# steineggerlab/Metabuli

Hardware: AMD Instinct MI355X
Metric: Mreads/s classified (metabuli classify hot path, reads + index resident in HBM) (higher is better)
Workload: dtype u64

## Files before the change

include/mtb.h:

```cpp
#ifndef MTB_H
#define MTB_H
#include <stddef.h>
#include <stdint.h>

#ifdef __cplusplus
extern "C" {
#endif

typedef enum {
    MTB_OK = 0,
    MTB_ERR_ARG = 1,
    MTB_ERR_IO = 2,
    MTB_ERR_DEVICE = 3,
    MTB_ERR_CAPACITY = 4,
    MTB_ERR_OOM = 5,
    MTB_ERR_UNSUPPORTED = 6
} mtb_status;

typedef struct { uint64_t value; uint64_t qinfo; } mtb_kmer;

typedef struct {
    uint64_t qinfo;
    int32_t  target_id;
    int32_t  species_id;
    uint32_t dna;
    uint16_t right_end_hamming;
    uint8_t  hamming;
    uint8_t  pad;
} mtb_match;

typedef struct {
    int32_t seq_mode;
    int32_t syncmer;
    int32_t smer_len;
    int32_t kmer_format;
    int32_t min_cons_cnt;
    int32_t min_cons_cnt_euk;
    float   min_score;
    float   min_sp_score;
    float   tie_ratio;
    int32_t accession_level;
    int32_t skip_redundancy;
} mtb_params;

typedef struct {
    int32_t  classification;
    float    score;
    int32_t  query_length;
    int32_t  query_length2;
    uint8_t  is_classified;
    uint8_t  reserved;
    uint16_t n_taxcnt;
    uint32_t taxcnt_off;
} mtb_result;

typedef struct mtb_ctx mtb_ctx;
typedef struct mtb_index mtb_index;

enum {
    MTB_K_EXTRACT_COUNT = 0, MTB_K_EXTRACT_EMIT = 1, MTB_K_RADIX_HIST = 2, MTB_K_RADIX_SCATTER = 3,
    MTB_K_JOIN = 4, MTB_K_REGROUP = 5, MTB_K_SEGSORT = 6, MTB_K_SCORE = 7, MTB_K_SCAN = 8, MTB_K_SCORE_FAST = 9,
    MTB_K_SCORE_MANY = 10,
    MTB_NUM_KERNELS = 11
};

typedef struct {
    float    ms_extract, ms_sort, ms_join, ms_regroup, ms_segsort, ms_score, ms_total;
    uint64_t n_reads, n_bases, n_kmers, n_matches, n_targets;
    float    ms_kernel[MTB_NUM_KERNELS];
    uint32_t n_launch[MTB_NUM_KERNELS];
    uint64_t n_generic_reads;
    uint64_t n_slot_reads;
    uint64_t n_deferred_reads, n_many_reads, n_many_matches, n_many_kept;
    int32_t  join_variant, join_tuned;
    float    join_tune_ms[3];
    uint32_t join_tiles, join_tiles_windowed, join_tiles_outside;
    uint32_t lslot_tail_factor, n_lslot_big_reads;
} mtb_batch_stats;

typedef enum { MTB_JOIN_AUTO = 0, MTB_JOIN_Q1W6 = 1, MTB_JOIN_Q2W5 = 2, MTB_JOIN_WINDOW = 3 } mtb_join_variant;

const char *mtb_version(void);
const char *mtb_last_error(void);
void mtb_default_params(mtb_params *p);

mtb_status mtb_ctx_create(int device, void *stream, mtb_ctx **out);
void       mtb_ctx_destroy(mtb_ctx *);
mtb_status mtb_ctx_sync(mtb_ctx *);
mtb_status mtb_ctx_set_profiling(mtb_ctx *, int on);
mtb_status mtb_ctx_set_streams(mtb_ctx *, int n);
mtb_status mtb_ctx_set_workspace_limit(mtb_ctx *, uint64_t bytes);
mtb_status mtb_ctx_set_placement_probe(mtb_ctx *, int on);
mtb_status mtb_ctx_set_join_variant(mtb_ctx *, int variant);
mtb_status mtb_ctx_set_option(mtb_ctx *, const char *name, const char *value);
uint32_t   mtb_ctx_last_sub_batches(const mtb_ctx *);
uint64_t   mtb_ctx_last_scratch_bytes(const mtb_ctx *);

mtb_status mtb_index_open(mtb_ctx *, const char *dbdir, const char *taxonomy_dir,
                          mtb_params *params, mtb_index **out);
mtb_status mtb_index_open_stats(const mtb_index *, uint64_t *out4);
mtb_status mtb_index_from_device(mtb_ctx *, uint64_t *d_values, uint32_t *d_info,
                                 uint64_t n_targets, const char *taxonomy_dir,
                                 const int32_t *taxid_list, size_t n_taxids,
                                 const mtb_params *params, mtb_index **out);
mtb_status mtb_index_clone(mtb_index *src, mtb_ctx *dst_ctx, mtb_index **out);
typedef struct {
    uint8_t  values_handle[64], info_handle[64], dir_handle[64], dirbase_handle[64];
    uint64_t values_off, info_off, dir_off, dirbase_off;
    uint64_t n_targets;
    uint32_t dir_buckets, info_mask;
    int32_t  dir_depth, packed, has_info, match_last, device;
    int64_t  exporter_pid;
    uint64_t values_ptr, info_ptr, dir_ptr, dirbase_ptr;
} mtb_index_share;
mtb_status mtb_index_export(mtb_index *src, mtb_index_share *out);
mtb_status mtb_index_import(mtb_ctx *, const mtb_index_share *, const char *taxonomy_dir, const int32_t *taxid_list, size_t n_taxids,
                            const mtb_params *params, mtb_index **out);
mtb_status mtb_index_seal(mtb_index *);
void       mtb_index_close(mtb_index *);
uint64_t   mtb_index_num_targets(const mtb_index *);
mtb_status mtb_index_state(const mtb_index *, int32_t *dir_depth, int32_t *packed, int32_t *sealed);
mtb_status mtb_index_download(mtb_index *, uint64_t *values, uint32_t *info, uint64_t cap);
int32_t    mtb_tax_lca(const mtb_index *, int32_t a, int32_t b);
int32_t    mtb_tax_species(const mtb_index *, int32_t taxid);
int32_t    mtb_tax_parent(const mtb_index *, int32_t taxid);
int32_t    mtb_tax_max_id(const mtb_index *);
int32_t    mtb_tax_original_id(const mtb_index *, int32_t taxid);
int32_t    mtb_tax_num_children(const mtb_index *, int32_t taxid);
int32_t    mtb_tax_child(const mtb_index *, int32_t taxid, int32_t k);
const char *mtb_tax_rank(const mtb_index *, int32_t taxid);
const char *mtb_tax_name(const mtb_index *, int32_t taxid);

mtb_status mtb_extract(mtb_ctx *, const mtb_params *, const char *bases, const uint64_t *offs,
                       const char *bases2, const uint64_t *offs2, uint64_t n_reads,
                       mtb_kmer *out, uint64_t cap, uint64_t *count,
                       int32_t *qlen, int32_t *qlen2);
mtb_status mtb_sort_kmers(mtb_ctx *, mtb_kmer *kmers, uint64_t n);
mtb_status mtb_match_kmers(mtb_ctx *, mtb_index *, const mtb_kmer *sorted, uint64_t n,
                     mtb_match *out, uint64_t cap, uint64_t *count);
mtb_status mtb_sort_matches(mtb_ctx *, mtb_match *matches, uint64_t n, uint64_t n_reads);
mtb_status mtb_score(mtb_ctx *, mtb_index *, const mtb_params *, const mtb_match *sorted,
                     uint64_t n_matches, uint64_t n_reads, const int32_t *qlen,
                     const int32_t *qlen2, mtb_result *results, int32_t *taxcnt_tax,
                     uint32_t *taxcnt_cnt, uint64_t taxcnt_cap, uint64_t *n_taxcnt);

mtb_status mtb_classify_batch(mtb_ctx *, mtb_index *, const mtb_params *, const char *bases,
                              const uint64_t *offs, const char *bases2, const uint64_t *offs2,
                              uint64_t n_reads, mtb_result *results, int32_t *taxcnt_tax,
                              uint32_t *taxcnt_cnt, uint64_t taxcnt_cap, uint64_t *n_taxcnt);
mtb_status mtb_classify_batch_device(mtb_ctx *, mtb_index *, const mtb_params *,
                                     const char *d_bases, const uint64_t *d_offs,
                                     const char *d_bases2, const uint64_t *d_offs2,
                                     uint64_t n_reads, uint64_t n_bases_total,
                                     mtb_result *d_results, int32_t *d_taxcnt_tax,
                                     uint32_t *d_taxcnt_cnt, uint64_t taxcnt_cap,
                                     uint64_t *n_taxcnt);
void      *mtb_host_alloc(size_t bytes);
void       mtb_host_free(void *);
mtb_status mtb_classify_batch_packed(mtb_ctx *, mtb_index *, const mtb_params *, const uint8_t *packed2, const uint8_t *nmask,
                                     const uint32_t *lens, const uint8_t *packed2_mate, const uint8_t *nmask_mate,
// ... 148 lines not shown
```

metabuli_amd/__init__.py:

```python
from __future__ import annotations

import ctypes as C
import os
import subprocess

import numpy as np

_HERE = os.path.dirname(os.path.abspath(__file__))
_CSRC = os.path.join(_HERE, "csrc")
LIB_PATH = os.environ.get("MTB_LIB") or os.path.join(_CSRC, "libmtb.so")

kmer_dt = np.dtype([("value", "<u8"), ("qinfo", "<u8")])
match_dt = np.dtype([("qinfo", "<u8"), ("target_id", "<i4"), ("species_id", "<i4"), ("dna", "<u4"),
                     ("reh", "<u2"), ("ham", "u1"), ("pad", "u1")])
result_dt = np.dtype([("classification", "<i4"), ("score", "<f4"), ("qlen", "<i4"), ("qlen2", "<i4"),
                      ("is_classified", "u1"), ("flag", "u1"), ("n_taxcnt", "<u2"), ("taxcnt_off", "<u4")])

block_dt = np.dtype([("seq", "<u4"), ("strand", "<i4"), ("start", "<u8"), ("end", "<u8")])

MTB_OK, MTB_ERR_ARG, MTB_ERR_IO, MTB_ERR_DEVICE, MTB_ERR_CAPACITY, MTB_ERR_OOM, MTB_ERR_UNSUPPORTED = range(7)


class Params(C.Structure):
    _fields_ = [("seq_mode", C.c_int32), ("syncmer", C.c_int32), ("smer_len", C.c_int32),
                ("kmer_format", C.c_int32), ("min_cons_cnt", C.c_int32), ("min_cons_cnt_euk", C.c_int32),
                ("min_score", C.c_float), ("min_sp_score", C.c_float), ("tie_ratio", C.c_float),
                ("accession_level", C.c_int32), ("skip_redundancy", C.c_int32)]


class BatchStats(C.Structure):
    _fields_ = [("ms_extract", C.c_float), ("ms_sort", C.c_float), ("ms_join", C.c_float), ("ms_regroup", C.c_float),
                ("ms_segsort", C.c_float), ("ms_score", C.c_float), ("ms_total", C.c_float),
                ("n_reads", C.c_uint64), ("n_bases", C.c_uint64), ("n_kmers", C.c_uint64),
                ("n_matches", C.c_uint64), ("n_targets", C.c_uint64),
                ("ms_kernel", C.c_float * 11), ("n_launch", C.c_uint32 * 11), ("n_generic_reads", C.c_uint64), ("n_slot_reads", C.c_uint64),
                ("n_deferred_reads", C.c_uint64), ("n_many_reads", C.c_uint64), ("n_many_matches", C.c_uint64), ("n_many_kept", C.c_uint64),
                ("join_variant", C.c_int32), ("join_tuned", C.c_int32), ("join_tune_ms", C.c_float * 3),
                ("join_tiles", C.c_uint32), ("join_tiles_windowed", C.c_uint32), ("join_tiles_outside", C.c_uint32),
                ("lslot_tail_factor", C.c_uint32), ("n_lslot_big_reads", C.c_uint32)]


SHARE_BYTES = 4 * 64 + 4 * 8 + 8 + 2 * 4 + 5 * 4 + 4 + 8 + 4 * 8
JOIN_VARIANTS = {0: "other", 1: "q1w6", 2: "q2w5", 3: "window", -3: "q1w5", -4: "q2w6", -15: "windoww5", -16: "windoww6", -17: "windoww7"}


class JoinFootprint(C.Structure):
    _fields_ = [("n_queries", C.c_uint64), ("distinct_buckets", C.c_uint64), ("dir_sectors", C.c_uint64),
                ("target_sectors", C.c_uint64), ("n_buckets", C.c_uint64), ("n_targets", C.c_uint64)]


KERNEL_NAMES = ["extract_count", "extract_emit", "radix_hist", "radix_scatter", "join", "regroup", "segsort", "score", "scan", "score_fast", "score_many"]


class MtbError(RuntimeError):
    def __init__(self, status, msg):
        super().__init__(f"mtb status {status}: {msg}")
        self.status = status


def build(force=False):
    if force and os.path.exists(LIB_PATH):
        os.remove(LIB_PATH)
    subprocess.check_call(["make", "-C", _CSRC, "libmtb.so"], stdout=subprocess.DEVNULL)
    return LIB_PATH


_lib = None


def lib():
    global _lib
    if _lib is not None:
        return _lib
    if not os.path.exists(LIB_PATH):
        raise RuntimeError(f"{LIB_PATH} not found: the HIP extension must be built (python -c 'import __graft_entry__ as g; g.build()'); "
                           "there is no CPU implementation of this path")
    L = C.CDLL(LIB_PATH)
    L.mtb_version.restype = C.c_char_p
    L.mtb_last_error.restype = C.c_char_p
    L.mtb_index_num_targets.restype = C.c_uint64
    L.mtb_index_num_targets.argtypes = [C.c_void_p]
    for f in ("mtb_tax_lca", "mtb_tax_species", "mtb_tax_parent", "mtb_tax_max_id"):
        getattr(L, f).restype = C.c_int32
    L.mtb_tax_lca.argtypes = [C.c_void_p, C.c_int32, C.c_int32]
    L.mtb_tax_species.argtypes = [C.c_void_p, C.c_int32]
    L.mtb_tax_parent.argtypes = [C.c_void_p, C.c_int32]
    L.mtb_tax_max_id.argtypes = [C.c_void_p]
    L.mtb_tax_original_id.restype = C.c_int32
    L.mtb_tax_original_id.argtypes = [C.c_void_p, C.c_int32]
    for f in ("mtb_tax_rank", "mtb_tax_name"):
        getattr(L, f).restype = C.c_char_p
        getattr(L, f).argtypes = [C.c_void_p, C.c_int32]
    _lib = L
    return L


def part_bounds(dbdir, n_parts):
    b = np.zeros(n_parts, np.uint64)
    _chk(lib().mtb_index_part_bounds(dbdir.encode(), C.c_uint32(n_parts), _p(b)))
    return b


def default_params(**kw):
    p = Params(seq_mode=1, syncmer=1, smer_len=5, kmer_format=2, min_cons_cnt=4, min_cons_cnt_euk=9,
               min_score=0.0, min_sp_score=0.0, tie_ratio=0.95, accession_level=0, skip_redundancy=1)
    for k, v in kw.items():
        setattr(p, k, v)
    return p


def _p(a):
    if a is None:
        return None
    if isinstance(a, int):
        return C.c_void_p(a)
    return a.ctypes.data_as(C.c_void_p)


def _chk(st):
    if st != MTB_OK:
        raise MtbError(st, lib().mtb_last_error().decode())

# ... 605 lines not shown
```

metabuli_amd/csrc/kernels_score.h:

```cpp
#ifndef MTB_KERNELS_SCORE_H
#define MTB_KERNELS_SCORE_H
#include "dev_util.h"
#include "mtb_core.h"
#include "kernels_join.h"
#include "mtb_score_par.h"

#ifdef MTB_SCORE_PHASE_CYCLES
#define MTB_NPHASE 16
__device__ unsigned long long mtb_phase_cycles[MTB_NPHASE];
__shared__ unsigned long long mtb_phase_lds[MTB_NPHASE];
#define MTB_PHASE_BEGIN() unsigned long long ph_t0_ = __builtin_readcyclecounter()
#define MTB_PHASE_MARK(k) do { unsigned long long t_ = __builtin_readcyclecounter(); if (threadIdx.x == 0) mtb_phase_lds[k] += t_ - ph_t0_; ph_t0_ = t_; } while (0)
#define MTB_PHASE_KERNEL_BEGIN() do { if (threadIdx.x < MTB_NPHASE) mtb_phase_lds[threadIdx.x] = 0; __syncthreads(); } while (0)
#define MTB_PHASE_KERNEL_END() do { __syncthreads(); if (threadIdx.x < MTB_NPHASE) atomicAdd(&mtb_phase_cycles[threadIdx.x], mtb_phase_lds[threadIdx.x]); } while (0)
#else
#define MTB_PHASE_BEGIN() do {} while (0)
#define MTB_PHASE_MARK(k) do {} while (0)
#define MTB_PHASE_KERNEL_BEGIN() do {} while (0)
#define MTB_PHASE_KERNEL_END() do {} while (0)
#endif

#ifndef MTB_SCORE_LDS
#define MTB_SCORE_LDS 160
#endif
#ifndef MTB_SCORE_MINWAVES
#define MTB_SCORE_MINWAVES 4
#endif
#define MTB_SCORE_BKT 128

__host__ __device__ __forceinline__ uint64_t score_slab_bytes(uint64_t n, uint64_t nb) {
    uint64_t b = mtb_sws_bytes<uint32_t>(n);
    b += nb * 12 + (MTB_LR_MAXE + MTB_LR_MAXE * MTB_LR_K) * 4 + ((nb + 15) & ~15ull);
    return (b + 63) & ~63ull;
}

__global__ __launch_bounds__(64) void k_taxcnt_bound(const uint64_t *__restrict__ seg_start, const uint32_t *__restrict__ cursor,
                                                      const int32_t *__restrict__ qlen, const int32_t *__restrict__ qlen2, uint64_t n_reads,
                                                      int32_t dna_shift, uint32_t *__restrict__ bound) {
    uint64_t r = (uint64_t)blockIdx.x * 64 + threadIdx.x;
    if (r >= n_reads) return;
    uint64_t nb = (uint64_t)mtb_num_buckets(qlen[r] + qlen2[r], dna_shift);
    if (cursor) { bound[r] = (uint32_t)nb; return; }
    uint64_t n = seg_start[r + 1] - seg_start[r];
    bound[r] = (uint32_t)(n < nb ? n : nb);
}

__global__ __launch_bounds__(256) void k_count_flags(const uint8_t *__restrict__ f, uint64_t n, unsigned long long *__restrict__ out) {
    uint32_t c = 0;
    for (uint64_t i = (uint64_t)blockIdx.x * 256 + threadIdx.x; i < n; i += (uint64_t)gridDim.x * 256) c += f[i] == 1 ? 1u : 0u;
    for (int d = 32; d > 0; d >>= 1) c += __shfl_down(c, d, 64);
    if ((threadIdx.x & 63) == 0 && c) atomicAdd(out, (unsigned long long)c);
}

__global__ __launch_bounds__(256) void k_list_flag2(const uint8_t *__restrict__ f, uint64_t n, uint32_t *__restrict__ list, uint32_t *__restrict__ n_list) {
    __shared__ uint32_t s_w[4]; __shared__ uint32_t s_base;
    const uint64_t r = (uint64_t)blockIdx.x * 256 + threadIdx.x;
    const bool on = r < n && f[r] == 2;
    const uint64_t m = __ballot(on);
    const uint32_t wv = threadIdx.x >> 6, lane = threadIdx.x & 63u;
    if (lane == 0) s_w[wv] = (uint32_t)__popcll(m);
    __syncthreads();
    if (threadIdx.x == 0) { const uint32_t tot = s_w[0] + s_w[1] + s_w[2] + s_w[3]; s_base = tot ? atomicAdd(n_list, tot) : 0u; }
    __syncthreads();
    if (on) {
        uint32_t at = s_base + (uint32_t)__popcll(m & ((1ull << lane) - 1ull));
        for (uint32_t q = 0; q < wv; q++) at += s_w[q];
        list[at] = (uint32_t)r;
    }
}

__global__ __launch_bounds__(256) void k_list_large(const uint64_t *__restrict__ seg_start, uint64_t n_reads, uint32_t threshold,
                                                     uint32_t *__restrict__ large, uint32_t *__restrict__ n_large, uint32_t *__restrict__ max_seg) {
    uint64_t r = (uint64_t)blockIdx.x * 256 + threadIdx.x;
    uint32_t n = 0;
    if (r < n_reads) {
        n = (uint32_t)(seg_start[r + 1] - seg_start[r]);
        if (n > threshold) large[atomicAdd(n_large, 1u)] = (uint32_t)r;
    }
    for (int d = 32; d > 0; d >>= 1) { uint32_t o = __shfl_down(n, d, 64); n = o > n ? o : n; }
    if ((threadIdx.x & 63) == 0 && n > threshold) atomicMax(max_seg, n);
}

__device__ __forceinline__ int32_t taxcnt_gather_wave(const int32_t *btax, const uint8_t *bham, int32_t nb, int32_t *otax, uint32_t *ocnt, int32_t cap) {
    const int32_t lane = (int32_t)threadIdx.x;
    int32_t ntc = 0;
    int32_t last = -1;
    while (ntc < cap) {
        int32_t mn = INT32_MAX;
        for (int32_t q = lane; q < nb; q += 64) if (bham[q] != 255) { int32_t t = btax[q]; if (t > last && t < mn) mn = t; }
        for (int d = 32; d > 0; d >>= 1) { int32_t o = __shfl_xor(mn, d, 64); mn = o < mn ? o : mn; }
        if (mn == INT32_MAX) break;
        uint32_t cnt = 0;
        for (int32_t q0 = 0; q0 < nb; q0 += 64) { int32_t q = q0 + lane; cnt += (uint32_t)__popcll(__ballot(q < nb && bham[q] != 255 && btax[q] == mn)); }
        if (lane == 0) { otax[ntc] = mn; ocnt[ntc] = cnt; }
        ntc++; last = mn;
    }
    return ntc;
}

template <typename IDX>
__device__ __forceinline__ void score_sync() {
    if (sizeof(IDX) == 2) { __builtin_amdgcn_fence(__ATOMIC_ACQ_REL, "wavefront"); __builtin_amdgcn_wave_barrier(); }
    else __syncthreads();
}

template <typename IDX, bool SORT, bool KEY64, typename REC, bool INPLACE = false, int CAP = MTB_SCORE_LDS>
__device__ __forceinline__ void score_read_par(const REC *src, int32_t n, mtb_sws<IDX> w, int32_t *btax,
                                               uint8_t *bham, int32_t *otax, uint32_t *ocnt, int32_t *lr_lev, int32_t *lr_anc,
                                               int32_t nb, int32_t read_len, const mtb_tax_view &tx, const mtb_score_params &sp,
                                               uint64_t tc_off, uint64_t tc_room, int32_t *__restrict__ tc_tax,
                                               uint32_t *__restrict__ tc_cnt, uint64_t tc_cap, mtb_match *__restrict__ sorted_out,
                                               mtb_result &R) {
    constexpr int MAXPER = (CAP + 63) / 64;
    if (sizeof(IDX) == 2) __builtin_assume(n >= 1 && n <= CAP);
    const int32_t lane = (int32_t)threadIdx.x;
    const uint64_t lt = lanemask_lt();
    w.n = n;
    MTB_PHASE_BEGIN();
    if (SORT) {
        uint64_t *k1 = (uint64_t *)w.path; uint32_t *k2 = (uint32_t *)(k1 + n);
        mtb_match rec[MAXPER]; uint64_t a1[MAXPER]; uint32_t a2[MAXPER]; int32_t rank[MAXPER];
#pragma unroll
        for (int k = 0; k < MAXPER; k++) {
            int32_t i = lane + 64 * k;
            rank[k] = 0; a1[k] = 0; a2[k] = 0;
            if (i < n) {
                rec[k] = rec_m(src[i]);
                if (KEY64) {
                    a1[k] = ((uint64_t)(uint32_t)rec[k].species_id << 41) | ((uint64_t)mtb_q_frame(rec[k].qinfo) << 38) |
                            ((uint64_t)(mtb_q_pos(rec[k].qinfo) & 0x7FFu) << 27) | ((uint64_t)(rec[k].hamming & 7u) << 24) | (rec[k].dna & 0xFFFFFFu);
                    k1[i] = a1[k];
                } else { a1[k] = mtb_key1(rec[k]); a2[k] = mtb_key2(rec[k]); k1[i] = a1[k]; k2[i] = a2[k]; }
            }
        }
        score_sync<IDX>();
        MTB_PHASE_MARK(0);
        const int32_t nslot = (n + 63) >> 6;
        uint32_t n_desc = 0; int32_t split = 0;
#pragma unroll
        for (int k = 0; k < MAXPER; k++) {
// ... 656 lines not shown
```

metabuli_amd/csrc/kernels_score_fast.h:

```cpp
#ifndef MTB_KERNELS_SCORE_FAST_H
#define MTB_KERNELS_SCORE_FAST_H
#include "dev_util.h"
#include "kernels_score.h"
#include "mtb_core.h"
#include "mtb_score_par.h"

#define MTB_FAST_BKT 128
#ifndef MTB_FAST_MERGE_SINGLES
#define MTB_FAST_MERGE_SINGLES 1
#endif

#ifdef MTB_FAST_DEBUG
__device__ unsigned long long mtb_fast_reasons[32];
#define MTB_FAST_COUNT(k, v) do { if (threadIdx.x == 0) atomicAdd(&mtb_fast_reasons[k], (unsigned long long)(v)); } while (0)
#define MTB_FAST_T0() unsigned long long ft_ = __builtin_readcyclecounter()
#define MTB_FAST_MARK(k) do { const unsigned long long t_ = __builtin_readcyclecounter(); if (threadIdx.x == 0) s_ph[k] += t_ - ft_; ft_ = t_; } while (0)
#else
#define MTB_FAST_COUNT(k, v) do {} while (0)
#define MTB_FAST_T0() do {} while (0)
#define MTB_FAST_MARK(k) do {} while (0)
#endif

#define MTB_DPP_RED(v, OP) do { \
    { const uint32_t o_ = (uint32_t)__builtin_amdgcn_update_dpp((int)(v), (int)(v), 0x111, 0xF, 0xF, false); (v) = OP((v), o_); } \
    { const uint32_t o_ = (uint32_t)__builtin_amdgcn_update_dpp((int)(v), (int)(v), 0x112, 0xF, 0xF, false); (v) = OP((v), o_); } \
    { const uint32_t o_ = (uint32_t)__builtin_amdgcn_update_dpp((int)(v), (int)(v), 0x114, 0xF, 0xF, false); (v) = OP((v), o_); } \
    { const uint32_t o_ = (uint32_t)__builtin_amdgcn_update_dpp((int)(v), (int)(v), 0x118, 0xF, 0xF, false); (v) = OP((v), o_); } \
    { const uint32_t o_ = (uint32_t)__builtin_amdgcn_update_dpp((int)(v), (int)(v), 0x142, 0xA, 0xF, false); (v) = OP((v), o_); } \
    { const uint32_t o_ = (uint32_t)__builtin_amdgcn_update_dpp((int)(v), (int)(v), 0x143, 0xC, 0xF, false); (v) = OP((v), o_); } } while (0)
#define MTB_MINU(a, b) ((b) < (a) ? (b) : (a))
#define MTB_MAXU(a, b) ((b) > (a) ? (b) : (a))
__device__ __forceinline__ uint32_t wave_min_u32(uint32_t v) { MTB_DPP_RED(v, MTB_MINU); return (uint32_t)__builtin_amdgcn_readlane((int)v, 63); }
__device__ __forceinline__ uint32_t wave_max_u32(uint32_t v) { MTB_DPP_RED(v, MTB_MAXU); return (uint32_t)__builtin_amdgcn_readlane((int)v, 63); }

struct FKey { uint32_t lo, hi; };
__device__ __forceinline__ uint32_t fk_species(const FKey &k) { return k.hi >> 10; }
__device__ __forceinline__ uint32_t fk_frame(const FKey &k) { return (k.hi >> 7) & 7u; }
__device__ __forceinline__ uint32_t fk_pos(const FKey &k) { return ((k.hi & 127u) << 4) | (k.lo >> 27); }
__device__ __forceinline__ uint32_t fk_ham(const FKey &k) { return (k.lo >> 24) & 7u; }
__device__ __forceinline__ uint32_t fk_dna(const FKey &k) { return k.lo & 0xFFFFFFu; }

struct FastPath { int32_t start, end; float score; int32_t ham; uint32_t rehs;  int32_t species; };

template <int K, int KL = K, bool BYFRAME = false>
__global__ __launch_bounds__(64, K <= 3 ? 5 : 4) void k_score_fast(const mtb_slot16 *__restrict__ slots_all, uint64_t n_reads, const int32_t *__restrict__ qlen,
                                                       const int32_t *__restrict__ qlen2, mtb_tax_view tx, mtb_score_params sp,
                                                       const uint64_t *__restrict__ tc_off, mtb_result *__restrict__ results,
                                                       int32_t *__restrict__ tc_tax, uint32_t *__restrict__ tc_cnt, uint64_t tc_cap, uint64_t tc_base,
                                                       const uint32_t *__restrict__ cursor, uint32_t stride, uint32_t direct, uint32_t epoch,
                                                       uint8_t *__restrict__ slow_flag, uint32_t *__restrict__ cnt_out) {
    constexpr int NMAX = 64 * K;
    __shared__ FKey s_key[NMAX];
    __shared__ uint64_t s_aux[NMAX];
    __shared__ uint64_t s_pp[NMAX];
    __shared__ FastPath s_path[64];
    __shared__ uint32_t s_pf[64];
    __shared__ uint32_t s_tl[(BYFRAME || MTB_FAST_MERGE_SINGLES) ? 64 : 1];
    typedef uint32_t __attribute__((may_alias)) u32a; typedef int32_t __attribute__((may_alias)) i32a;
    static_assert(NMAX * 8 >= 2 * MTB_FAST_BKT * 4 && NMAX * 8 >= 256 * 4 && NMAX * 8 >= (MTB_LR_MAXE + MTB_LR_MAXE * MTB_LR_K) * 4, "tables fit the arrays they live in");
    u32a *const s_hcnt = (u32a *)s_pp;
    u32a *const s_hmin = (u32a *)s_key; i32a *const s_btax = (i32a *)s_key + MTB_FAST_BKT;
    i32a *const s_otax = (i32a *)s_pp; u32a *const s_ocnt = (u32a *)s_pp + MTB_FAST_BKT;
    i32a *const s_lev = (i32a *)s_aux; i32a *const s_anc = (i32a *)s_aux + MTB_LR_MAXE;
    const int32_t lane = (int32_t)threadIdx.x;
    MTB_BEGIN_ACQUIRE();
#ifdef MTB_FAST_DEBUG
    __shared__ unsigned long long s_ph[16];
    if (threadIdx.x < 16) s_ph[threadIdx.x] = 0;
#endif
    const uint64_t lt = lanemask_lt();
    const uint64_t le = lt | (1ull << lane);
    const uint32_t tail_cap = stride - direct;
    const uint32_t div_m = (65536u + (uint32_t)sp.dna_shift - 1u) / (uint32_t)sp.dna_shift;
    const uint32_t lines = (stride * (uint32_t)sizeof(mtb_slot16) + 127u) / 128u;

    for (uint64_t r = blockIdx.x; r < n_reads; r += gridDim.x) {
        if (r + gridDim.x < n_reads && (uint32_t)lane < lines) {
            const uint8_t *pf = (const uint8_t *)(slots_all + (r + gridDim.x) * (uint64_t)stride) + (uint64_t)lane * 128u;
            __builtin_amdgcn_global_load_lds((const __attribute__((address_space(1))) void *)pf, (__attribute__((address_space(3))) void *)s_pf, 4, 0, 0);
        }
        MTB_FAST_T0();
        const int32_t ql1 = qlen[r], ql2 = qlen2[r];
        const int32_t read_len = ql1 + ql2;
        const int32_t nb = mtb_num_buckets(read_len, sp.dna_shift);
        const uint32_t cur = cursor[r];
        const mtb_slot16 *slots = slots_all + r * (uint64_t)stride;
        mtb_slot16 x[KL];
#pragma unroll
        for (int k = 0; k < KL; k++) { const uint32_t i = (uint32_t)lane + 64u * k; x[k].a = 0; x[k].b = 0; if (i < stride) x[k] = slots[i]; }
        bool slow = cur > tail_cap || nb > MTB_FAST_BKT;
        wave_fence();
        MTB_FAST_MARK(0);
        int32_t n = 0, n_live = 0;
        uint32_t spc[KL]; bool live[KL]; int32_t dst[KL];
        uint32_t smin = 0xFFFFFFFFu, smax = 0u;
#pragma unroll
        for (int k = 0; k < KL; k++) {
            const uint32_t i = (uint32_t)lane + 64u * k;
            live[k] = i < stride && mtb_slot_epoch(x[k]) == epoch && (i < direct || i - direct < cur);
            spc[k] = live[k] ? (uint32_t)(x[k].a >> 32) : 0xFFFFFFFFu;
            dst[k] = 0;
            n_live += (int32_t)__popcll(__ballot(live[k]));
            smin = spc[k] < smin ? spc[k] : smin;
            if (live[k]) smax = spc[k] > smax ? spc[k] : smax;
        }
        smin = wave_min_u32(smin); smax = wave_max_u32(smax);
        uint32_t todo_min = 0xFFFFFFFFu;
        if (smin != smax) {
            for (int32_t q = lane; q < 256; q += 64) s_hcnt[q] = 0;
            wave_fence();
#pragma unroll
            for (int k = 0; k < KL; k++) if (live[k]) atomicAdd(&s_hcnt[(spc[k] * 0x9E3779B1u) >> 24], 1u);
            wave_fence();
#pragma unroll
            for (int k = 0; k < KL; k++) if (live[k] && s_hcnt[(spc[k] * 0x9E3779B1u) >> 24] < 2u) { live[k] = false; spc[k] = 0xFFFFFFFFu; }
        } else if (n_live < 2) {
#pragma unroll
            for (int k = 0; k < KL; k++) { live[k] = false; spc[k] = 0xFFFFFFFFu; }
        }
        if (BYFRAME) {
#pragma unroll
            for (int k = 0; k < KL; k++) if (live[k]) spc[k] = (spc[k] << 3) | ((uint32_t)(x[k].b >> 52) & 7u);
        }
#pragma unroll
        for (int k = 0; k < KL; k++) todo_min = spc[k] < todo_min ? spc[k] : todo_min;
        for (int round = 0; ; round++) {
            const uint32_t m = wave_min_u32(todo_min);
            if (m == 0xFFFFFFFFu) break;
            if (round == 24) { slow = true; break; }
            todo_min = 0xFFFFFFFFu;
#pragma unroll
            for (int k = 0; k < KL; k++) {
                const bool mine = spc[k] == m;
                const uint64_t mask = __ballot(mine);
                if (mine) { dst[k] = n + (int32_t)__popcll(mask & lt); spc[k] = 0xFFFFFFFFu; }
                n += (int32_t)__popcll(mask);
                todo_min = spc[k] < todo_min ? spc[k] : todo_min;
            }
        }
        if (KL > K && n > NMAX) slow = true;
#pragma unroll
        for (int k = 0; k < KL; k++) {
            if (live[k] && !slow) {
                const uint64_t b = x[k].b;
                const uint32_t bh = (uint32_t)(b >> 32), ps_ = (bh >> 8) & 0x7FFu;
                FKey fk; fk.hi = ((uint32_t)(x[k].a >> 32) << 10) | (((bh >> 20) & 7u) << 7) | (ps_ >> 4);
                fk.lo = ((ps_ & 15u) << 27) | (((bh >> 23) & 7u) << 24) | ((uint32_t)b & 0xFFFFFFu);
                s_key[dst[k]] = fk;
                s_aux[dst[k]] = (x[k].a & 0xFFFFFFFFull) | (((b >> 24) & 0xFFFFull) << 32) | ((uint32_t)lane + 64u * k >= direct ? (1ull << 63) : 0ull);
            }
        }
        MTB_FAST_MARK(1);
        mtb_result R = mtb_result_blank(ql1, ql2, (uint32_t)tc_base);
        if (!slow && n == 0) { if (lane == 0) { cnt_out[r] = (uint32_t)n_live; results[r] = R; } continue; }
        wave_fence();
        {
            uint32_t nt = 0;
            bool any_tail = false;
#pragma unroll
            for (int k = 0; k < KL; k++) any_tail |= live[k] && (uint32_t)lane + 64u * k >= direct;
            if ((BYFRAME || MTB_FAST_MERGE_SINGLES) && !slow && __any(any_tail)) {
                FKey ke[K]; uint64_t ax[K]; int32_t np[K]; bool tl[K];
                const int32_t nsl = (n + 63) >> 6;
                auto same_run = [&](const FKey &a, const FKey &b) { return BYFRAME ? ((a.hi ^ b.hi) >> 7) == 0 : ((a.hi ^ b.hi) >> 10) == 0; };
                auto less = [&](const FKey &a, const FKey &b) { return a.hi < b.hi || (a.hi == b.hi && a.lo < b.lo); };
                bool unsorted = false;
#pragma unroll
                for (int k = 0; k < K; k++) {
                    const int32_t i = lane + 64 * k;
                    ke[k].lo = 0; ke[k].hi = 0; ax[k] = 0; np[k] = i; tl[k] = false;
                    if (k < nsl && i < n) {
                        ke[k] = s_key[i]; ax[k] = s_aux[i]; tl[k] = (ax[k] >> 63) != 0;
                        if (i > 0 && !tl[k]) { const FKey pk = s_key[i - 1]; if ((s_aux[i - 1] >> 63) == 0 && same_run(pk, ke[k]) && less(ke[k], pk)) unsorted = true; }
                    }
                    if (k < nsl) {
                        const uint64_t tm = __ballot(tl[k]);
                        if (tl[k]) { const uint32_t at = nt + (uint32_t)__popcll(tm & lt); if (at < 64u) s_tl[at] = (uint32_t)i; }
                        nt += (uint32_t)__popcll(tm);
                    }
                }
                if (nt > 64u || __any(unsorted)) slow = true;
                wave_fence();
                if (!slow) {
                    const bool mine = (uint32_t)lane < nt;
                    const int32_t ti = mine ? (int32_t)s_tl[lane] : 0;
                    const FKey kt = s_key[ti]; const uint64_t at = s_aux[ti];
                    uint32_t n_tl_run = 0, n_tl_less = 0;
                    for (uint32_t u = 0; u < nt; u++) {
                        FKey ku; ku.hi = (uint32_t)rl_i((int32_t)kt.hi, (int32_t)u); ku.lo = (uint32_t)rl_i((int32_t)kt.lo, (int32_t)u);
                        if (same_run(ku, kt)) { n_tl_run++; n_tl_less += (less(ku, kt) || (!less(kt, ku) && u < (uint32_t)lane)) ? 1u : 0u; }
#pragma unroll
                        for (int k = 0; k < K; k++)
                            if (k < nsl && !tl[k] && same_run(ke[k], ku) && !less(ke[k], ku)) np[k]++;
                    }
                    const uint32_t rid = BYFRAME ? kt.hi >> 7 : kt.hi >> 10;
                    int32_t lo0 = 0, hi0 = n, lo1 = 0, hi1 = n;
                    for (int32_t len = n; len; len >>= 1) {
                        const int32_t m0 = (lo0 + hi0) >> 1, m1 = (lo1 + hi1) >> 1;
                        const uint32_t r0 = BYFRAME ? s_key[m0 < n ? m0 : 0].hi >> 7 : s_key[m0 < n ? m0 : 0].hi >> 10;
                        const uint32_t r1 = BYFRAME ? s_key[m1 < n ? m1 : 0].hi >> 7 : s_key[m1 < n ? m1 : 0].hi >> 10;
                        if (lo0 < hi0) { if (r0 < rid) lo0 = m0 + 1; else hi0 = m0; }
                        if (lo1 < hi1) { if (r1 <= rid) lo1 = m1 + 1; else hi1 = m1; }
                    }
                    const int32_t run_start = lo0, n_dir_run = lo1 - lo0 - (int32_t)n_tl_run;
                    int32_t lo2 = run_start, hi2 = run_start + n_dir_run;
                    for (int32_t len = n; len; len >>= 1) {
                        const int32_t m2 = (lo2 + hi2) >> 1;
                        const FKey km = s_key[m2 < n ? m2 : 0];
                        if (lo2 < hi2) { if (less(km, kt)) lo2 = m2 + 1; else hi2 = m2; }
                    }
                    const int32_t place = lo2 + (int32_t)n_tl_less;
                    wave_fence();
#pragma unroll
                    for (int k = 0; k < K; k++) { const int32_t i = lane + 64 * k; if (k < nsl && i < n && !tl[k]) { s_key[np[k]] = ke[k]; s_aux[np[k]] = ax[k]; } }
                    if (mine) { s_key[place] = kt; s_aux[place] = at & ~(1ull << 63); }
                    wave_fence();
                }
            }
        }
        FKey key[K]; uint32_t tid[K], reh[K];
        int32_t tcanon[K]; uint8_t euk[K];
        const mtb_tax_node *nodes = (const mtb_tax_node *)tx.node;
        bool bhead[K], linked[K];
        int32_t shv[K];
        uint64_t bmask[K + 1], lmask[K + 1], rmask[K];
        const int32_t nslot = (n + 63) >> 6;
        bool bad = false, bad2 = false;
#ifdef MTB_FAST_DEBUG
        if (slow) MTB_FAST_COUNT(cur > tail_cap || nb > MTB_FAST_BKT ? 0 : 1, 1);
#endif
#pragma unroll
        for (int k = 0; k < K; k++) {
            const int32_t i = lane + 64 * k;
            key[k].lo = 0; key[k].hi = 0; tid[k] = 0; reh[k] = 0; bhead[k] = true; linked[k] = false; shv[k] = 0; tcanon[k] = -1; euk[k] = 0;
            bmask[k] = ~0ull; lmask[k] = 0; rmask[k] = 0;
            if (k < nslot && !slow) {
                FKey pk; pk.lo = 0; pk.hi = 0;
                if (i < n) {
                    key[k] = s_key[i]; const uint64_t a = s_aux[i]; tid[k] = (uint32_t)a; reh[k] = (uint32_t)(a >> 32) & 0xFFFFu; if (i > 0) pk = s_key[i - 1];
                }
                {
                    const int32_t t_ = (int32_t)tid[k], s_ = (int32_t)fk_species(key[k]);
                    const bool tv = i < n && t_ >= 0 && t_ <= tx.max_taxid, sv = i < n && s_ >= 0 && s_ <= tx.max_taxid;
                    const int32_t tc_ = nodes[tv ? t_ : 0].canon; const uint8_t eu_ = tx.under_euk[sv ? s_ : 0];
                    tcanon[k] = tv ? tc_ : -1; euk[k] = sv ? eu_ : 0;
                }
                const bool first = i == 0;
                if (i < n && !first) {
                    if (pk.hi > key[k].hi || (pk.hi == key[k].hi && pk.lo > key[k].lo)) bad = true;
                    if (pk.hi == key[k].hi && ((pk.lo ^ key[k].lo) >> 27) == 0) bad2 = true;
                }
                bhead[k] = i >= n || first || ((pk.hi ^ key[k].hi) >> 7) != 0;
                if (i < n && !bhead[k]) {
                    const int32_t pos = (int32_t)fk_pos(key[k]), ppos = (int32_t)fk_pos(pk);
                    const int32_t s = (pos - ppos) / 3;
                    if (s > 0 && s <= sp.max_codon_shift) {
                        shv[k] = s;
                        const bool fwd = fk_frame(key[k]) < 3u;
                        linked[k] = mtb_consecutive(fk_dna(pk), fk_dna(key[k]), s, fwd, sp.kmer_format);
                    }
                }
                bmask[k] = __ballot(bhead[k]);
                lmask[k] = __ballot(linked[k]);
                rmask[k] = __ballot(i < n && !linked[k]);
            }
        }
        bmask[K] = ~0ull; lmask[K] = 0;
#ifdef MTB_FAST_DEBUG
        if (!slow) { if (__any(bad)) MTB_FAST_COUNT(2, 1); else if (__any(bad2)) MTB_FAST_COUNT(3, 1); }
#endif
        slow = slow || __any(bad || bad2);
        if (slow) { if (lane == 0) slow_flag[r] = cur > tail_cap ? 2 : 1; continue; }
        if (lane == 0) cnt_out[r] = (uint32_t)n_live;
        MTB_FAST_MARK(2);
        float ps[K]; int32_t phd[K]; int32_t root[K];
        bool cand[K];
        {
            float carry_s = 0.0f; int32_t carry_hd = 0, last_root = 0;
#pragma unroll
            for (int k = 0; k < K; k++) {
                ps[k] = 0.0f; phd[k] = 0; root[k] = 0; cand[k] = false;
                if (k < nslot) {
                    const int32_t i = lane + 64 * k;
                    float is = 0.0f; int32_t ihd = 0;
                    if (linked[k]) mtb_link_inc(reh[k], shv[k], &is, &ihd);
                    ps[k] = wave_inclusive_scan_dpp(is) + carry_s; phd[k] = wave_inclusive_scan_dpp(ihd) + carry_hd;
                    carry_s = rl_f(ps[k], 63); carry_hd = rl_i(phd[k], 63);
                    const uint64_t mr = rmask[k];
                    const uint64_t lo_roots = mr & le;
                    root[k] = lo_roots ? 64 * k + 63 - (int32_t)__builtin_clzll(lo_roots) : last_root;
                    if (mr) last_root = 64 * k + 63 - (int32_t)__builtin_clzll(mr);
                    if (i < n) s_pp[i] = (uint64_t)__float_as_uint(ps[k]) | ((uint64_t)(uint32_t)phd[k] << 32);
                    const uint64_t bnext = (bmask[k] >> 1) | ((bmask[k + 1] & 1ull) << 63);
                    const uint64_t lnext = (lmask[k] >> 1) | ((lmask[k + 1] & 1ull) << 63);
                    const bool has_next = !((bnext >> lane) & 1ull);
                    const bool conn = (lnext >> lane) & 1ull;
                    cand[k] = i < n && (!bhead[k] || has_next) && !conn;
                }
            }
        }
        wave_fence();
        MTB_FAST_MARK(3);
        int32_t ne = 0;
        bool too_many = false;
#pragma unroll
        for (int k = 0; k < K; k++) {
            if (k < nslot) {
                bool e = false;
                FastPath P; P.start = 0; P.end = 0; P.score = 0.0f; P.ham = 0; P.rehs = 0; P.species = 0;
                if (cand[k]) {
                    const int32_t spc = (int32_t)fk_species(key[k]);
                    const int32_t md = euk[k] ? sp.min_cons_cnt_euk : sp.min_cons_cnt;
                    const int32_t rt = root[k];
                    const uint64_t pr = s_pp[rt]; const FKey rkey = s_key[rt];
                    const uint32_t rreh = (uint32_t)(s_aux[rt] >> 32);
                    const int32_t dhd = phd[k] - (int32_t)(uint32_t)(pr >> 32);
                    const int32_t depth = 1 + mtb_link_depth(dhd);
                    if (depth >= md) {
                        e = true;
                        P.start = (int32_t)fk_pos(rkey);
                        P.end = (int32_t)fk_pos(key[k]) + 23;
                        P.score = mtb_part_score(rreh, 8, false) + (rt == lane + 64 * k ? 0.0f : ps[k] - __uint_as_float((uint32_t)pr));
                        P.ham = (int32_t)fk_ham(rkey) + (rt == lane + 64 * k ? 0 : mtb_link_ham(dhd));
                        P.rehs = rreh | (reh[k] << 16);
                        P.species = spc;
                    }
                }
                const uint64_t me = __ballot(e);
                const int32_t at = ne + (int32_t)__popcll(me & lt);
                if (e && at < 64) s_path[at] = P;
                ne += (int32_t)__popcll(me);
            }
        }
        too_many = ne > 64;
        if (too_many) MTB_FAST_COUNT(4, 1); else { MTB_FAST_COUNT(5, 1); MTB_FAST_COUNT(6, ne); }
        if (too_many) { if (lane == 0) slow_flag[r] = 1; continue; }
        if (ne == 0) { if (lane == 0) results[r] = R; continue; }
        wave_fence();
        MTB_FAST_MARK(4);
        FastPath P = s_path[lane < ne ? lane : 0];
        const bool have = lane < ne;
        int32_t prev_spc = __shfl_up(P.species, 1, 64);
        const bool shead = have && (lane == 0 || prev_spc != P.species);
        const uint64_t hmask = __ballot(shead);
        const int32_t nsp = (int32_t)__popcll(hmask);
        MTB_FAST_COUNT(7, nsp);

        float sp_score = -1.0f; int32_t sp_id = 0;
        int32_t s_idx = 0;
        const uint32_t ord = __float_as_uint(P.score);
        const uint32_t tie = ((uint32_t)(1023 - (P.ham < 1023 ? P.ham : 1023)) << 17) | ((uint32_t)(P.start & 0x7FF) << 6) | (uint32_t)(63 - lane);
        for (uint64_t hm = hmask; hm; hm &= hm - 1, s_idx++) {
            const int32_t slo = (int32_t)__builtin_ctzll(hm);
            const int32_t shi = (hm & (hm - 1)) ? (int32_t)__builtin_ctzll(hm & (hm - 1)) : ne;
            const bool in = lane >= slo && lane < shi;
// ... 140 lines not shown
```

metabuli_amd/csrc/mtb_api.hip:

```cpp
#include <hip/hip_runtime.h>

#include <fcntl.h>
#include <limits.h>
#include <stdlib.h>
#include <sys/stat.h>
#include <unistd.h>

#include <atomic>
#include <chrono>
#include <condition_variable>
#include <mutex>
#include <functional>
#include <map>
#include <string>
#include <thread>
#include <vector>

#include "../../include/mtb.h"
#include "host_db.h"
#include "host/merge_plan.h"
#include "host/audit_plan.h"
#include "host/clade_filter.h"
#include "kernels_extract.h"
#include "kernels_extract_blocks.h"
#include "kernels_index.h"
#include "kernels_join.h"
#include "kernels_build.h"
#include "kernels_merge.h"
#include "kernels_clade_filter.h"
#include "kernels_audit.h"
#include "kernels_coverage.h"
#include "kernels_inspect.h"
#include "kernels_dir.h"
#include "kernels_scan.h"
#include "kernels_score.h"
#include "kernels_score_fast.h"
#include "kernels_score_long.h"
#include "kernels_score_many.h"
#include "kernels_seg_order.h"
#include "kernels_sort.h"
#include "mtb_core.h"
#include "mtb_options.h"

#if defined(__HIP_DEVICE_COMPILE__) && defined(__AMDGCN__) && !defined(__gfx950__)
#error "libmtb is written for gfx950 (MI355X) only: 160 KB of LDS per CU (k_score_long holds 70 KB per workgroup), global_load_lds_dwordx4, wave64"
#endif

static thread_local std::string g_err;
static mtb_status fail(mtb_status s, const std::string &m) { g_err = m; return s; }

#define HIPCHK(x)                                                                                  \
    do {                                                                                           \
        hipError_t e_ = (x);                                                                       \
        if (e_ != hipSuccess)                                                                      \
            return fail(MTB_ERR_DEVICE, std::string(#x) + ": " + hipGetErrorString(e_));           \
    } while (0)
#define STCHK(x)                                                                                   \
    do { mtb_status s_ = (x); if (s_ != MTB_OK) return s_; } while (0)

__global__ __launch_bounds__(256) void k_taxcnt_n(const mtb_result *__restrict__ res, uint64_t n, uint32_t *__restrict__ cnt) {
    const uint64_t i = (uint64_t)blockIdx.x * 256 + threadIdx.x;
    if (i < n) cnt[i] = res[i].n_taxcnt;
}
__global__ __launch_bounds__(256) void k_taxcnt_pack(mtb_result *__restrict__ res, uint64_t n, const uint64_t *__restrict__ new_off, const int32_t *__restrict__ tt,
                                                      const uint32_t *__restrict__ tc, int32_t *__restrict__ tt2, uint32_t *__restrict__ tc2) {
    const uint64_t i = (uint64_t)blockIdx.x * 256 + threadIdx.x;
    if (i >= n) return;
    const uint32_t k = res[i].n_taxcnt, src = res[i].taxcnt_off;
    const uint64_t dst = new_off[i];
    for (uint32_t j = 0; j < k; j++) { tt2[dst + j] = tt[src + j]; tc2[dst + j] = tc[src + j]; }
    res[i].taxcnt_off = (uint32_t)dst;
}

__global__ __launch_bounds__(256) void k_pack_slots(const uint32_t *__restrict__ lens, uint64_t n, uint32_t *__restrict__ slots) {
    const uint64_t i = (uint64_t)blockIdx.x * 256 + threadIdx.x;
    if (i < n) slots[i] = (lens[i] + 7u) >> 3;
}
__global__ __launch_bounds__(64) void k_unpack_reads(const uint8_t *__restrict__ packed2, const uint8_t *__restrict__ nmask, const uint64_t *__restrict__ offs,
                                                     const uint64_t *__restrict__ slot_off, uint64_t n, char *__restrict__ bases) {
    for (uint64_t r = blockIdx.x; r < n; r += gridDim.x) {
        const uint64_t o = offs[r], s0 = slot_off[r];
        const uint32_t L = (uint32_t)(offs[r + 1] - o);
        for (uint32_t k = threadIdx.x; k < L; k += 64) {
            const uint64_t g = s0 + (k >> 3); const uint32_t j = k & 7u;
            const uint32_t w = (uint32_t)packed2[2 * g] | ((uint32_t)packed2[2 * g + 1] << 8);
            const bool bad = (nmask[g] >> j) & 1u;
            const uint32_t c = (w >> (2 * j)) & 3u;
            bases[o + k] = bad ? 'N' : (char)((0x47544341u >> (8 * c)) & 0xFFu);
        }
    }
}

enum BufKind : uint8_t { BUF_WORK = 0, BUF_IO = 1, BUF_FIXED = 2 };
struct DevBuf { void *p = nullptr; size_t cap = 0; BufKind kind = BUF_WORK; };
#define MTB_SLAB_POOL_MAX (16ull << 30)
#define MTB_LONG_WIN_MAX_PER_Q 24.0
#define MTB_OVF_STRIPES 256u

enum Scal : uint32_t {
    SC_JOIN_COUNT = 0, SC_JOIN_OVERFLOW = 1,
    SC_BAD_SEQ = SC_JOIN_OVERFLOW,
    SC_N_LARGE = 2, SC_MAX_SEG = 3,
    SC_MAX_LEN = 4, SC_OPEN_CARRY = 5,
    SC_N_GENERIC = 6, SC_LONG_N_SECOND = 7,
    SC_EXTRACT = 8, SC_WIN_STATS = 16,
    SC_N_UNGROUPED = 18, SC_MAX_BIG_SEG = 19, SC_N_DEFERRED = 20, SC_DEFER_N_LARGE = 21,
    SC_SCORE_WORK = 22, SC_LONG_WORK = 24,
    SC_LS_N_FAIL = 25, SC_LS_N_ALL = 26, SC_LS_MAX_SEG = 27, SC_LS_WORK = 28,
    SC_OPEN_FLAGS = 29, SC_WORDS = 30
};
struct ExtractCounters { uint64_t records , overflow, real, max_q , off_max_q, off_reads, off_max_len , spare; };
static_assert(sizeof(ExtractCounters) == 8 * (SC_WIN_STATS - SC_EXTRACT) && SC_WIN_STATS + 2 <= SC_N_UNGROUPED && SC_SCORE_WORK + 2 <= SC_LONG_WORK && SC_OPEN_FLAGS < SC_WORDS, "scalar names overlap or leave the block");
struct mtb_ctx {
    int device = 0;
    int audit_mode = 0;
    hipStream_t stream = nullptr;
    mtb_tables *d_tabs = nullptr;
    mtb_tables h_tabs;
    std::map<std::string, DevBuf> bufs;
    std::mutex bufs_mu;
    std::mutex reserve_mu;
    std::atomic<bool> reserve_cancel{false};
    uint64_t *d_scal = nullptr;
    unsigned long long *d_ovfctr = nullptr;
    uint64_t ovf_region = 0, ovf_max_region = 0;
    hipEvent_t ev[8];
    mtb_batch_stats stats;
    int profiling = 0;
    struct KEv { int id; hipEvent_t a, b; };
    std::vector<KEv> kev;
    std::vector<hipEvent_t> ev_pool;
    std::vector<mtb_ctx *> lanes;
    bool is_lane = false;
    uint32_t seg_epoch = 0;
    const void *seg_clean_p = nullptr; size_t seg_clean_cap = 0;
    double extract_yield = 0.0;
    uint64_t part_n_reads = 0; uint32_t part_max_len = 0;
    int part_mode = 0; uint32_t part_max_q = 0; uint64_t part_nk_real = 0;
    bool placement_probe = false;
    uint64_t ws_limit = 0;
    double ws_per_base = 0.0;
    uint64_t ws_max_sub_bases = 0;
    int ws_seq_mode = 0;
    uint32_t last_sub_batches = 0;
    bool fast_used = false;
    const mtb_kmer *last_sorted = nullptr; uint64_t last_sorted_n = 0;
    struct DeadSeg { char *p; size_t cap, used; };
    DeadSeg dead[3]; int n_dead = 0;
    uint64_t last_scratch_bytes = 0;
    hipStream_t copy_stream = nullptr; hipEvent_t copy_done[2] = {nullptr, nullptr};
    hipEvent_t unpacked[2] = {nullptr, nullptr};
    bool unpacked_rec[2] = {false, false};
    uint64_t prefetch_issued = 0, prefetch_used = 0;
    hipStream_t down_stream = nullptr; hipEvent_t down_ready = nullptr, down_done = nullptr; bool down_pending = false; int res_set = 0;
    int pk_set = 0;
    struct Prefetched { const void *key = nullptr, *key2 = nullptr; uint64_t n_reads = 0; bool valid = false; } pre[2];
    struct JoinTune { uint64_t key = 0; int calls = 0, pending = -1, best = -1; float ms[3] = {0.0f, 0.0f, 0.0f}; hipEvent_t e0 = nullptr, e1 = nullptr; } join_tunes[4]; uint32_t join_tune_next = 0;
    uint64_t many_stats[4] = {0, 0, 0, 0};
    uint32_t lslot_tf_start = 1;
    unsigned long long *d_cov_pend = nullptr; uint64_t cov_pend_words = 0; bool cov_call = false;
    MtbOptions opt;
};
template <typename T> static T *scal(mtb_ctx *c, Scal s) { return (T *)(c->d_scal + s); }
static hipError_t scal_clear(mtb_ctx *c, Scal first, uint32_t words = 1) { return hipMemsetAsync(c->d_scal + first, 0, 8 * (size_t)words, c->stream); }
static DevBuf buf_get(mtb_ctx *c, const std::string &name) { std::lock_guard<std::mutex> lk(c->bufs_mu); auto it = c->bufs.find(name); return it == c->bufs.end() ? DevBuf() : it->second; }
static size_t buf_cap(mtb_ctx *c, const char *name) { return buf_get(c, name).cap; }
static size_t held_bytes(mtb_ctx *c, BufKind upto) { std::lock_guard<std::mutex> lk(c->bufs_mu); size_t b = 0; for (auto &kv : c->bufs) if (kv.second.kind == BUF_WORK || kv.second.kind == upto) b += kv.second.cap; return b; }
static void release_workspace(mtb_ctx *c) {
    std::lock_guard<std::mutex> lk(c->bufs_mu);
    for (auto &kv : c->bufs) if (kv.second.p && kv.second.kind != BUF_IO) { hipError_t e = hipFree(kv.second.p); (void)e; kv.second.p = nullptr; kv.second.cap = 0; }
    c->ws_per_base = 0.0; c->ws_max_sub_bases = 0;
    c->seg_clean_p = nullptr; c->seg_clean_cap = 0;
}

struct KTimer {
    mtb_ctx *c; int id; hipEvent_t a = nullptr, b = nullptr;
    KTimer(mtb_ctx *c_, int id_) : c(c_), id(id_) {
        if (!c->profiling) return;
        a = take(); b = take();
        hipError_t e = hipEventRecord(a, c->stream); (void)e;
    }
    ~KTimer() {
        if (!c->profiling) return;
        hipError_t e = hipEventRecord(b, c->stream); (void)e;
        c->kev.push_back({id, a, b});
    }
    hipEvent_t take() {
        hipEvent_t ev;
        if (!c->ev_pool.empty()) { ev = c->ev_pool.back(); c->ev_pool.pop_back(); return ev; }
        hipError_t e = hipEventCreate(&ev); (void)e;
        return ev;
    }
};
static void collect_kernel_times(mtb_ctx *c) {
    for (auto &k : c->kev) {
        float ms = 0;
        if (hipEventElapsedTime(&ms, k.a, k.b) == hipSuccess) { c->stats.ms_kernel[k.id] += ms; c->stats.n_launch[k.id]++; }
        c->ev_pool.push_back(k.a); c->ev_pool.push_back(k.b);
    }
    c->kev.clear();
}

struct mtb_index {
    mtb_ctx *ctx = nullptr;
    uint64_t T = 0;
    uint64_t *d_values = nullptr; uint32_t *d_info = nullptr; bool own = false;
    bool own_tax = true;
    bool match_last = false;
    mtbhost::Taxonomy tax;
    int32_t *d_canon = nullptr, *d_parent = nullptr, *d_depth = nullptr, *d_spparent = nullptr, *d_tax2species = nullptr;
    uint8_t *d_under = nullptr, *d_accleaf = nullptr;
    mtb_tax_node *d_node = nullptr;
    mtb_params params;
    uint32_t info_mask = 0xFFFFFFFFu;
    uint32_t *d_dir = nullptr; uint64_t *d_dirbase = nullptr; int32_t dir_L = 0; uint32_t dir_buckets = 0;
    bool packed = false;
    bool info_owned = false;
    std::mutex state_mu; std::condition_variable state_cv; int users = 0;
    int views = 0;
    mtb_index *parent = nullptr;
    uint64_t open_chunks = 0, open_chunk_words = 0, open_peak_bytes = 0, open_free0 = 0;
    void *ipc_stage[4] = {nullptr, nullptr, nullptr, nullptr};
    bool is_part = false;
    uint32_t *d_cov_bits = nullptr; unsigned long long *d_cov_hits = nullptr;
};

enum ResKind { RES_ROWS = 0, RES_TAX = 1, RES_CNT = 2 };
static const char *res_name(ResKind k, int set) { static const char *const names[2][3] = {{"results", "tctax2", "tccnt2"}, {"resultsb", "tctax2b", "tccnt2b"}}; return names[set ? 1 : 0][k]; }
template <typename T>
static mtb_status ensure(mtb_ctx *c, const char *name, size_t elems, T **out, BufKind kind = BUF_WORK) {
    if (c->down_pending) {
        const int fl = c->res_set ^ 1;
        if (!strcmp(name, res_name(RES_ROWS, fl)) || !strcmp(name, res_name(RES_TAX, fl)) || !strcmp(name, res_name(RES_CNT, fl))) { HIPCHK(hipEventSynchronize(c->down_done)); c->down_pending = false; }
    }
    std::lock_guard<std::mutex> lk(c->bufs_mu);
    DevBuf &b = c->bufs.emplace(name, DevBuf{nullptr, 0, kind}).first->second;
    size_t bytes = elems * sizeof(T);
    if (bytes == 0) bytes = 64;
// ... 50 lines not shown
        const size_t want = bytes + bytes / 16 + 256 + (c->opt.segm_pad ? (1u << 20) : 0);
        hipError_t e = hipExtMallocWithFlags(&b.p, want, hipDeviceMallocContiguous);
        if (e != hipSuccess) { b.p = nullptr; (void)hipGetLastError(); return fail(MTB_ERR_OOM, std::string("contiguous allocation failed for ") + name + ": " + hipGetErrorString(e)); }
        b.cap = want;
        *out = (mtb_slot16 *)b.p;
        return MTB_OK;
    }
    const bool no_probe = c->opt.no_placement_probe != 0, env_probe = c->opt.placement_probe != 0;
    if (b.cap >= bytes || bytes < (8ull << 30) || no_probe || !(c->placement_probe || env_probe)) return plain();
    if (b.p) { hipError_t e = hipFree(b.p); (void)e; b.p = nullptr; b.cap = 0; }
    const size_t want = bytes + bytes / 16 + 256;
    const auto t_begin = std::chrono::steady_clock::now();
    struct Cand { void *p; float ms; size_t bytes; };
    std::vector<Cand> held;
    std::vector<float> seen; std::vector<void *> seen_p, pads; std::vector<size_t> sizes;
    hipEvent_t e0 = nullptr, e1 = nullptr;
    struct Guard {
        std::vector<Cand> &held; std::vector<void *> &pads; hipEvent_t &e0, &e1; bool armed = true;
        ~Guard() { if (!armed) return; for (auto &h : held) { hipError_t e = hipFree(h.p); (void)e; } for (void *q : pads) { hipError_t e = hipFree(q); (void)e; }
                   if (e0) { hipError_t e = hipEventDestroy(e0); (void)e; } if (e1) { hipError_t e = hipEventDestroy(e1); (void)e; } }
    } guard{held, pads, e0, e1};
    HIPCHK(hipEventCreate(&e0)); HIPCHK(hipEventCreate(&e1));
    for (int attempt = 0; attempt < 8; attempt++) {
        if (attempt >= 2 && std::chrono::duration<double>(std::chrono::steady_clock::now() - t_begin).count() > 2.0) break;
        size_t fr = 0, tot = 0;
        HIPCHK(hipMemGetInfo(&fr, &tot));
        if (want + (attempt ? (8ull << 30) : 0) > fr) {
            if (held.size() < 2) break;
            size_t worst = 0; for (size_t k = 1; k < held.size(); k++) if (held[k].ms > held[worst].ms) worst = k;
            { hipError_t e = hipFree(held[worst].p); (void)e; } held.erase(held.begin() + (long)worst);
            void *pad = nullptr;
            if (hipMalloc(&pad, ((size_t)(attempt % 3) + 1) * (3ull << 30)) == hipSuccess) pads.push_back(pad); else (void)hipGetLastError();
            HIPCHK(hipMemGetInfo(&fr, &tot));
            if (want + (4ull << 30) > fr) break;
        }
        void *p = nullptr;
        const size_t ask = want;
        if (hipMalloc(&p, ask) != hipSuccess) { (void)hipGetLastError(); break; }
        sizes.push_back(ask);
        float best = 1e30f;
        for (int rep = 0; rep < 3; rep++) {
            HIPCHK(hipEventRecord(e0, c->stream));
            hipLaunchKernelGGL(k_probe_scatter, dim3(8192), dim3(256), 0, c->stream, (mtb_slot16 *)p, (uint64_t)(bytes / sizeof(mtb_slot16)), 8u, 12345u + (uint32_t)rep);
            HIPCHK(hipEventRecord(e1, c->stream));
            HIPCHK(hipEventSynchronize(e1));
            float ms = 0; HIPCHK(hipEventElapsedTime(&ms, e0, e1));
            if (rep && ms < best) best = ms;
        }
        held.push_back({p, best, ask}); seen.push_back(best); seen_p.push_back(p);
        float lo = 1e30f; for (float v : seen) lo = std::min(lo, v);
        int near = 0; for (float v : seen) if (v <= lo * 1.03f) near++;
        float hi = 0.0f; for (float v : seen) hi = std::max(hi, v);
        if (seen.size() >= 4 && near >= 2 && lo <= 0.9f * hi) break;
    }
    guard.armed = false;
    (void)hipEventDestroy(e0); (void)hipEventDestroy(e1);
    for (void *q : pads) { hipError_t e = hipFree(q); (void)e; }
    if (held.empty()) return plain();
    size_t pick = 0;
    for (size_t k = 1; k < held.size(); k++) if (held[k].ms < held[pick].ms) pick = k;
    for (size_t k = 0; k < held.size(); k++) if (k != pick) { hipError_t e = hipFree(held[k].p); (void)e; }
    std::vector<Cand> &cands = held;
    if (c->opt.placement_verbose) { fprintf(stderr, "mtb: slot buffer placement probe:"); for (size_t k = 0; k < seen.size(); k++) fprintf(stderr, " %.3f@%p", seen[k], seen_p[k]); fprintf(stderr, " ms -> %.3f (%.0f ms spent)\n", cands[pick].ms, std::chrono::duration<double, std::milli>(std::chrono::steady_clock::now() - t_begin).count()); }
    b.p = cands[pick].p; b.cap = cands[pick].bytes;
    *out = (mtb_slot16 *)b.p;
    return MTB_OK;
}
static void release(mtb_ctx *c, const char *name) {
    std::lock_guard<std::mutex> lk(c->bufs_mu);
    auto it = c->bufs.find(name);
    if (it != c->bufs.end()) { if (it->second.p) { hipError_t e = hipFree(it->second.p); (void)e; } c->bufs.erase(it); }
}

extern "C" {

const char *mtb_version(void) { return "metabuli_amd 0.1 (gfx950)"; }
const char *mtb_last_error(void) { return g_err.c_str(); }

void mtb_default_params(mtb_params *p) {
    p->seq_mode = 2; p->syncmer = 0; p->smer_len = 5; p->kmer_format = 1; p->min_cons_cnt = 4; p->min_cons_cnt_euk = 9;
    p->min_score = 0.0f; p->min_sp_score = 0.0f; p->tie_ratio = 0.95f; p->accession_level = 0; p->skip_redundancy = 0;
}

mtb_status mtb_ctx_create(int device, void *stream, mtb_ctx **out) {
    if (!out) return fail(MTB_ERR_ARG, "out is NULL");
    int n = 0;
    hipError_t e = hipGetDeviceCount(&n);
    if (e != hipSuccess || n <= 0) return fail(MTB_ERR_DEVICE, "no HIP device available (this library has no CPU path)");
    if (device < 0 || device >= n) return fail(MTB_ERR_ARG, "bad device ordinal");
    HIPCHK(hipSetDevice(device));
    mtb_ctx *c = new mtb_ctx();
    c->device = device; c->stream = (hipStream_t)stream;
    mtb_build_tables(&c->h_tabs);
    HIPCHK(hipMalloc((void **)&c->d_tabs, sizeof(mtb_tables)));
    HIPCHK(hipMemcpy(c->d_tabs, &c->h_tabs, sizeof(mtb_tables), hipMemcpyHostToDevice));
    HIPCHK(hipMalloc((void **)&c->d_scal, SC_WORDS * sizeof(uint64_t)));
    HIPCHK(hipMalloc((void **)&c->d_ovfctr, MTB_OVF_STRIPES * 64));
    for (int i = 0; i < 8; i++) HIPCHK(hipEventCreate(&c->ev[i]));
    memset(&c->stats, 0, sizeof(c->stats));
    mtbopt::from_environment(&c->opt);
    *out = c;
    return MTB_OK;
}
void mtb_ctx_destroy(mtb_ctx *c) {
    if (!c) return;
    for (mtb_ctx *l : c->lanes) mtb_ctx_destroy(l);
    c->lanes.clear();
    hipError_t e = hipSetDevice(c->device); (void)e;
    e = hipStreamSynchronize(c->stream);
    { std::lock_guard<std::mutex> lk(c->bufs_mu); for (auto &kv : c->bufs) if (kv.second.p) e = hipFree(kv.second.p); }
    if (c->d_tabs && !c->is_lane) e = hipFree(c->d_tabs);
    if (c->d_scal) e = hipFree(c->d_scal);
    if (c->d_ovfctr) e = hipFree(c->d_ovfctr);
    if (c->d_cov_pend && !c->is_lane) e = hipFree(c->d_cov_pend);
    if (c->is_lane && c->stream) e = hipStreamDestroy(c->stream);
    if (c->down_stream) { e = hipStreamSynchronize(c->down_stream); e = hipStreamDestroy(c->down_stream); }
    if (c->down_ready) e = hipEventDestroy(c->down_ready);
    if (c->down_done) e = hipEventDestroy(c->down_done);
    if (c->copy_stream) { e = hipStreamSynchronize(c->copy_stream); e = hipStreamDestroy(c->copy_stream); }
    for (int k = 0; k < 2; k++) { if (c->copy_done[k]) e = hipEventDestroy(c->copy_done[k]); if (c->unpacked[k]) e = hipEventDestroy(c->unpacked[k]); }
    for (int q = 0; q < 4; q++) if (c->join_tunes[q].e0) { e = hipEventDestroy(c->join_tunes[q].e0); e = hipEventDestroy(c->join_tunes[q].e1); }
    for (int i = 0; i < 8; i++) e = hipEventDestroy(c->ev[i]);
    for (auto &k : c->kev) { e = hipEventDestroy(k.a); e = hipEventDestroy(k.b); }
    for (auto &x : c->ev_pool) e = hipEventDestroy(x);
    delete c;
}
mtb_status mtb_ctx_sync(mtb_ctx *c) { HIPCHK(hipStreamSynchronize(c->stream)); return MTB_OK; }
mtb_status mtb_ctx_set_profiling(mtb_ctx *c, int on) {
    if (!c) return fail(MTB_ERR_ARG, "NULL ctx");
    c->profiling = on;
    for (mtb_ctx *l : c->lanes) l->profiling = on;
    return MTB_OK;
}
mtb_status mtb_ctx_set_placement_probe(mtb_ctx *c, int on) {
    if (!c) return fail(MTB_ERR_ARG, "NULL ctx");
    c->placement_probe = on != 0;
    for (mtb_ctx *l : c->lanes) l->placement_probe = on != 0;
    return MTB_OK;
}
mtb_status mtb_ctx_set_workspace_limit(mtb_ctx *c, uint64_t bytes) {
    if (!c) return fail(MTB_ERR_ARG, "NULL ctx");
    c->ws_limit = bytes;
    for (mtb_ctx *l : c->lanes) l->ws_limit = bytes;
    return MTB_OK;
}
mtb_status mtb_ctx_set_option(mtb_ctx *c, const char *name, const char *value) {
    if (!c || !name) return fail(MTB_ERR_ARG, "NULL ctx / name");
    if (!mtbopt::set(&c->opt, name, value)) return fail(MTB_ERR_ARG, std::string("unknown switch or bad value: ") + name + "=" + (value ? value : "(unset)"));
    for (mtb_ctx *l : c->lanes) l->opt = c->opt;
    return MTB_OK;
}
mtb_status mtb_ctx_set_join_variant(mtb_ctx *c, int variant) {
    static const char *const names[] = {"auto", "q1w6", "q2w5", "window"};
    if (!c || variant < 0 || variant > 3) return fail(MTB_ERR_ARG, "variant must be MTB_JOIN_AUTO .. MTB_JOIN_WINDOW");
    return mtb_ctx_set_option(c, "MTB_JOIN_VARIANT", names[variant]);
}
uint32_t mtb_ctx_last_sub_batches(const mtb_ctx *c) { return c ? c->last_sub_batches : 0; }
uint64_t mtb_ctx_last_scratch_bytes(const mtb_ctx *c) { return c ? c->last_scratch_bytes : 0; }
mtb_status mtb_ctx_set_streams(mtb_ctx *c, int n) {
    if (!c || n < 1 || n > 8) return fail(MTB_ERR_ARG, "streams must be 1..8");
    HIPCHK(hipSetDevice(c->device));
    while ((int)c->lanes.size() > (n == 1 ? 0 : n)) { mtb_ctx_destroy(c->lanes.back()); c->lanes.pop_back(); }
    while (n > 1 && (int)c->lanes.size() < n) {
        mtb_ctx *l = new mtb_ctx();
        l->device = c->device; l->is_lane = true; l->d_tabs = c->d_tabs; l->h_tabs = c->h_tabs; l->profiling = c->profiling; l->placement_probe = c->placement_probe; l->opt = c->opt;
        HIPCHK(hipStreamCreateWithFlags(&l->stream, hipStreamNonBlocking));
        HIPCHK(hipMalloc((void **)&l->d_scal, SC_WORDS * sizeof(uint64_t)));
        HIPCHK(hipMalloc((void **)&l->d_ovfctr, MTB_OVF_STRIPES * 64));
        for (int i = 0; i < 8; i++) HIPCHK(hipEventCreate(&l->ev[i]));
        memset(&l->stats, 0, sizeof(l->stats));
        c->lanes.push_back(l);
    }
    return MTB_OK;
}

}

static mtb_status d2h(mtb_ctx *c, void *dst, const void *src, size_t bytes) {
    HIPCHK(hipMemcpyAsync(dst, src, bytes, hipMemcpyDeviceToHost, c->stream));
    HIPCHK(hipStreamSynchronize(c->stream));
    return MTB_OK;
}
static mtb_status h2d(mtb_ctx *c, void *dst, const void *src, size_t bytes) {
    if (bytes == 0) return MTB_OK;
    HIPCHK(hipMemcpyAsync(dst, src, bytes, hipMemcpyHostToDevice, c->stream));
    HIPCHK(hipStreamSynchronize(c->stream));
    return MTB_OK;
}

static bool sort_msd_first(const mtb_ctx *c) { return !c->opt.sort_lsd; }

static uint64_t extract_bound(uint64_t n_bases, uint32_t grid) { return 2 * n_bases + (uint64_t)grid * MTB_EXTRACT_CHUNK; }
static uint64_t extract_cap_guess(const mtb_ctx *c, const mtb_params *p, uint64_t n_bases, uint32_t grid) {
    const double guess = c->extract_yield > 0.0 ? c->extract_yield : (p->syncmer ? 1.0 : 2.0);
    return std::min<uint64_t>(extract_bound(n_bases, grid), (uint64_t)((double)n_bases * guess * 1.15) + 4096 + (uint64_t)grid * 64);
}

struct Reads {
    const char *d_bases = nullptr; const uint64_t *d_offs = nullptr; const char *d_bases2 = nullptr; const uint64_t *d_offs2 = nullptr; uint64_t n_reads = 0;
    Reads range(uint64_t lo, uint64_t cnt) const { Reads r = *this; r.d_offs += lo; if (r.d_offs2) r.d_offs2 += lo; r.n_reads = cnt; return r; }
};
struct ReadLens { const int32_t *d_ql = nullptr, *d_ql2 = nullptr; uint32_t max_len = 0; };
struct ResultSink { mtb_result *d_res = nullptr; int32_t *d_tc_tax = nullptr; uint32_t *d_tc_cnt = nullptr; uint64_t tc_cap = 0, tc_base = 0; };
struct ExtractOpts {
    bool single_pass = false;
    bool tag_ordinals = false, want_digits = false;
    bool want_max_len = true;
    uint32_t *d_counts = nullptr;
    uint8_t *d_off_reads = nullptr;
};
struct Extracted {
    mtb_kmer *d_k = nullptr; uint64_t nk = 0, nk_real = 0;
    uint32_t max_len = 0, max_q = 0;
    uint16_t *d_dig = nullptr; uint64_t n_bases = 0;
    uint64_t off_max_q = 0, off_reads = 0, off_max_len = 0;
};
static mtb_status dev_extract(mtb_ctx *c, const mtb_params *p, const Reads &rd, int32_t *d_qlen, int32_t *d_qlen2, const ExtractOpts &opt, Extracted *ex) {
    const uint64_t n_reads = rd.n_reads;
    if (n_reads >= (1ull << 29)) return fail(MTB_ERR_ARG, "more than 2^29-1 reads per batch (sequenceID is 29 bits, Kmer.h:13)");
    if (p->kmer_format != 1 && p->kmer_format != 2) return fail(MTB_ERR_UNSUPPORTED, "only kmer_format 1 and 2 are implemented");
    if (p->syncmer && (p->smer_len < 1 || p->smer_len > 8)) return fail(MTB_ERR_ARG, "smer_len out of range");
    *ex = Extracted();
    if (n_reads == 0) return MTB_OK;
    const bool single_pass = opt.single_pass;
    ExtractArgs a{rd.d_bases, rd.d_offs, rd.d_bases2, rd.d_offs2, n_reads, p->seq_mode, p->syncmer, p->smer_len, p->kmer_format, (single_pass && opt.tag_ordinals) ? 1 : 0, sort_msd_first(c) ? 54 : 34};
    uint32_t grid = (uint32_t)std::min<uint64_t>(n_reads, 256ull * 256);
    HIPCHK(scal_clear(c, SC_MAX_LEN));
    uint64_t &n_bases = ex->n_bases;
    if (single_pass) {
        uint64_t o[2];
        STCHK(d2h(c, &o[0], rd.d_offs, 8)); STCHK(d2h(c, &o[1], rd.d_offs + n_reads, 8));
        n_bases = o[1] - o[0];
        if (p->seq_mode == 2 && rd.d_offs2) { STCHK(d2h(c, &o[0], rd.d_offs2, 8)); STCHK(d2h(c, &o[1], rd.d_offs2 + n_reads, 8)); n_bases += o[1] - o[0]; }
    }
    if (single_pass && n_bases) {
        const uint64_t bound = extract_bound(n_bases, grid);
        uint64_t cap = extract_cap_guess(c, p, n_bases, grid);
        cap = std::max<uint64_t>(cap, std::min<uint64_t>(bound, buf_cap(c, "kmersA") / sizeof(mtb_kmer)));
        for (int attempt = 0; attempt < 2; attempt++) {
            mtb_kmer *d_k; uint16_t *d_dig = nullptr;
            STCHK(ensure(c, "kmersA", cap, &d_k));
            if (opt.want_digits) { STCHK(ensure(c, "digA", cap + 8, &d_dig)); ex->d_dig = d_dig; }
            HIPCHK(scal_clear(c, SC_EXTRACT, 8));
            if (opt.d_off_reads) HIPCHK(hipMemsetAsync(opt.d_off_reads, 0, n_reads, c->stream));
            { KTimer kt(c, MTB_K_EXTRACT_EMIT);
            hipLaunchKernelGGL((k_extract<2>), dim3(grid), dim3(64), 0, c->stream, a, c->d_tabs, opt.d_counts, (const uint64_t *)nullptr,
                               d_k, d_qlen, d_qlen2, scal<uint32_t>(c, SC_MAX_LEN), scal<unsigned long long>(c, SC_EXTRACT), cap, d_dig, opt.d_off_reads); }
            HIPCHK(hipGetLastError());
            ExtractCounters sc;
            STCHK(d2h(c, &sc, scal<uint64_t>(c, SC_EXTRACT), sizeof(sc)));
            ex->off_max_q = sc.off_max_q; ex->off_reads = sc.off_reads; ex->off_max_len = sc.off_max_len;
            if (opt.want_max_len) { uint64_t ml = 0; STCHK(d2h(c, &ml, scal<uint64_t>(c, SC_MAX_LEN), 8)); ex->max_len = (uint32_t)ml; }
            if (sc.overflow == 0) {
                if (sc.records >= (1ull << 32)) return fail(MTB_ERR_ARG, "more than 2^32-1 query metamers in one batch; split the batch");
                c->extract_yield = (double)sc.records / (double)n_bases;
                ex->d_k = d_k; ex->nk = sc.records; ex->nk_real = sc.real; ex->max_q = (uint32_t)sc.max_q;
                return MTB_OK;
            }
            if (cap >= bound) return fail(MTB_ERR_DEVICE, "extract: output bound exceeded");
            cap = bound;
        }
    }
    uint32_t *d_cnt; uint64_t *d_koff; uint64_t *d_ws;
    STCHK(ensure(c, "counts", n_reads, &d_cnt)); STCHK(ensure(c, "koff", n_reads + 1, &d_koff));
    STCHK(ensure(c, "scanws", scan_ws_elems(n_reads + 1), &d_ws));
// ... 297 lines not shown
    } else {
        JoinSegArgs sa; memset(&sa, 0, sizeof(sa));
        hipLaunchKernelGGL((k_join<false>), dim3(grid), dim3(256), 0, c->stream, d_q, n, index_view(ix), (const mtb_tables *)c->d_tabs,
                           (const uint64_t *)d_bounds, d_out, cap, scal<unsigned long long>(c, SC_JOIN_COUNT), d_read_cnt, scal<uint32_t>(c, SC_JOIN_OVERFLOW), sa);
    } }
    HIPCHK(hipGetLastError());
    uint64_t sc[2];
    STCHK(d2h(c, sc, scal<uint64_t>(c, SC_JOIN_COUNT), 16));
    if (win_tiles) {
        uint64_t ws[2];
        STCHK(d2h(c, ws, scal<uint64_t>(c, SC_WIN_STATS), 16));
        c->stats.join_tiles = win_tiles; c->stats.join_tiles_windowed = (uint32_t)ws[0]; c->stats.join_tiles_outside = (uint32_t)ws[1];
    }
    if (striped) {
        unsigned long long h[MTB_OVF_STRIPES * 8];
        STCHK(d2h(c, h, c->d_ovfctr, sizeof(h)));
        uint64_t tot = 0, mx = 0;
        for (uint32_t k = 0; k < MTB_OVF_STRIPES; k++) { tot += h[8 * k]; mx = std::max<uint64_t>(mx, h[8 * k]); }
        c->ovf_max_region = mx;
        if (seg->rb) {
            *count = tot;
            if (tot > seg->ovf_cap) return fail(MTB_ERR_CAPACITY, "match buffer too small");
            return MTB_OK;
        }
        *count = mx > c->ovf_region ? (mx + mx / 8 + 64) * MTB_OVF_STRIPES : tot;
        if (tot >= (1ull << 32)) return fail(MTB_ERR_ARG, "more than 2^32-1 matches in one batch; split the batch");
        if (mx > c->ovf_region) return fail(MTB_ERR_CAPACITY, "match buffer too small");
        return MTB_OK;
    }
    c->ovf_region = 0;
    *count = sc[0];
    if (sc[0] >= (1ull << 32)) return fail(MTB_ERR_ARG, "more than 2^32-1 matches in one batch; split the batch");
    if (sc[0] > (seg ? seg->ovf_cap : cap)) return fail(MTB_ERR_CAPACITY, "match buffer too small");
    return MTB_OK;
}

template <typename REC>
static mtb_status dev_regroup(mtb_ctx *c, const mtb_match *d_in, uint64_t m, uint64_t n_reads, uint32_t *d_read_cnt,
                              uint64_t **seg_start, REC *d_out) {
    uint64_t *d_seg; uint64_t *d_ws; uint32_t *d_cur;
    STCHK(ensure(c, "segstart", n_reads + 1, &d_seg));
    STCHK(ensure(c, "scanws", scan_ws_elems(n_reads + 1), &d_ws));
    STCHK(ensure(c, "cursor", n_reads, &d_cur));
    { KTimer kt(c, MTB_K_SCAN); scan_launch<uint32_t, uint64_t, false>(c->stream, d_read_cnt, n_reads, true, d_seg, d_ws); }
    HIPCHK(hipMemsetAsync(d_cur, 0, n_reads * 4, c->stream));
    if (m) { KTimer kt(c, MTB_K_REGROUP); hipLaunchKernelGGL((k_regroup<REC>), dim3((uint32_t)((m + 255) / 256)), dim3(256), 0, c->stream, d_in, m, (const uint64_t *)d_seg, d_cur, d_out); }
    HIPCHK(hipGetLastError());
    *seg_start = d_seg;
    return MTB_OK;
}

static mtb_status dev_segsort(mtb_ctx *c, mtb_match *d_m, const uint64_t *d_seg, uint64_t n_reads, uint32_t *max_seg) {
    uint32_t *d_large;
    STCHK(ensure(c, "large", n_reads, &d_large));
    HIPCHK(scal_clear(c, SC_N_LARGE, 2));
    uint32_t grid = (uint32_t)std::min<uint64_t>(n_reads, 256ull * 40);
    { KTimer kt(c, MTB_K_SEGSORT);
    hipLaunchKernelGGL(k_segsort_small, dim3(grid), dim3(64), 0, c->stream, d_m, d_seg, n_reads, d_large, scal<uint32_t>(c, SC_N_LARGE),
                       scal<uint32_t>(c, SC_MAX_SEG)); }
    hipLaunchKernelGGL((k_segsort_large<mtb_match>), dim3(1024), dim3(256), 0, c->stream, d_m, d_seg, (const uint32_t *)d_large,
                       scal<const uint32_t>(c, SC_N_LARGE));
    HIPCHK(hipGetLastError());
    if (max_seg) { uint64_t sc[2]; STCHK(d2h(c, sc, scal<uint64_t>(c, SC_N_LARGE), 16)); *max_seg = (uint32_t)sc[1]; }
    return MTB_OK;
}

struct ScoreSrc {
    const mtb_match *m = nullptr;
    const uint64_t *seg = nullptr;
    const uint32_t *cursor = nullptr;
    uint32_t stride = 0, direct = 0, epoch = 0;
    uint32_t *big_list = nullptr, *n_big = nullptr;
    uint32_t *cnt_out = nullptr;
    uint32_t cap = MTB_SCORE_LDS;
    const uint32_t *list = nullptr, *n_list = nullptr;
    int seg_by_list = 0;
    bool sort = false;
    uint32_t max_seg = 0;
    uint32_t max_len_deferred = 0;
    uint32_t grid = 0;
    const uint8_t *only_flagged = nullptr;
    const uint32_t *seg_cnt = nullptr;
    const void *bound_by_buckets = nullptr;
};

struct ScoreLaunch { const uint64_t *d_tcoff; bool key64; mtb_score_params sp; ReadLens lens; ResultSink out; };
typedef std::function<mtb_status(ScoreSrc *, bool *, const ScoreLaunch &)> ScoreSecond;
static mtb_status taxcnt_layout(mtb_ctx *c, uint64_t n_reads, const uint64_t *d_seg, const uint32_t *d_cnt, const ReadLens &lens, const ResultSink &out, int dna_shift, uint64_t *d_tcoff, uint64_t *n_tc) {
    uint32_t *d_bound; uint64_t *d_ws;
    STCHK(ensure(c, "bound", n_reads, &d_bound)); STCHK(ensure(c, "scanws", scan_ws_elems(n_reads + 1), &d_ws));
    hipLaunchKernelGGL(k_taxcnt_bound, dim3((uint32_t)((n_reads + 63) / 64)), dim3(64), 0, c->stream, d_seg, d_cnt, lens.d_ql, lens.d_ql2, n_reads, dna_shift, d_bound);
    { KTimer kt(c, MTB_K_SCAN); scan_launch<uint32_t, uint64_t, false>(c->stream, d_bound, n_reads, true, d_tcoff, d_ws); }
    STCHK(d2h(c, n_tc, d_tcoff + n_reads, 8));
    if (*n_tc > out.tc_cap) return fail(MTB_ERR_CAPACITY, "taxcnt buffers too small");
    if (out.tc_base + *n_tc >= (1ull << 32)) return fail(MTB_ERR_ARG, "more than 2^32-1 taxcnt slots in one batch (mtb_result.taxcnt_off is 32 bits); split the batch");
    return MTB_OK;
}
static mtb_status dev_score(mtb_ctx *c, mtb_index *ix, const mtb_params *p, uint64_t n_reads, const ReadLens &lens, const ResultSink &out, uint64_t *n_tc,
                            const ScoreSrc &first, const ScoreSecond *second) {
    mtb_score_params sp; mtb_make_score_params(p, &sp);
    uint64_t *d_tcoff;
    STCHK(ensure(c, "tcoff", n_reads + 1, &d_tcoff));
    STCHK(taxcnt_layout(c, n_reads, first.seg, first.cursor ? first.cursor : (const uint32_t *)first.bound_by_buckets, lens, out, sp.dna_shift, d_tcoff, n_tc));
    const bool key64 = ix->tax.max_id < (1 << 22) && lens.max_len + 3 < (1u << 11);
    const uint32_t max_nb_first = (uint32_t)mtb_num_buckets((int32_t)lens.max_len, sp.dna_shift);
    const uint32_t max_nb_second = (uint32_t)mtb_num_buckets((int32_t)std::max(lens.max_len, first.max_len_deferred), sp.dna_shift);
    if (max_nb_second > 65535u) return fail(MTB_ERR_ARG, "read too long for mtb_result.n_taxcnt (16 bits): more than 65535 position buckets");
    ScoreSrc second_src;
    for (int pass = 0; pass < 2; pass++) {
        const uint32_t max_nb = pass ? max_nb_second : max_nb_first;
        const ScoreSrc *S = &first;
        if (pass == 1) {
            if (!second) break;
            bool go = false;
            const ScoreLaunch SL{d_tcoff, key64, sp, lens, out};
            STCHK((*second)(&second_src, &go, SL));
            if (!go) break;
            S = &second_src;
        }
        uint32_t grid = S->grid ? S->grid : (uint32_t)std::min<uint64_t>(n_reads, std::max<uint64_t>(256ull * 14, n_reads / 8));
        bool need_slab = S->max_seg > S->cap || max_nb > MTB_SCORE_BKT;
        uint32_t slab_n = need_slab ? std::max<uint32_t>(S->max_seg, 1) : 0;
        uint32_t slab_nb = need_slab ? max_nb : 0;
        uint64_t slab_bytes = need_slab ? score_slab_bytes(slab_n, slab_nb) : 0;
        uint8_t *d_slabs = nullptr;
        const bool dynamic = need_slab && !S->cursor;
        if (dynamic) grid = std::min<uint32_t>(grid, 256u * 14u);
        if (slab_bytes) {
            while ((uint64_t)grid * slab_bytes > (MTB_SLAB_POOL_MAX) && grid > 64) grid /= 2;
            STCHK(ensure(c, "slabs", (size_t)grid * slab_bytes, &d_slabs, BUF_FIXED));
        }
        unsigned long long *d_work = nullptr;
        if (dynamic) { d_work = scal<unsigned long long>(c, SC_SCORE_WORK) + pass; HIPCHK(hipMemsetAsync(d_work, 0, 8, c->stream)); }
#define MTB_LAUNCH_SCORE(SRT, K, CAPV, DYNV, SLOTV) hipLaunchKernelGGL((k_score<SRT, K, mtb_match, CAPV, DYNV, SLOTV>), dim3(grid), dim3(64), 0, c->stream, S->m, S->seg, n_reads, lens.d_ql, \
        lens.d_ql2, tax_view(ix), sp, (const uint64_t *)d_tcoff, out.d_res, out.d_tc_tax, out.d_tc_cnt, out.tc_cap, d_slabs, slab_bytes, slab_n, slab_nb, (mtb_match *)nullptr,  \
        out.tc_base, S->list, S->n_list, S->cursor, S->stride, S->seg_by_list, S->direct, S->epoch, S->big_list, S->n_big, S->cnt_out, d_work, S->only_flagged, S->seg_cnt)
        ScoreSrc S_rest;
        const bool pairs = p->seq_mode == 2;
        if (S->cursor && pass == 0 && key64 && S->stride <= 384u && !c->opt.no_fast_scorer && !(pairs && c->opt.no_fast_pairs)) {
            uint8_t *d_slow;
            STCHK(ensure(c, "slowflag", n_reads, &d_slow));
            HIPCHK(hipMemsetAsync(d_slow, 0, n_reads, c->stream));
            HIPCHK(scal_clear(c, SC_N_GENERIC));
#define MTB_LAUNCH_FAST(...) hipLaunchKernelGGL((k_score_fast<__VA_ARGS__>), dim3(grid), dim3(64), 0, c->stream, (const mtb_slot16 *)S->m, n_reads, lens.d_ql, lens.d_ql2, tax_view(ix), sp, \
            (const uint64_t *)d_tcoff, out.d_res, out.d_tc_tax, out.d_tc_cnt, out.tc_cap, out.tc_base, S->cursor, S->stride, S->direct, S->epoch, d_slow, S->cnt_out)
            { KTimer ktf(c, MTB_K_SCORE_FAST);
              if (pairs) { if (S->stride <= 192) MTB_LAUNCH_FAST(3, 3, true); else if (S->stride <= 256) MTB_LAUNCH_FAST(4, 4, true); else MTB_LAUNCH_FAST(5, 6, true); }
              else if (S->stride <= 128) MTB_LAUNCH_FAST(2); else if (S->stride <= 192) MTB_LAUNCH_FAST(3); else if (S->stride <= 256) MTB_LAUNCH_FAST(4); else MTB_LAUNCH_FAST(5, 6, false); }
#undef MTB_LAUNCH_FAST
            hipLaunchKernelGGL(k_count_flags, dim3(256), dim3(256), 0, c->stream, (const uint8_t *)d_slow, n_reads, scal<unsigned long long>(c, SC_N_GENERIC));
            if (S->big_list && S->n_big) hipLaunchKernelGGL(k_list_flag2, dim3((uint32_t)((n_reads + 255) / 256)), dim3(256), 0, c->stream, (const uint8_t *)d_slow, n_reads, S->big_list, S->n_big);
            c->fast_used = true;
            S_rest = *S; S_rest.only_flagged = d_slow;
            S = &S_rest;
        }
        KTimer kt(c, pass == 0 ? MTB_K_SCORE : MTB_K_SEGSORT);
        if (S->cursor) {
#define MTB_LAUNCH_SLOT(CAPV) do { if (key64) MTB_LAUNCH_SCORE(true, true, CAPV, false, true); else MTB_LAUNCH_SCORE(true, false, CAPV, false, true); } while (0)
            if (S->cap <= 144) MTB_LAUNCH_SLOT(144);
            else if (S->cap <= 160) MTB_LAUNCH_SLOT(160);
            else if (S->cap <= 224) MTB_LAUNCH_SLOT(224);
            else if (S->cap <= 288) MTB_LAUNCH_SLOT(288);
            else MTB_LAUNCH_SLOT(320);
#undef MTB_LAUNCH_SLOT
        } else if (dynamic) {
            if (!S->sort) MTB_LAUNCH_SCORE(false, false, MTB_SCORE_LDS, true, false);
            else if (key64) MTB_LAUNCH_SCORE(true, true, MTB_SCORE_LDS, true, false); else MTB_LAUNCH_SCORE(true, false, MTB_SCORE_LDS, true, false);
        }
        else if (S->sort) { if (key64) MTB_LAUNCH_SCORE(true, true, MTB_SCORE_LDS, false, false); else MTB_LAUNCH_SCORE(true, false, MTB_SCORE_LDS, false, false); }
        else if (S->cap >= 320) MTB_LAUNCH_SCORE(false, false, 320, false, false);
        else MTB_LAUNCH_SCORE(false, false, MTB_SCORE_LDS, false, false);
#undef MTB_LAUNCH_SCORE
    }
    HIPCHK(hipGetLastError());
    return MTB_OK;
}

struct LongSegs {
    const mtb_match *d_m = nullptr; const uint64_t *d_seg = nullptr; uint32_t max_seg = 0;
    const uint32_t *d_segcnt = nullptr, *d_list = nullptr; uint32_t n_list = 0;
};
static mtb_status dev_score_long(mtb_ctx *c, mtb_index *ix, const mtb_params *p, uint64_t n_reads, const ReadLens &lens, const ResultSink &out, uint64_t *n_tc, const LongSegs &sg) {
    mtb_score_params sp; mtb_make_score_params(p, &sp);
    uint64_t *d_tcoff; uint8_t *d_todo;
    STCHK(ensure(c, "tcoff", n_reads + 1, &d_tcoff)); STCHK(ensure(c, "slowflag", n_reads, &d_todo));
    if (!sg.d_list) {
        STCHK(taxcnt_layout(c, n_reads, sg.d_seg, sg.d_segcnt, lens, out, sp.dna_shift, d_tcoff, n_tc));
        const uint32_t max_nb = (uint32_t)mtb_num_buckets((int32_t)lens.max_len, sp.dna_shift);
        if (max_nb > 65535u) return fail(MTB_ERR_ARG, "read too long for mtb_result.n_taxcnt (16 bits): more than 65535 position buckets");
    }
    HIPCHK(hipMemsetAsync(d_todo, 0, n_reads, c->stream));
    unsigned long long *d_work = scal<unsigned long long>(c, SC_LONG_WORK);
    HIPCHK(hipMemsetAsync(d_work, 0, 8, c->stream));
    HIPCHK(scal_clear(c, SC_LONG_N_SECOND));
    {   KTimer kt(c, MTB_K_SCORE_FAST);
        const uint64_t n_it = sg.d_list ? sg.n_list : n_reads;
        hipLaunchKernelGGL((k_score_long<MTB_LONG_MAXBLK, MTB_LONG_MAXSP, 512, 2048>), dim3((uint32_t)std::min<uint64_t>(n_it, 256ull * 4)), dim3(MTB_LONG_NT), 0, c->stream, sg.d_m, sg.d_seg, n_reads, lens.d_ql, lens.d_ql2, tax_view(ix), sp, (const uint64_t *)d_tcoff,
                           out.d_res, out.d_tc_tax, out.d_tc_cnt, out.tc_cap, out.tc_base, d_todo, d_work, sg.d_segcnt, sg.d_list, sg.n_list, 0u);
        hipLaunchKernelGGL(k_count_flags, dim3(256), dim3(256), 0, c->stream, (const uint8_t *)d_todo, n_reads, scal<unsigned long long>(c, SC_LONG_N_SECOND));
        uint64_t n_second = 0;
        STCHK(d2h(c, &n_second, scal<uint64_t>(c, SC_LONG_N_SECOND), 8));
        HIPCHK(scal_clear(c, SC_N_GENERIC));
        if (n_second) {
            HIPCHK(hipMemsetAsync(d_work, 0, 8, c->stream));
            hipLaunchKernelGGL((k_score_long<MTB_LONG_MAXBLK, MTB_LONG_MAXSP>), dim3((uint32_t)std::min<uint64_t>(n_it, 256ull * 2)), dim3(MTB_LONG_NT), 0, c->stream, sg.d_m, sg.d_seg, n_reads, lens.d_ql, lens.d_ql2, tax_view(ix), sp, (const uint64_t *)d_tcoff,
                               out.d_res, out.d_tc_tax, out.d_tc_cnt, out.tc_cap, out.tc_base, d_todo, d_work, sg.d_segcnt, sg.d_list, sg.n_list, 1u);
        }
#ifdef MTB_LONG_PHASE_CYCLES
    {
        HIPCHK(hipStreamSynchronize(c->stream));
        unsigned long long h[16], z[16] = {0};
        HIPCHK(hipMemcpyFromSymbol(h, HIP_SYMBOL(mtb_long_cycles), sizeof(h)));
        HIPCHK(hipMemcpyToSymbol(HIP_SYMBOL(mtb_long_cycles), z, sizeof(z)));
        static const char *nm[10] = {"setup", "block list", "walk", "rank", "species ranges", "combination", "decision", "filter", "taxCnt gather", "descent + output + next read"};
        unsigned long long tot = 0; for (int k = 0; k < 10; k++) tot += h[k];
        fprintf(stderr, "k_score_long phases (%llu reads):", (unsigned long long)(sg.d_list ? sg.n_list : n_reads));
        for (int k = 0; k < 10; k++) fprintf(stderr, " %s %.1f %%;", nm[k], tot ? 100.0 * (double)h[k] / (double)tot : 0.0);
        fprintf(stderr, "\n");
    }
#endif
    }
    hipLaunchKernelGGL(k_count_flags, dim3(256), dim3(256), 0, c->stream, (const uint8_t *)d_todo, n_reads, scal<unsigned long long>(c, SC_N_GENERIC));
    HIPCHK(hipGetLastError());
    uint64_t n_left = 0;
    STCHK(d2h(c, &n_left, scal<uint64_t>(c, SC_N_GENERIC), 8));
    c->fast_used = true;
    if (n_left == 0) return MTB_OK;
    ScoreSrc a; a.m = sg.d_m; a.seg = sg.d_seg; a.sort = false; a.max_seg = std::max<uint32_t>(sg.max_seg, MTB_SCORE_LDS + 1); a.only_flagged = d_todo; a.seg_cnt = sg.d_segcnt;
    a.bound_by_buckets = sg.d_segcnt ? (const void *)sg.d_segcnt : (const void *)sg.d_list;
    uint32_t *d_nl = nullptr;
    if (sg.d_list) { STCHK(ensure(c, "lnlist", 2, &d_nl)); STCHK(h2d(c, d_nl, &sg.n_list, 4)); a.list = sg.d_list; a.n_list = d_nl; a.seg_by_list = 1; }
    uint64_t n_tc2 = 0;
    STCHK(dev_score(c, ix, p, n_reads, lens, out, &n_tc2, a,  nullptr));
    HIPCHK(scal_clear(c, SC_N_GENERIC));
// ... 944 lines not shown
    scan_launch<uint32_t, uint64_t, false>(c->stream, d_rc, n_reads, true, d_seg, d_ws);
    std::vector<uint32_t> rc(n_reads);
    STCHK(d2h(c, rc.data(), d_rc, n_reads * 4));
    uint32_t max_seg = 0, max_len = 0;
    for (uint64_t i = 0; i < n_reads; i++) { max_seg = std::max(max_seg, rc[i]); max_len = std::max<uint32_t>(max_len, (uint32_t)(qlen[i] + (qlen2 ? qlen2[i] : 0))); }
    mtb_result *d_res; int32_t *d_tt; uint32_t *d_tc;
    STCHK(ensure(c, res_name(RES_ROWS, 0), n_reads, &d_res, BUF_IO)); STCHK(ensure(c, "tctax", taxcnt_cap, &d_tt, BUF_IO)); STCHK(ensure(c, "tccnt", taxcnt_cap, &d_tc, BUF_IO));
    ScoreSrc src; src.m = d_m; src.seg = d_seg; src.sort = false; src.max_seg = max_seg;
    const ReadLens lens{d_ql, d_ql2, max_len};
    const ResultSink out{d_res, d_tt, d_tc, taxcnt_cap,  0};
    mtb_status st = (p->seq_mode == 3 && !c->opt.no_long_scorer)
        ? dev_score_long(c, ix, p, n_reads, lens, out, n_taxcnt, LongSegs{d_m, d_seg, max_seg})
        : dev_score(c, ix, p, n_reads, lens, out, n_taxcnt, src,  nullptr);
    if (st != MTB_OK) return st;
    STCHK(d2h(c, results, d_res, n_reads * sizeof(mtb_result)));
    if (*n_taxcnt) { STCHK(d2h(c, taxcnt_tax, d_tt, *n_taxcnt * 4)); STCHK(d2h(c, taxcnt_cnt, d_tc, *n_taxcnt * 4)); }
    return MTB_OK;
}

}

static mtb_status score_join_order(mtb_ctx *c, mtb_index *ix, const mtb_params *p, mtb_match *d_tmp, uint64_t nm, uint64_t n_reads, uint32_t *d_rc,
                                   const ReadLens &lens, const ResultSink &out, uint64_t *n_taxcnt) {
    hipStream_t st = c->stream; mtb_match *d_m; uint64_t *d_seg;
    STCHK(ensure(c, "matches", nm, &d_m));
    STCHK(dev_regroup(c, d_tmp, nm, n_reads, d_rc, &d_seg, d_m));
    HIPCHK(hipEventRecord(c->ev[4], st));
    const bool long_scorer = p->seq_mode == 3 && !c->opt.no_long_scorer;
    uint32_t max_seg = 0;
    {
        uint32_t *d_large;
        STCHK(ensure(c, "large", n_reads, &d_large));
        HIPCHK(scal_clear(c, SC_N_LARGE, 2));
        { KTimer kt(c, MTB_K_SEGSORT);
        hipLaunchKernelGGL(k_list_large, dim3((uint32_t)((n_reads + 255) / 256)), dim3(256), 0, st, (const uint64_t *)d_seg, n_reads,
                           long_scorer ? 1u : (uint32_t)MTB_SCORE_LDS, d_large, scal<uint32_t>(c, SC_N_LARGE), scal<uint32_t>(c, SC_MAX_SEG)); }
        uint64_t sc[2];
        STCHK(d2h(c, sc, scal<uint64_t>(c, SC_N_LARGE), 16));
        max_seg = (uint32_t)sc[1];
        if (sc[0]) {
            const size_t lds = (size_t)MTB_SEGLDS_CHUNK * 14;
            HIPCHK(hipFuncSetAttribute((const void *)k_segsort_lds<mtb_match>, hipFuncAttributeMaxDynamicSharedMemorySize, (int)lds));
            KTimer kt(c, MTB_K_SEGSORT);
            hipLaunchKernelGGL((k_segsort_lds<mtb_match>), dim3(std::min<uint32_t>((uint32_t)sc[0], 2048)), dim3(MTB_SEGLDS_THREADS), lds, st, d_m,
                               (const uint64_t *)d_seg, (const uint32_t *)d_large, scal<const uint32_t>(c, SC_N_LARGE), d_tmp);
        }
    }
    HIPCHK(hipEventRecord(c->ev[5], st));
    if (long_scorer) return dev_score_long(c, ix, p, n_reads, lens, out, n_taxcnt, LongSegs{d_m, d_seg, max_seg});
    ScoreSrc a; a.m = d_m; a.seg = d_seg; a.sort = true; a.max_seg = max_seg;
    return dev_score(c, ix, p, n_reads, lens, out, n_taxcnt, a,  nullptr);
}

static void slot_geometry(const mtb_ctx *c, uint32_t max_q, uint32_t *direct, uint32_t *stride) {
    const uint32_t tail_min = c->opt.tail_min > 0 ? (uint32_t)std::max(8, c->opt.tail_min) & ~7u : 16u;
    *direct = std::max<uint32_t>(8, (max_q + 7) & ~7u);
    *stride = *direct + std::max<uint32_t>(tail_min, (*direct / 8 + 7) & ~7u);
}
struct SlotSegs {
    mtb_slot16 *d_segm = nullptr; uint32_t *d_rc = nullptr, stride = 0, direct = 0, epoch = 0;
    mtb_match *d_ovf = nullptr; uint64_t n_ovf = 0, ovf_region = 0;
    const uint8_t *d_off_reads = nullptr; uint32_t max_len_off = 0;
};
static mtb_status make_slots(mtb_ctx *c, uint64_t n_reads, uint32_t max_q, uint32_t *d_rc, SlotSegs *sl) {
    hipStream_t st = c->stream; *sl = SlotSegs(); sl->d_rc = d_rc;
    slot_geometry(c, max_q, &sl->direct, &sl->stride);
    STCHK(ensure_placed(c, "segm", n_reads * (uint64_t)sl->stride, &sl->d_segm));
    const DevBuf sb = buf_get(c, "segm");
    const char *clear_mode = c->opt.segm_clear[0] ? c->opt.segm_clear : nullptr;
    const bool always = clear_mode && !strcmp(clear_mode, "always");
    if (sb.p != c->seg_clean_p || sb.cap != c->seg_clean_cap || c->seg_epoch == 0 || c->seg_epoch >= MTB_SLOT_EPOCHS || always) {
        if (clear_mode && !strcmp(clear_mode, "kernel")) hipLaunchKernelGGL(k_clear_words, dim3(2048), dim3(256), 0, st, (uint64_t *)sb.p, (uint64_t)(sb.cap / 8));
        else HIPCHK(hipMemsetAsync(sb.p, 0, sb.cap, st));
        if (clear_mode && !strcmp(clear_mode, "sync")) HIPCHK(hipDeviceSynchronize());
        c->seg_epoch = 0; c->seg_clean_p = sb.p; c->seg_clean_cap = sb.cap;
    }
    sl->epoch = ++c->seg_epoch;
    return MTB_OK;
}
static uint64_t ovf_cap_first(mtb_ctx *c, uint64_t n_items) { return std::max<uint64_t>(buf_cap(c, "ovf") / sizeof(mtb_match), n_items / 64 + 4096); }
static uint64_t ovf_cap_regrown(uint64_t n) { return n + n / 16 + 1024; }

static mtb_status score_fixed_slots(mtb_ctx *c, mtb_index *ix, const mtb_params *p, uint64_t n_reads, const ReadLens &lens, uint64_t nk_real, const SlotSegs &sl,
                                    const ResultSink &out, uint64_t *n_taxcnt, uint64_t *nm_out) {
    hipStream_t st = c->stream;
    uint64_t nm = 0;
    memset(c->many_stats, 0, sizeof(c->many_stats));
    uint32_t *d_biglist, *d_bigcnt, *d_bigidx, *d_bigcur, *d_cnt; uint64_t *d_bigstart = nullptr, *d_ws2, *d_tot; mtb_match *d_big = nullptr;
    STCHK(ensure(c, "biglist", n_reads, &d_biglist)); STCHK(ensure(c, "bigidx", n_reads, &d_bigidx)); STCHK(ensure(c, "livecnt", n_reads, &d_cnt));
    STCHK(ensure(c, "segstart", n_reads + 1, &d_tot)); STCHK(ensure(c, "scanws", scan_ws_elems(n_reads + 1), &d_ws2));
    HIPCHK(hipMemsetAsync(d_cnt, 0, n_reads * 4, st));
    HIPCHK(scal_clear(c, SC_N_UNGROUPED, 3));
    uint64_t big_total = 0;
    ScoreSrc a; a.m = (const mtb_match *)sl.d_segm; a.cursor = sl.d_rc;        a.stride = sl.stride; a.direct = sl.direct; a.epoch = sl.epoch; a.sort = true; a.max_len_deferred = sl.max_len_off;
    {
        const uint32_t want = std::min<uint32_t>(sl.direct, (uint32_t)((double)nk_real / (double)n_reads * 1.12) + 1);
        a.cap = want <= 144 ? 144 : want <= 160 ? 160 : want <= 224 ? 224 : want <= 288 ? 288 : 320;
    }
    a.max_seg = a.cap;
    a.big_list = d_biglist; a.n_big = scal<uint32_t>(c, SC_N_DEFERRED); a.cnt_out = d_cnt;
    ScoreSecond second = [&](ScoreSrc *b, bool *go, const ScoreLaunch &SL) -> mtb_status {
        uint64_t sc = 0;
        STCHK(d2h(c, &sc, scal<uint64_t>(c, SC_N_DEFERRED), 8));
        uint32_t n_big = (uint32_t)sc;
        *go = n_big != 0;
        if (!n_big) return MTB_OK;
        c->many_stats[0] = n_big; c->many_stats[1] = 0;
        const bool no_many = c->opt.no_score_many != 0;
        uint32_t *d_novf = nullptr; uint64_t *d_ostart = nullptr; mtb_match *d_ovfg = nullptr;
        if (!no_many && sl.stride <= 384u) {
            KTimer ktm(c, MTB_K_SCORE_MANY);
            uint32_t *d_ocur = nullptr, *d_rest;
            STCHK(ensure(c, "restlist", n_reads, &d_rest));
            const bool have_ovf = sl.ovf_region ? c->ovf_max_region != 0 : sl.n_ovf != 0;
            if (have_ovf) {
                STCHK(ensure(c, "novf", n_reads, &d_novf)); STCHK(ensure(c, "ocur", n_reads, &d_ocur)); STCHK(ensure(c, "ovfstart", n_reads + 1, &d_ostart));
                STCHK(scratch(c, "ovfg", sl.n_ovf + 1, &d_ovfg));
                HIPCHK(hipMemsetAsync(d_ocur, 0, n_reads * 4, st));
                hipLaunchKernelGGL(k_ovf_count, dim3((uint32_t)((n_reads + 255) / 256)), dim3(256), 0, st, (const uint32_t *)sl.d_rc, sl.d_off_reads, n_reads, sl.stride - sl.direct, d_novf);
                scan_launch<uint32_t, uint64_t, false>(st, d_novf, n_reads, true, d_ostart, d_ws2);
                if (sl.ovf_region) hipLaunchKernelGGL(k_ovf_group, dim3((uint32_t)((c->ovf_max_region + 255) / 256), MTB_OVF_STRIPES), dim3(256), 0, st, (const mtb_match *)sl.d_ovf, sl.n_ovf,
                                                   (const uint64_t *)d_ostart, (const uint32_t *)d_novf, d_ocur, d_ovfg, sl.ovf_region, (const unsigned long long *)c->d_ovfctr);
                else hipLaunchKernelGGL(k_ovf_group, dim3((uint32_t)((sl.n_ovf + 255) / 256)), dim3(256), 0, st, (const mtb_match *)sl.d_ovf, sl.n_ovf,
                                        (const uint64_t *)d_ostart, (const uint32_t *)d_novf, d_ocur, d_ovfg, (uint64_t)0, (const unsigned long long *)nullptr);
            }
            unsigned long long *d_ms;
            STCHK(ensure(c, "manystat", 16, &d_ms));
            HIPCHK(hipMemsetAsync(d_ms, 0, 16 * 8, st));
            const bool cap192 = c->opt.many_cap ? c->opt.many_cap <= 192 : sl.stride <= 192u;
            const uint32_t gridm = std::min<uint32_t>(n_big, 256u * (cap192 ? 12u : 7u));
#define MTB_LAUNCH_MANY(K64, CAPV) hipLaunchKernelGGL((k_score_many<K64, CAPV>), dim3(gridm), dim3(64), 0, st, (const mtb_slot16 *)sl.d_segm, sl.stride, sl.direct, sl.epoch, (const uint32_t *)sl.d_rc, sl.d_off_reads, \
            (const mtb_match *)d_ovfg, (const uint64_t *)d_ostart, (const uint32_t *)d_biglist, scal<const uint32_t>(c, SC_N_DEFERRED), SL.lens.d_ql, SL.lens.d_ql2, tax_view(ix), SL.sp, SL.d_tcoff, SL.out.d_res, \
            SL.out.d_tc_tax, SL.out.d_tc_cnt, SL.out.tc_cap, SL.out.tc_base, d_rest, (uint32_t *)d_ms, d_cnt, d_ms + 1, d_ms + 2)
            if (cap192) { if (SL.key64) MTB_LAUNCH_MANY(true, 192); else MTB_LAUNCH_MANY(false, 192); }
            else { if (SL.key64) MTB_LAUNCH_MANY(true, 320); else MTB_LAUNCH_MANY(false, 320); }
#undef MTB_LAUNCH_MANY
            HIPCHK(hipGetLastError());
            uint64_t ms4[8] = {0, 0, 0, 0, 0, 0, 0, 0};
            STCHK(d2h(c, ms4, d_ms, 64));
            const uint32_t n_rest = (uint32_t)(ms4[0] & 0xFFFFFFFFull);
            c->many_stats[1] = n_big - n_rest; c->many_stats[2] = ms4[2]; c->many_stats[3] = ms4[3];
            if (c->opt.many_verbose) fprintf(stderr, "mtb: k_score_many: %u reads listed, %u handed on (routed off / buckets / counts %llu, species table full %llu, survivors beyond the staging %llu); %llu matches, %llu survive the dead-species drop\n",
                                                    n_big, n_rest, (unsigned long long)ms4[4], (unsigned long long)ms4[5], (unsigned long long)ms4[6], (unsigned long long)ms4[2], (unsigned long long)ms4[3]);
            n_big = n_rest;
            const unsigned long long *d_nleft = d_ms;
            if (n_big && SL.key64 && !c->opt.no_many_sort) {
                uint32_t *d_bc3, *d_segcnt, *d_rest2; uint64_t *d_bs3; uint8_t *d_todo; mtb_match *d_big3;
                STCHK(ensure(c, "bigcnt", n_big, &d_bc3)); STCHK(ensure(c, "bigstart", (uint64_t)n_big + 1, &d_bs3)); STCHK(ensure(c, "bigseg", n_big, &d_segcnt));
                STCHK(ensure(c, "restlist2", n_reads, &d_rest2)); STCHK(ensure(c, "todoflag", n_reads, &d_todo));
                hipLaunchKernelGGL(k_big_count, dim3(std::min<uint32_t>(n_big, 4096)), dim3(64), 0, st, (const mtb_slot16 *)sl.d_segm, sl.stride, sl.direct, sl.epoch,
                                   (const uint32_t *)sl.d_rc, (const uint32_t *)d_rest, n_big, d_bc3, d_bigidx, scal<uint32_t>(c, SC_MAX_BIG_SEG), sl.d_off_reads);
                scan_launch<uint32_t, uint64_t, false>(st, d_bc3, n_big, true, d_bs3, d_ws2);
                uint64_t total3 = 0;
                STCHK(d2h(c, &total3, d_bs3 + n_big, 8));
                STCHK(scratch(c, "manym", total3 + 1, &d_big3));
                HIPCHK(hipMemsetAsync(d_todo, 0, n_reads, st));
                hipLaunchKernelGGL((k_many_sort<11, 2048u>), dim3(std::min<uint32_t>(n_big, 256u * 8u)), dim3(MTB_MSORT_NT), 0, st, (const mtb_slot16 *)sl.d_segm, sl.stride, sl.direct, sl.epoch, (const uint32_t *)sl.d_rc, sl.d_off_reads,
                                   (const mtb_match *)d_ovfg, (const uint64_t *)d_ostart, (const uint32_t *)d_rest, n_big, SL.lens.d_ql, SL.lens.d_ql2, SL.sp.dna_shift, (const uint64_t *)d_bs3, d_big3, d_segcnt, d_todo, 0u, 2u);
                hipLaunchKernelGGL((k_many_sort<12, 4096u>), dim3(std::min<uint32_t>(n_big, 256u * 3u)), dim3(MTB_MSORT_NT), 0, st, (const mtb_slot16 *)sl.d_segm, sl.stride, sl.direct, sl.epoch, (const uint32_t *)sl.d_rc, sl.d_off_reads,
                                   (const mtb_match *)d_ovfg, (const uint64_t *)d_ostart, (const uint32_t *)d_rest, n_big, SL.lens.d_ql, SL.lens.d_ql2, SL.sp.dna_shift, (const uint64_t *)d_bs3, d_big3, d_segcnt, d_todo, 2u, 1u);
                hipLaunchKernelGGL((k_score_long<2048, 256, 256, 256>), dim3(std::min<uint32_t>(n_big, 256u * 5u)), dim3(MTB_LONG_NT), 0, st, (const mtb_match *)d_big3, (const uint64_t *)d_bs3, n_reads, SL.lens.d_ql, SL.lens.d_ql2,
                                   tax_view(ix), SL.sp, SL.d_tcoff, SL.out.d_res, SL.out.d_tc_tax, SL.out.d_tc_cnt, SL.out.tc_cap, SL.out.tc_base, d_todo, d_ms + 8, (const uint32_t *)d_segcnt, (const uint32_t *)d_rest, n_big);
                hipLaunchKernelGGL(k_list_flagged, dim3((n_big + 255) / 256), dim3(256), 0, st, (const uint32_t *)d_rest, n_big, (const uint8_t *)d_todo, (const uint32_t *)d_bc3, d_rest2, (uint32_t *)(d_ms + 9), d_cnt);
                HIPCHK(hipGetLastError());
                uint64_t left = 0;
                STCHK(d2h(c, &left, d_ms + 9, 8));
                if (c->opt.many_verbose) fprintf(stderr, "mtb: k_many_sort + k_score_long: %u reads (%llu records), %llu left for the exact-segment path\n", n_big, (unsigned long long)total3, (unsigned long long)(left & 0xFFFFFFFFull));
                n_big = (uint32_t)(left & 0xFFFFFFFFull);
                d_rest = d_rest2; d_nleft = d_ms + 9;
            }
            c->many_stats[1] = c->many_stats[0] - n_big;
            *go = n_big != 0;
            if (!n_big) return MTB_OK;
            d_biglist = d_rest;
            HIPCHK(hipMemcpyAsync(scal<uint64_t>(c, SC_N_DEFERRED), d_nleft, 8, hipMemcpyDeviceToDevice, st));
        }
        KTimer kt(c, MTB_K_SEGSORT);
        HIPCHK(hipMemsetAsync(d_bigidx, 0xFF, n_reads * 4, st));
        STCHK(ensure(c, "bigcnt", n_big, &d_bigcnt)); STCHK(ensure(c, "bigstart", (uint64_t)n_big + 1, &d_bigstart)); STCHK(ensure(c, "bigcur", n_big, &d_bigcur));
        hipLaunchKernelGGL(k_big_count, dim3(std::min<uint32_t>(n_big, 4096)), dim3(64), 0, st, (const mtb_slot16 *)sl.d_segm, sl.stride, sl.direct, sl.epoch,
                           (const uint32_t *)sl.d_rc, (const uint32_t *)d_biglist, n_big, d_bigcnt, d_bigidx, scal<uint32_t>(c, SC_MAX_BIG_SEG), sl.d_off_reads,
                           (const uint32_t *)(d_ovfg ? d_novf : nullptr), scal<unsigned long long>(c, SC_N_UNGROUPED));
        scan_launch<uint32_t, uint64_t, false>(st, d_bigcnt, n_big, true, d_bigstart, d_ws2);
        uint64_t mx = 0, n_ungrouped = 0;
        STCHK(d2h(c, &big_total, d_bigstart + n_big, 8));
        STCHK(d2h(c, &mx, scal<uint64_t>(c, SC_MAX_BIG_SEG), 8));
        STCHK(d2h(c, &n_ungrouped, scal<uint64_t>(c, SC_N_UNGROUPED), 8));
        STCHK(scratch(c, "bigm", big_total, &d_big));
        hipLaunchKernelGGL(k_big_copy, dim3(std::min<uint32_t>(n_big, 4096)), dim3(64), 0, st, (const mtb_slot16 *)sl.d_segm, sl.stride, sl.direct, sl.epoch,
                           (const uint32_t *)sl.d_rc, (const uint32_t *)d_biglist, (const uint64_t *)d_bigstart, n_big, d_bigcur, d_big,
                           (const mtb_match *)d_ovfg, (const uint64_t *)d_ostart, (const uint32_t *)(d_ovfg ? d_novf : nullptr));
        const uint32_t *skip_grouped = d_ovfg ? d_novf : nullptr;
        if (d_ovfg && n_ungrouped == 0) {  }
        else if (sl.ovf_region) {
            if (c->ovf_max_region) hipLaunchKernelGGL(k_big_ovf, dim3((uint32_t)((c->ovf_max_region + 255) / 256), MTB_OVF_STRIPES), dim3(256), 0, st, (const mtb_match *)sl.d_ovf, sl.n_ovf,
                                                      (const uint32_t *)d_bigidx, (const uint64_t *)d_bigstart, d_bigcur, d_big, sl.ovf_region, (const unsigned long long *)c->d_ovfctr, skip_grouped);
        } else
        if (sl.n_ovf) hipLaunchKernelGGL(k_big_ovf, dim3((uint32_t)((sl.n_ovf + 255) / 256)), dim3(256), 0, st, (const mtb_match *)sl.d_ovf, sl.n_ovf,
                                      (const uint32_t *)d_bigidx, (const uint64_t *)d_bigstart, d_bigcur, d_big, (uint64_t)0, (const unsigned long long *)nullptr, skip_grouped);
        uint32_t *d_lg;
        STCHK(ensure(c, "large", n_big, &d_lg));
        HIPCHK(scal_clear(c, SC_DEFER_N_LARGE));
        hipLaunchKernelGGL(k_segsort_small, dim3(std::min<uint32_t>(n_big, 256u * 40u)), dim3(64), 0, st, d_big, (const uint64_t *)d_bigstart, (uint64_t)n_big, d_lg,
                           scal<uint32_t>(c, SC_DEFER_N_LARGE), (uint32_t *)nullptr);
        hipLaunchKernelGGL((k_segsort_large<mtb_match>), dim3(std::min<uint32_t>(n_big, 1024)), dim3(256), 0, st, d_big, (const uint64_t *)d_bigstart,
                           (const uint32_t *)d_lg, scal<const uint32_t>(c, SC_DEFER_N_LARGE));
        HIPCHK(hipGetLastError());
        b->m = d_big; b->seg = d_bigstart; b->list = d_biglist; b->n_list = scal<const uint32_t>(c, SC_N_DEFERRED); b->seg_by_list = 1;
        b->sort = false; b->max_seg = (uint32_t)mx; b->grid = std::min<uint32_t>(n_big, 256u * 14u); b->cap = 320;
        return MTB_OK;
    };
    STCHK(dev_score(c, ix, p, n_reads, lens, out, n_taxcnt, a, &second));
    { KTimer kt(c, MTB_K_SCAN); scan_launch<uint32_t, uint64_t, false>(st, d_cnt, n_reads, true, d_tot, d_ws2); }
    STCHK(d2h(c, &nm, d_tot + n_reads, 8));
    nm += big_total;
    *nm_out = nm;
    return MTB_OK;
}

static mtb_status download_packed(mtb_ctx *c, mtb_result *d_res, const int32_t *d_tt, const uint32_t *d_tc, uint64_t n_reads, mtb_result *results,
                                  int32_t *taxcnt_tax, uint32_t *taxcnt_cnt, uint64_t *n_taxcnt, uint64_t host_cap = ~0ull, int async_set = -1 ) {
    uint32_t *d_n; uint64_t *d_off, *d_ws; int32_t *d_tt2; uint32_t *d_tc2;
    STCHK(ensure(c, "tcn", n_reads, &d_n)); STCHK(ensure(c, "tcnewoff", n_reads + 1, &d_off)); STCHK(ensure(c, "scanws", scan_ws_elems(n_reads + 1), &d_ws));
    hipLaunchKernelGGL(k_taxcnt_n, dim3((uint32_t)((n_reads + 255) / 256)), dim3(256), 0, c->stream, (const mtb_result *)d_res, n_reads, d_n);
    scan_launch<uint32_t, uint64_t, false>(c->stream, d_n, n_reads, true, d_off, d_ws);
    uint64_t total = 0;
    STCHK(d2h(c, &total, d_off + n_reads, 8));
    if (total > host_cap) { *n_taxcnt = total; return fail(MTB_ERR_CAPACITY, "taxcnt arrays too small for the batch's taxID:count lists"); }
    STCHK(ensure(c, res_name(RES_TAX, async_set == 1), total, &d_tt2)); STCHK(ensure(c, res_name(RES_CNT, async_set == 1), total, &d_tc2));
    hipLaunchKernelGGL(k_taxcnt_pack, dim3((uint32_t)((n_reads + 255) / 256)), dim3(256), 0, c->stream, d_res, n_reads, (const uint64_t *)d_off, d_tt, d_tc, d_tt2, d_tc2);
    HIPCHK(hipGetLastError());
    if (async_set >= 0) {
        HIPCHK(hipEventRecord(c->down_ready, c->stream));
        HIPCHK(hipStreamWaitEvent(c->down_stream, c->down_ready, 0));
        HIPCHK(hipMemcpyAsync(results, d_res, n_reads * sizeof(mtb_result), hipMemcpyDeviceToHost, c->down_stream));
        if (total) { HIPCHK(hipMemcpyAsync(taxcnt_tax, d_tt2, total * 4, hipMemcpyDeviceToHost, c->down_stream)); HIPCHK(hipMemcpyAsync(taxcnt_cnt, d_tc2, total * 4, hipMemcpyDeviceToHost, c->down_stream)); }
        HIPCHK(hipEventRecord(c->down_done, c->down_stream));
        c->down_pending = true;
        *n_taxcnt = total;
        return MTB_OK;
    }
    STCHK(d2h(c, results, d_res, n_reads * sizeof(mtb_result)));
    if (total) { STCHK(d2h(c, taxcnt_tax, d_tt2, total * 4)); STCHK(d2h(c, taxcnt_cnt, d_tc2, total * 4)); }
    *n_taxcnt = total;
    return MTB_OK;
}

static uint64_t cov_bitmap_words(const mtb_index *ix) { return std::max<uint64_t>((ix->T + 31) / 32, 1); }
static uint64_t cov_bin_words(const mtb_index *ix) { return (uint64_t)ix->tax.max_id + 1 + MTB_COV_EXTRA; }
static dim3 cov_grid(uint64_t n, uint64_t per_block, uint64_t most) { return dim3((uint32_t)std::max<uint64_t>(1, std::min<uint64_t>((n + per_block - 1) / per_block, most))); }
struct CovCall {
    mtb_ctx *c = nullptr; mtb_index *ix = nullptr;
    mtb_status begin(mtb_ctx *c_, mtb_index *ix_) {
        if (!ix_->d_cov_bits || c_->cov_call) return MTB_OK;
        const uint64_t words = cov_bin_words(ix_);
        if (c_->cov_pend_words < words) {
            if (c_->d_cov_pend) { hipError_t e = hipFree(c_->d_cov_pend); (void)e; c_->d_cov_pend = nullptr; c_->cov_pend_words = 0; }
            if (hipMalloc((void **)&c_->d_cov_pend, words * 8) != hipSuccess) { c_->d_cov_pend = nullptr; (void)hipGetLastError(); return fail(MTB_ERR_OOM, "no HBM for the pending coverage bins"); }
            c_->cov_pend_words = words;
        }
        HIPCHK(hipMemsetAsync(c_->d_cov_pend, 0, words * 8, c_->stream));
        HIPCHK(hipStreamSynchronize(c_->stream));
        for (mtb_ctx *l : c_->lanes) { l->d_cov_pend = c_->d_cov_pend; l->cov_pend_words = c_->cov_pend_words; }
        c = c_; ix = ix_; c->cov_call = true;
        return MTB_OK;
    }
    mtb_status end(mtb_status st) {
        if (!c) return st;
        mtb_ctx *cc = c; c = nullptr; cc->cov_call = false;
        if (st != MTB_OK) return st;
        const uint64_t words = cov_bin_words(ix);
        hipLaunchKernelGGL(k_cov_commit, cov_grid(words, 256, ~0u), dim3(256), 0, cc->stream, ix->d_cov_hits, cc->d_cov_pend, words, (uint64_t)ix->tax.max_id + 1 + MTB_COV_N_BATCHES, 1u);
        HIPCHK(hipGetLastError());
        HIPCHK(hipStreamSynchronize(cc->stream));
        return MTB_OK;
    }
    ~CovCall() { if (c) c->cov_call = false; }
};
static mtb_status dev_cov_mark(mtb_ctx *c, mtb_index *ix, const mtb_kmer *d_q, uint64_t n, const mtb_result *d_res, uint64_t n_reads, uint32_t *d_rs, IndexUse *use) {
    if (!c->d_cov_pend || c->cov_pend_words < cov_bin_words(ix)) return fail(MTB_ERR_ARG, "k-mer coverage: no classify call is open on this context");
    if (n_reads == 0 || n == 0) return MTB_OK;
    hipStream_t st = c->stream;
    hipLaunchKernelGGL(k_cov_read_species, cov_grid(n_reads, 256, ~0u), dim3(256), 0, st, d_res, n_reads, (const int32_t *)ix->d_tax2species, ix->tax.max_id, d_rs);
    HIPCHK(hipGetLastError());
    bool packed = false;
    use->hold(ix, &packed);
    const mtb_index_view v = index_view(ix); const mtb_dir_view dv = dir_view(ix);
    const dim3 grid = cov_grid(n, 256, 1u << 14);
    if (packed) hipLaunchKernelGGL((k_cov_mark<true, true>), grid, dim3(256), 0, st, d_q, n, (const uint32_t *)d_rs, n_reads, v, dv, ix->d_cov_bits, c->d_cov_pend);
    else if (ix->d_dir) hipLaunchKernelGGL((k_cov_mark<false, true>), grid, dim3(256), 0, st, d_q, n, (const uint32_t *)d_rs, n_reads, v, dv, ix->d_cov_bits, c->d_cov_pend);
    else hipLaunchKernelGGL((k_cov_mark<false, false>), grid, dim3(256), 0, st, d_q, n, (const uint32_t *)d_rs, n_reads, v, dv, ix->d_cov_bits, c->d_cov_pend);
    HIPCHK(hipGetLastError());
    return MTB_OK;
}

// ... 257 lines not shown
    bool lslot = p->seq_mode == 3 && ix->d_dir && long_slots && !c->opt.no_long_slots;
    const bool aa6 = p->kmer_format == 2;
    ExtractOpts xo; xo.single_pass = true; xo.tag_ordinals = fixed || lslot; xo.want_digits = aa6;
    if (lslot) { STCHK(ensure(c, "dcnt", n_reads, &xo.d_counts)); HIPCHK(hipMemsetAsync(xo.d_counts, 0, n_reads * 4, st)); }
    if (fixed && ix->d_dir) STCHK(ensure(c, "offreads", n_reads, &xo.d_off_reads));
    Extracted ex; STCHK(dev_extract(c, p, rd, d_ql, d_ql2, xo, &ex));
    ReadLens lens{d_ql, d_ql2, ex.max_len};
    uint32_t max_q = ex.max_q; const uint32_t max_len_all = ex.max_len; bool route_off = false;
    if (fixed && xo.d_off_reads && ex.off_reads > 0 && ex.off_reads * 4 <= n_reads && ex.max_len + 3 < 65536u && max_q < 65535u && ex.off_reads < n_reads) {
        route_off = true;
        max_q = (uint32_t)ex.off_max_q; lens.max_len = (uint32_t)ex.off_max_len;
    }
    if ((fixed && !route_off && (lens.max_len + 3 >= MTB_SLOT_MAX_POS || max_q > MTB_SLOT_MAX_Q)) || (lslot && (lens.max_len + 3 >= 65536u || max_q >= 65535u))) {
        fixed = false; lslot = false;
        ExtractOpts untagged; untagged.single_pass = true; untagged.want_digits = aa6;
        STCHK(dev_extract(c, p, rd, d_ql, d_ql2, untagged, &ex));
        lens.max_len = ex.max_len; max_q = ex.max_q;
    }
    HIPCHK(hipEventRecord(c->ev[1], st));
    int aa_first_shift = 34;
    if (aa6 && fixed && ix->d_dir && c->opt.sort_pairs > 0) aa_first_shift = 64 - 10 * std::max(1, std::min(3, c->opt.sort_pairs));
    mtb_kmer *d_s; uint32_t *d_rc;
    STCHK(dev_sort(c, ex.d_k, ex.nk, aa6 ? MTB_SORT_AA6 : 32, &d_s, aa_first_shift == 34 ? ex.d_dig : nullptr, aa_first_shift));
    HIPCHK(hipEventRecord(c->ev[2], st));
    SortedQueries q; q.d_s = d_s; q.nk = ex.nk; q.low_bits = aa6 ? aa_first_shift : 32; q.max_q = max_q; q.d_counts = xo.d_counts;
    c->last_sorted = (fixed && ix->d_dir) ? d_s : nullptr; c->last_sorted_n = ex.nk;
    STCHK(ensure(c, "readcnt", n_reads, &d_rc));
    HIPCHK(hipMemsetAsync(d_rc, 0, n_reads * 4, st));
    uint64_t nm = 0;
    if (fixed) {
        SlotSegs sl;
        STCHK(make_slots(c, n_reads, max_q, d_rc, &sl));
        if (route_off) { sl.d_off_reads = xo.d_off_reads; sl.max_len_off = max_len_all; }
        uint64_t ovf_cap = ovf_cap_first(c, q.nk);
        for (int attempt = 0; attempt < 3; attempt++) {
            STCHK(ensure(c, "ovf", ovf_cap, &sl.d_ovf));
            JoinSegArgs sa; memset(&sa, 0, sizeof(sa));
            sa.seg = sl.d_segm; sa.stride = sl.stride; sa.direct = sl.direct; sa.cursor = d_rc; sa.ovf = sl.d_ovf; sa.ovf_cap = ovf_cap;
            sa.ovf_counter = nullptr; sa.epoch = sl.epoch; sa.off = sl.d_off_reads;
            sa.dense_ovf = attempt == 2 ? 1u : 0u;
            sa.retry = attempt > 0 ? 1u : 0u;
            mtb_status s2 = dev_join(c, ix, q.d_s, q.nk, MatchList(), &sl.n_ovf, &sa, q.low_bits);
            if (s2 == MTB_OK) break;
            if (s2 != MTB_ERR_CAPACITY || attempt == 2) return s2;
            ovf_cap = ovf_cap_regrown(sl.n_ovf);
            HIPCHK(hipMemsetAsync(d_rc, 0, n_reads * 4, st));
        }
        sl.ovf_region = c->ovf_region;
        for (int k = 3; k <= 5; k++) HIPCHK(hipEventRecord(c->ev[k], st));
        set_dead_segments(c, d_s);
        struct DeadEnd { mtb_ctx *c; ~DeadEnd() { c->n_dead = 0; } } dead_end{c};
        STCHK(score_fixed_slots(c, ix, p, n_reads, lens, ex.nk_real, sl, out, n_taxcnt, &nm));
    } else if (lslot) {
        bool done = false;
        STCHK(score_long_slots(c, ix, p, n_reads, lens, q, out, n_taxcnt, &nm, &done));
        if (!done) { *redo_exact = true; return MTB_OK; }
    } else {
        MatchList ml; ml.d_read_cnt = d_rc;
        ml.cap = std::max<uint64_t>(buf_cap(c, "jtemp") / sizeof(mtb_match), q.nk + q.nk / 2 + 1024);
        for (int attempt = 0; attempt < 3; attempt++) {
            STCHK(ensure(c, "jtemp", ml.cap, &ml.d_out));
            mtb_status s2 = dev_join(c, ix, q.d_s, q.nk, ml, &nm,  nullptr, q.low_bits);
            if (s2 == MTB_OK) break;
            if (s2 != MTB_ERR_CAPACITY || attempt == 2) return s2;
            ml.cap = nm + nm / 16 + 1024;
            HIPCHK(hipMemsetAsync(d_rc, 0, n_reads * 4, st));
        }
        HIPCHK(hipEventRecord(c->ev[3], st));
        STCHK(score_join_order(c, ix, p, ml.d_out, nm, n_reads, d_rc, lens, out, n_taxcnt));
    }
    IndexUse cov_use;
    if (d_cov_rs) STCHK(dev_cov_mark(c, ix, d_s, ex.nk, out.d_res, n_reads, d_cov_rs, &cov_use));
    HIPCHK(hipEventRecord(c->ev[6], st));
    HIPCHK(hipEventSynchronize(c->ev[6]));
    cov_use.release();
    mtb_batch_stats &S = c->stats;
    float *const stage_ms[6] = {&S.ms_extract, &S.ms_sort, &S.ms_join, &S.ms_regroup, &S.ms_segsort, &S.ms_score};
    for (int k = 0; k < 6; k++) HIPCHK(hipEventElapsedTime(stage_ms[k], c->ev[k], c->ev[k + 1]));
    HIPCHK(hipEventElapsedTime(&S.ms_total, c->ev[0], c->ev[6]));
    collect_kernel_times(c);
    S.n_reads = n_reads; S.n_bases = ex.n_bases; S.n_kmers = ex.nk_real; S.n_matches = nm; S.n_targets = ix->T;
    STCHK(take_generic_reads(c, n_reads, &S.n_generic_reads));
    S.n_slot_reads = (fixed || lslot) ? n_reads : 0;
    if (fixed) { S.n_deferred_reads = c->many_stats[0]; S.n_many_reads = c->many_stats[1]; S.n_many_matches = c->many_stats[2]; S.n_many_kept = c->many_stats[3]; }
    return MTB_OK;
}
static mtb_status classify_one(mtb_ctx *c, mtb_index *ix, const mtb_params *p, const Reads &rd, const ResultSink &out, uint64_t *n_taxcnt) {
    bool redo_exact = false;
    STCHK(classify_attempt(c, ix, p, rd, out, n_taxcnt,  true, &redo_exact));
    return redo_exact ? classify_attempt(c, ix, p, rd, out, n_taxcnt,  false, &redo_exact) : MTB_OK;
}

static void merge_stats(mtb_batch_stats &S, const mtb_batch_stats &L) {
    S.ms_extract += L.ms_extract; S.ms_sort += L.ms_sort; S.ms_join += L.ms_join; S.ms_regroup += L.ms_regroup;
    S.ms_segsort += L.ms_segsort; S.ms_score += L.ms_score;
    S.n_reads += L.n_reads; S.n_bases += L.n_bases; S.n_kmers += L.n_kmers; S.n_matches += L.n_matches; S.n_targets = L.n_targets;
    S.n_generic_reads += L.n_generic_reads; S.n_slot_reads += L.n_slot_reads;
    S.n_deferred_reads += L.n_deferred_reads; S.n_many_reads += L.n_many_reads; S.n_many_matches += L.n_many_matches; S.n_many_kept += L.n_many_kept;
    for (int i = 0; i < MTB_NUM_KERNELS; i++) { S.ms_kernel[i] += L.ms_kernel[i]; S.n_launch[i] += L.n_launch[i]; }
    S.join_variant = L.join_variant; S.join_tuned = L.join_tuned;
    for (int v = 0; v < 3; v++) S.join_tune_ms[v] = L.join_tune_ms[v];
    S.join_tiles += L.join_tiles; S.join_tiles_windowed += L.join_tiles_windowed; S.join_tiles_outside += L.join_tiles_outside;
    S.lslot_tail_factor = L.lslot_tail_factor; S.n_lslot_big_reads += L.n_lslot_big_reads;
}

static mtb_status classify_budgeted(mtb_ctx *c, mtb_index *ix, const mtb_params *p, const Reads &rd, uint64_t n_bases_total, const ResultSink &out, uint64_t *n_taxcnt) {
    const uint64_t n_reads = rd.n_reads, taxcnt_cap = out.tc_cap;
    HIPCHK(hipSetDevice(c->device));
    *n_taxcnt = 0;
    c->last_sub_batches = 0; c->last_scratch_bytes = 0;
    if (n_reads == 0) { memset(&c->stats, 0, sizeof(c->stats)); return MTB_OK; }
    if (c->ws_seq_mode != p->seq_mode) {
        if (c->ws_seq_mode) { HIPCHK(hipStreamSynchronize(c->stream)); release_workspace(c); }
        c->ws_seq_mode = p->seq_mode;
    }
    size_t fr = 0, tot = 0;
    HIPCHK(hipMemGetInfo(&fr, &tot));
    const size_t held = held_bytes(c, BUF_FIXED);
    uint64_t budget = c->ws_limit ? c->ws_limit : (uint64_t)fr + held;
    if (!c->ws_limit) budget -= std::min<uint64_t>(budget / 16, 4ull << 30);
    if (p->seq_mode == 3 && !c->ws_limit) budget -= std::min<uint64_t>(budget / 4, MTB_SLAB_POOL_MAX);
    const double mean_len = (double)n_bases_total / (double)n_reads;
    double per_base = c->ws_per_base;
    if (per_base <= 0.0) {
        const double yield = (c->extract_yield > 0.0 ? c->extract_yield : (p->syncmer ? 1.0 : 2.0)) * 1.15;
        per_base = yield * (16 + 16 + 2 + 2) + (p->seq_mode == 3 ? yield * 1.5 * 48 : yield * 1.2 * 16 + 24.0 * 16 / std::max(mean_len, 1.0)) + 100.0 / std::max(mean_len, 1.0);
    }
    const double safety = c->ws_per_base > 0.0 ? 1.02 : 1.08;
    uint64_t fit = (uint64_t)((double)budget / (per_base * safety * mean_len));
    fit = std::max<uint64_t>(fit, 1);
    uint64_t n_sub = (n_reads + fit - 1) / fit;
    if (c->opt.host_timing)
        fprintf(stderr, "mtb budget: free %.1f GiB + held %.1f GiB -> budget %.1f GiB; %.1f bytes per base (%s) x %.2f -> %llu reads fit, %llu sub-batch(es) for %llu reads\n",
                (double)fr / 1073741824.0, (double)held / 1073741824.0, (double)budget / 1073741824.0, per_base, c->ws_per_base > 0.0 ? "measured" : "estimate", safety,
                (unsigned long long)fit, (unsigned long long)n_sub, (unsigned long long)n_reads);
    mtb_batch_stats S; memset(&S, 0, sizeof(S));
    uint64_t tc_used = 0, lo = 0;
    uint32_t done = 0;
    while (lo < n_reads) {
        const uint64_t left_sub = std::max<uint64_t>(1, n_sub > done ? n_sub - done : 1);
        uint64_t cnt = (n_reads - lo + left_sub - 1) / left_sub;
        uint64_t n_tc = 0;
        mtb_status st;
        for (;;) {
            st = classify_one(c, ix, p, rd.range(lo, cnt),
                              ResultSink{out.d_res + lo, out.d_tc_tax + tc_used, out.d_tc_cnt + tc_used, taxcnt_cap - std::min(taxcnt_cap, tc_used), out.tc_base + tc_used}, &n_tc);
            if (st != MTB_ERR_OOM || cnt <= 1024) break;
            HIPCHK(hipStreamSynchronize(c->stream));
            if (c->opt.host_timing) fprintf(stderr, "mtb budget: %llu reads ran out of memory (%s); halving\n", (unsigned long long)cnt, mtb_last_error());
            release_workspace(c);
            cnt = (cnt + 1) / 2; n_sub *= 2; done *= 2;
        }
        if (st == MTB_ERR_CAPACITY) {
            const uint64_t rest = n_reads - lo - cnt;
            *n_taxcnt = std::max<uint64_t>(taxcnt_cap + 1, tc_used + n_tc + (uint64_t)((double)n_tc / (double)cnt * (double)rest * 1.05) + 64);
            return st;
        }
        if (st != MTB_OK) return st;
        c->ws_max_sub_bases = std::max<uint64_t>(c->ws_max_sub_bases, c->stats.n_bases);
        if (c->ws_max_sub_bases) c->ws_per_base = (double)held_bytes(c, BUF_WORK) / (double)c->ws_max_sub_bases;
        if (c->opt.host_timing) {
            std::lock_guard<std::mutex> lk(c->bufs_mu);
            fprintf(stderr, "mtb budget: sub-batch of %llu reads (%llu bases) done; buffers (GiB):", (unsigned long long)cnt, (unsigned long long)c->stats.n_bases);
            for (auto &kv : c->bufs) if (kv.second.cap >= (256u << 20)) fprintf(stderr, " %s %.2f", kv.first.c_str(), (double)kv.second.cap / 1073741824.0);
            fprintf(stderr, "\n");
        }
        merge_stats(S, c->stats); S.ms_total += c->stats.ms_total;
        tc_used += n_tc; lo += cnt; done++;
    }
    c->stats = S;
    c->last_sub_batches = done;
    *n_taxcnt = tc_used;
    return MTB_OK;
}

extern "C" {

static mtb_status classify_batch_device_impl(mtb_ctx *c, mtb_index *ix, const mtb_params *p, const char *d_bases, const uint64_t *d_offs,
                                             const char *d_bases2, const uint64_t *d_offs2, uint64_t n_reads, uint64_t n_bases_total,
                                             mtb_result *d_results, int32_t *d_taxcnt_tax, uint32_t *d_taxcnt_cnt, uint64_t taxcnt_cap,
                                             uint64_t *n_taxcnt) {
    const size_t L = c->lanes.size();
    if (L < 2 || n_reads < 4096 * L)
        return classify_budgeted(c, ix, p, Reads{d_bases, d_offs, d_bases2, d_offs2, n_reads}, n_bases_total, ResultSink{d_results, d_taxcnt_tax, d_taxcnt_cnt, taxcnt_cap,  0}, n_taxcnt);
    HIPCHK(hipSetDevice(c->device));
    HIPCHK(hipStreamSynchronize(c->stream));
// ... 321 lines not shown
    if (part_starts && p->seq_mode != 3 && !c->opt.part_exact) {
        const bool aa6 = p->kmer_format == 2;
        ExtractOpts tagged; tagged.single_pass = true; tagged.tag_ordinals = true; tagged.want_digits = aa6;
        STCHK(dev_extract(c, p, rd, d_ql, d_ql2, tagged, &ex));
        const uint64_t nk = ex.nk;
        if (ex.max_len + 3 < MTB_SLOT_MAX_POS && ex.max_q <= 384) {
            const int low_bits = aa6 ? 34 : 32;
            STCHK(dev_sort(c, ex.d_k, ex.nk, aa6 ? MTB_SORT_AA6 : 32, &d_s, ex.d_dig,  34));
            c->part_max_len = ex.max_len; c->part_mode = 1; c->part_max_q = ex.max_q; c->part_nk_real = ex.nk_real;
            std::vector<uint64_t> key(2 * n_parts), pos(2 * n_parts);
            for (uint32_t q = 0; q < n_parts; q++) {
                const uint64_t pre = bounds[q] >> low_bits;
                key[2 * q] = pre << low_bits;
                key[2 * q + 1] = pre + 1 >= (1ull << (64 - low_bits)) ? UINT64_MAX : (pre + 1) << low_bits;
            }
            if (nk) STCHK(lower_bounds(c, (const uint64_t *)d_s, nk, 2, key.data(), 2 * n_parts, pos.data()));
            for (uint32_t q = 0; q < n_parts; q++) {
                const uint64_t lo = q == 0 ? 0 : pos[2 * q];
                const uint64_t hi = q + 1 < n_parts ? (key[2 * (q + 1) + 1] == UINT64_MAX ? nk : pos[2 * (q + 1) + 1]) : nk;
                part_starts[q] = lo; part_counts[q] = hi > lo ? hi - lo : 0;
            }
            *d_sorted = d_s; *n_kmers = nk;
            return MTB_OK;
        }
    }
    STCHK(dev_extract(c, p, rd, d_ql, d_ql2,  ExtractOpts(), &ex));
    const uint64_t nk = ex.nk;
    STCHK(dev_sort(c, ex.d_k, ex.nk, 24, &d_s,  nullptr, 0));
    c->part_max_len = ex.max_len;
    std::vector<uint64_t> pos(n_parts);
    if (nk) STCHK(lower_bounds(c, (const uint64_t *)d_s, nk, 2, bounds, n_parts, pos.data()));
    for (uint32_t q = 0; q < n_parts; q++) { uint64_t hi = q + 1 < n_parts ? pos[q + 1] : nk; part_counts[q] = hi >= pos[q] ? hi - pos[q] : 0; if (part_starts) part_starts[q] = pos[q]; }
    if (nk && pos[0] != 0) return fail(MTB_ERR_ARG, "bounds[0] must be 0");
    *d_sorted = d_s; *n_kmers = nk;
    return MTB_OK;
}

mtb_status mtb_part_join(mtb_ctx *c, mtb_index *ix, const mtb_kmer *d_kmers, uint64_t n, mtb_match *d_out, uint64_t cap, uint64_t *count) {
    if (!c || !ix || !count) return fail(MTB_ERR_ARG, "NULL argument");
    HIPCHK(hipSetDevice(c->device));
    *count = 0;
    if (n == 0 || ix->T == 0) return MTB_OK;
    if (ix->d_dir && !c->opt.part_exact) {
        JoinSegArgs sa; memset(&sa, 0, sizeof(sa));
        sa.list = 1; sa.ovf = d_out; sa.ovf_cap = cap;
        return dev_join(c, ix, d_kmers, n, MatchList(), count, &sa,  32);
    }
    return dev_join(c, ix, d_kmers, n, MatchList{d_out, cap}, count,  nullptr, ix->params.kmer_format == 2 ? 34 : 32);
}

mtb_status mtb_part_score(mtb_ctx *c, mtb_index *ix, const mtb_params *p, mtb_match *d_matches, uint64_t n_matches, uint64_t n_reads,
                          mtb_result *results, int32_t *taxcnt_tax, uint32_t *taxcnt_cnt, uint64_t taxcnt_cap, uint64_t *n_taxcnt) {
    if (!c || !ix || !p || !results || !n_taxcnt) return fail(MTB_ERR_ARG, "NULL argument");
    if (n_reads != c->part_n_reads) return fail(MTB_ERR_ARG, "mtb_part_score must follow mtb_part_extract of the same batch on the same context");
    HIPCHK(hipSetDevice(c->device));
    *n_taxcnt = 0;
    if (n_reads == 0) return MTB_OK;
    if (n_matches >= (1ull << 32)) return fail(MTB_ERR_ARG, "more than 2^32-1 matches in one batch; split the batch");
    int32_t *d_ql, *d_ql2; uint32_t *d_rc; mtb_result *d_res; int32_t *d_tt; uint32_t *d_tc;
    STCHK(ensure(c, "qlen", n_reads, &d_ql)); STCHK(ensure(c, "qlen2", n_reads, &d_ql2));
    STCHK(ensure(c, "readcnt", n_reads, &d_rc));
    STCHK(ensure(c, res_name(RES_ROWS, 0), n_reads, &d_res, BUF_IO)); STCHK(ensure(c, "tctax", taxcnt_cap, &d_tt, BUF_IO)); STCHK(ensure(c, "tccnt", taxcnt_cap, &d_tc, BUF_IO));
    const ResultSink sink{d_res, d_tt, d_tc, taxcnt_cap,  0};
    if (c->part_mode == 1) {
        hipStream_t st = c->stream; SlotSegs sl;
        STCHK(make_slots(c, n_reads, c->part_max_q, d_rc, &sl));
        uint64_t ovf_cap = ovf_cap_first(c, n_matches);
        for (int attempt = 0; attempt < 3; attempt++) {
            STCHK(ensure(c, "ovf", ovf_cap, &sl.d_ovf));
            HIPCHK(hipMemsetAsync(d_rc, 0, n_reads * 4, st));
            HIPCHK(scal_clear(c, SC_JOIN_COUNT, 2));
            JoinSegArgs sa; memset(&sa, 0, sizeof(sa));
            sa.seg = sl.d_segm; sa.stride = sl.stride; sa.direct = sl.direct; sa.cursor = d_rc; sa.ovf = sl.d_ovf; sa.ovf_cap = ovf_cap; sa.ovf_counter = scal<unsigned long long>(c, SC_JOIN_COUNT); sa.epoch = sl.epoch;
            if (n_matches) hipLaunchKernelGGL(k_slot_place, dim3((uint32_t)((n_matches + 255) / 256)), dim3(256), 0, st, (const mtb_match *)d_matches, n_matches, sa, n_reads, scal<uint32_t>(c, SC_BAD_SEQ));
            HIPCHK(hipGetLastError());
            uint64_t sc[2]; STCHK(d2h(c, sc, scal<uint64_t>(c, SC_JOIN_COUNT), 16));
            if (sc[1] & 0xFFFFFFFFull) return fail(MTB_ERR_ARG, "match records with a sequenceID outside 1..n_reads");
            sl.n_ovf = sc[0];
            if (sl.n_ovf <= ovf_cap) break;
            if (attempt == 2) return fail(MTB_ERR_CAPACITY, "overflow list too small");
            ovf_cap = ovf_cap_regrown(sl.n_ovf);
        }
        uint64_t nm = 0; memset(&c->stats, 0, sizeof(c->stats));
        STCHK(score_fixed_slots(c, ix, p, n_reads, ReadLens{d_ql, d_ql2, c->part_max_len}, c->part_nk_real, sl, sink, n_taxcnt, &nm));
        c->stats.n_reads = n_reads; c->stats.n_matches = nm; c->stats.n_slot_reads = n_reads; c->stats.n_kmers = c->part_nk_real;
        STCHK(take_generic_reads(c,  0, &c->stats.n_generic_reads));
        return download_packed(c, d_res, d_tt, d_tc, n_reads, results, taxcnt_tax, taxcnt_cnt, n_taxcnt);
    }
    STCHK(count_reads(c, d_matches, n_matches, n_reads, d_rc));
    STCHK(score_join_order(c, ix, p, d_matches, n_matches, n_reads, d_rc, ReadLens{d_ql, d_ql2, c->part_max_len}, sink, n_taxcnt));
    return download_packed(c, d_res, d_tt, d_tc, n_reads, results, taxcnt_tax, taxcnt_cnt, n_taxcnt);
}

static mtb_status run_parallel_status(uint32_t n, const std::function<mtb_status(uint32_t)> &f, std::string *err) {
    std::vector<mtb_status> st(n, MTB_OK); std::vector<std::string> errs(n);
    std::vector<std::thread> th;
    for (uint32_t k = 0; k < n; k++) th.emplace_back([&, k] { st[k] = f(k); if (st[k] != MTB_OK) errs[k] = g_err; });
    for (auto &t : th) t.join();
    for (uint32_t k = 0; k < n; k++) if (st[k] != MTB_OK) { *err = errs[k]; return st[k]; }
    return MTB_OK;
}

mtb_status mtb_classify_batch_partitioned(mtb_ctx **ctxs, mtb_index **parts, uint32_t n, const uint64_t *bounds, const mtb_params *p,
                                          const char *bases, const uint64_t *offs, const char *bases2, const uint64_t *offs2, uint64_t n_reads,
                                          mtb_result *results, int32_t *taxcnt_tax, uint32_t *taxcnt_cnt, uint64_t taxcnt_cap, uint64_t *n_taxcnt) {
    if (!ctxs || !parts || !bounds || !p || !n_taxcnt || n == 0) return fail(MTB_ERR_ARG, "NULL argument");
    *n_taxcnt = 0;
    if (n_reads == 0) return MTB_OK;
    if (!bases || !offs || !results) return fail(MTB_ERR_ARG, "NULL argument");
    const bool paired = p->seq_mode == 2;
    if (paired && (!bases2 || !offs2)) return fail(MTB_ERR_ARG, "seq_mode 2 needs bases2/offs2");
    struct Rank {
        uint64_t lo = 0, hi = 0;
        const mtb_kmer *d_sorted = nullptr; uint64_t nk = 0;
        std::vector<uint64_t> counts, starts;
        std::vector<uint64_t> m_count, m_start;
        mtb_match *d_matches = nullptr;
        std::vector<mtb_result> res; std::vector<int32_t> tt; std::vector<uint32_t> tc; uint64_t ntc = 0;
    };
    for (uint32_t i = 0; i < n; i++) for (uint32_t j = 0; j < n; j++) {
        if (!ctxs[i] || !ctxs[j] || ctxs[i]->device == ctxs[j]->device) continue;
        int can = 0;
        if (hipDeviceCanAccessPeer(&can, ctxs[i]->device, ctxs[j]->device) != hipSuccess) { (void)hipGetLastError(); continue; }
        if (!can) continue;
        if (hipSetDevice(ctxs[i]->device) != hipSuccess) { (void)hipGetLastError(); continue; }
        const hipError_t e = hipDeviceEnablePeerAccess(ctxs[j]->device, 0);
        if (e != hipSuccess) (void)hipGetLastError();
    }
    std::vector<Rank> R(n);
    for (uint32_t k = 0; k < n; k++) { R[k].lo = n_reads * k / n; R[k].hi = n_reads * (k + 1) / n; R[k].counts.assign(n, 0); R[k].starts.assign(n, 0); R[k].m_count.assign(n, 0); R[k].m_start.assign(n, 0); }
    std::string err;
    mtb_status st = run_parallel_status(n, [&](uint32_t k) -> mtb_status {
        mtb_ctx *c = ctxs[k]; Rank &r = R[k];
        const uint64_t m = r.hi - r.lo;
        if (m == 0) return MTB_OK;
        HIPCHK(hipSetDevice(c->device));
        std::vector<uint64_t> o(m + 1), o2(paired ? m + 1 : 0);
        for (uint64_t i = 0; i <= m; i++) o[i] = offs[r.lo + i] - offs[r.lo];
        if (paired) for (uint64_t i = 0; i <= m; i++) o2[i] = offs2[r.lo + i] - offs2[r.lo];
        char *d_b, *d_b2; uint64_t *d_o, *d_o2; uint64_t nb;
        STCHK(upload_reads(c, p, bases + offs[r.lo], o.data(), paired ? bases2 + offs2[r.lo] : nullptr, paired ? o2.data() : nullptr, m, &d_b, &d_o, &d_b2, &d_o2, &nb));
        return mtb_part_extract(c, p, d_b, d_o, d_b2, d_o2, m, bounds, n, &r.d_sorted, &r.nk, r.counts.data(), r.starts.data());
    }, &err);
    if (st != MTB_OK) return fail(st, err);
    st = run_parallel_status(n, [&](uint32_t q) -> mtb_status {
        mtb_ctx *c = ctxs[q]; Rank &own = R[q];
        HIPCHK(hipSetDevice(c->device));
        uint64_t n_in = 0;
        for (uint32_t k = 0; k < n; k++) n_in += R[k].counts[q];
        if (n_in == 0) return MTB_OK;
        mtb_kmer *d_in;
        STCHK(ensure(c, "xkmers", n_in, &d_in));
        uint64_t at = 0;
        for (uint32_t k = 0; k < n; k++) {
            const uint64_t cnt = R[k].counts[q];
            if (cnt) HIPCHK(hipMemcpyPeerAsync(d_in + at, c->device, R[k].d_sorted + R[k].starts[q], ctxs[k]->device, cnt * sizeof(mtb_kmer), c->stream));
            at += cnt;
        }
        HIPCHK(hipStreamSynchronize(c->stream));
        uint64_t cap = n_in + n_in / 4 + 1024;
        for (int attempt = 0; attempt < 4; attempt++) {
            STCHK(ensure(c, "xmatches", cap, &own.d_matches));
            uint64_t used = 0, need = 0; bool again = false;
            at = 0;
            for (uint32_t k = 0; k < n && !again; k++) {
                const uint64_t cnt = R[k].counts[q];
                uint64_t got = 0;
// ... 1304 lines not shown
```

Before: 72.12.

## Overlap scoring of overflowed reads on a side stream with the fast scorer

Adds a side stream and events per context. Reads whose slot cursor overflowed the tail capacity are listed up front by a new kernel, then grouped, sorted and scored by the many/long kernels on the side stream while the fast scorer runs on the main stream. The fast scorer now skips overflowed reads immediately instead of loading their slots. This aims to hide the serial many-tier path and its host round-trips behind fast scoring, at the cost of extra buffers, cross-stream synchronisation and more complex error handling.

```diff
diff --git a/include/mtb.h b/include/mtb.h
--- a/include/mtb.h
+++ b/include/mtb.h
@@ -76,6 +76,7 @@
     float    join_tune_ms[3];
     uint32_t join_tiles, join_tiles_windowed, join_tiles_outside;
     uint32_t lslot_tail_factor, n_lslot_big_reads;
+    uint32_t score_overlapped;
 } mtb_batch_stats;
 
 typedef enum { MTB_JOIN_AUTO = 0, MTB_JOIN_Q1W6 = 1, MTB_JOIN_Q2W5 = 2, MTB_JOIN_WINDOW = 3 } mtb_join_variant;
diff --git a/metabuli_amd/__init__.py b/metabuli_amd/__init__.py
--- a/metabuli_amd/__init__.py
+++ b/metabuli_amd/__init__.py
@@ -37,7 +37,7 @@
                 ("n_deferred_reads", C.c_uint64), ("n_many_reads", C.c_uint64), ("n_many_matches", C.c_uint64), ("n_many_kept", C.c_uint64),
                 ("join_variant", C.c_int32), ("join_tuned", C.c_int32), ("join_tune_ms", C.c_float * 3),
                 ("join_tiles", C.c_uint32), ("join_tiles_windowed", C.c_uint32), ("join_tiles_outside", C.c_uint32),
-                ("lslot_tail_factor", C.c_uint32), ("n_lslot_big_reads", C.c_uint32)]
+                ("lslot_tail_factor", C.c_uint32), ("n_lslot_big_reads", C.c_uint32), ("score_overlapped", C.c_uint32)]
 
 
 SHARE_BYTES = 4 * 64 + 4 * 8 + 8 + 2 * 4 + 5 * 4 + 4 + 8 + 4 * 8
diff --git a/metabuli_amd/csrc/kernels_score.h b/metabuli_amd/csrc/kernels_score.h
--- a/metabuli_amd/csrc/kernels_score.h
+++ b/metabuli_amd/csrc/kernels_score.h
@@ -56,6 +56,23 @@
     __shared__ uint32_t s_w[4]; __shared__ uint32_t s_base;
     const uint64_t r = (uint64_t)blockIdx.x * 256 + threadIdx.x;
     const bool on = r < n && f[r] == 2;
+    const uint64_t m = __ballot(on);
+    const uint32_t wv = threadIdx.x >> 6, lane = threadIdx.x & 63u;
+    if (lane == 0) s_w[wv] = (uint32_t)__popcll(m);
+    __syncthreads();
+    if (threadIdx.x == 0) { const uint32_t tot = s_w[0] + s_w[1] + s_w[2] + s_w[3]; s_base = tot ? atomicAdd(n_list, tot) : 0u; }
+    __syncthreads();
+    if (on) {
+        uint32_t at = s_base + (uint32_t)__popcll(m & ((1ull << lane) - 1ull));
+        for (uint32_t q = 0; q < wv; q++) at += s_w[q];
+        list[at] = (uint32_t)r;
+    }
+}
+
+__global__ __launch_bounds__(256) void k_list_overflowed(const uint32_t *__restrict__ cursor, uint64_t n, uint32_t tail_cap, uint32_t *__restrict__ list, uint32_t *__restrict__ n_list) {
+    __shared__ uint32_t s_w[4]; __shared__ uint32_t s_base;
+    const uint64_t r = (uint64_t)blockIdx.x * 256 + threadIdx.x;
+    const bool on = r < n && cursor[r] > tail_cap;
     const uint64_t m = __ballot(on);
     const uint32_t wv = threadIdx.x >> 6, lane = threadIdx.x & 63u;
     if (lane == 0) s_w[wv] = (uint32_t)__popcll(m);
diff --git a/metabuli_amd/csrc/kernels_score_fast.h b/metabuli_amd/csrc/kernels_score_fast.h
--- a/metabuli_amd/csrc/kernels_score_fast.h
+++ b/metabuli_amd/csrc/kernels_score_fast.h
@@ -84,11 +84,12 @@
         const int32_t read_len = ql1 + ql2;
         const int32_t nb = mtb_num_buckets(read_len, sp.dna_shift);
         const uint32_t cur = cursor[r];
+        if (cur > tail_cap) { MTB_FAST_COUNT(0, 1); if (lane == 0) slow_flag[r] = 2; continue; }
         const mtb_slot16 *slots = slots_all + r * (uint64_t)stride;
         mtb_slot16 x[KL];
 #pragma unroll
         for (int k = 0; k < KL; k++) { const uint32_t i = (uint32_t)lane + 64u * k; x[k].a = 0; x[k].b = 0; if (i < stride) x[k] = slots[i]; }
-        bool slow = cur > tail_cap || nb > MTB_FAST_BKT;
+        bool slow = nb > MTB_FAST_BKT;
         wave_fence();
         MTB_FAST_MARK(0);
         int32_t n = 0, n_live = 0;
@@ -227,7 +228,7 @@
         const int32_t nslot = (n + 63) >> 6;
         bool bad = false, bad2 = false;
 #ifdef MTB_FAST_DEBUG
-        if (slow) MTB_FAST_COUNT(cur > tail_cap || nb > MTB_FAST_BKT ? 0 : 1, 1);
+        if (slow) MTB_FAST_COUNT(nb > MTB_FAST_BKT ? 0 : 1, 1);
 #endif
 #pragma unroll
         for (int k = 0; k < K; k++) {
@@ -270,7 +271,7 @@
         if (!slow) { if (__any(bad)) MTB_FAST_COUNT(2, 1); else if (__any(bad2)) MTB_FAST_COUNT(3, 1); }
 #endif
         slow = slow || __any(bad || bad2);
-        if (slow) { if (lane == 0) slow_flag[r] = cur > tail_cap ? 2 : 1; continue; }
+        if (slow) { if (lane == 0) slow_flag[r] = 1; continue; }
         if (lane == 0) cnt_out[r] = (uint32_t)n_live;
         MTB_FAST_MARK(2);
         float ps[K]; int32_t phd[K]; int32_t root[K];
diff --git a/metabuli_amd/csrc/mtb_api.hip b/metabuli_amd/csrc/mtb_api.hip
--- a/metabuli_amd/csrc/mtb_api.hip
+++ b/metabuli_amd/csrc/mtb_api.hip
@@ -96,6 +96,12 @@
 #define MTB_SLAB_POOL_MAX (16ull << 30)
 #define MTB_LONG_WIN_MAX_PER_Q 24.0
 #define MTB_OVF_STRIPES 256u
+#ifndef MTB_SCORE_OVERLAP
+#define MTB_SCORE_OVERLAP 1
+#endif
+#ifndef MTB_SCORE_OVERLAP_GRID
+#define MTB_SCORE_OVERLAP_GRID 4u
+#endif
 
 enum Scal : uint32_t {
     SC_JOIN_COUNT = 0, SC_JOIN_OVERFLOW = 1,
@@ -154,6 +160,8 @@
     uint64_t prefetch_issued = 0, prefetch_used = 0;
     hipStream_t down_stream = nullptr; hipEvent_t down_ready = nullptr, down_done = nullptr; bool down_pending = false; int res_set = 0;
     int pk_set = 0;
+    hipStream_t side_stream = nullptr; hipEvent_t side_ev[3] = {nullptr, nullptr, nullptr};
+    uint32_t score_overlapped = 0;
     struct Prefetched { const void *key = nullptr, *key2 = nullptr; uint64_t n_reads = 0; bool valid = false; } pre[2];
     struct JoinTune { uint64_t key = 0; int calls = 0, pending = -1, best = -1; float ms[3] = {0.0f, 0.0f, 0.0f}; hipEvent_t e0 = nullptr, e1 = nullptr; } join_tunes[4]; uint32_t join_tune_next = 0;
     uint64_t many_stats[4] = {0, 0, 0, 0};
@@ -370,6 +378,16 @@
     p->min_score = 0.0f; p->min_sp_score = 0.0f; p->tie_ratio = 0.95f; p->accession_level = 0; p->skip_redundancy = 0;
 }
 
+static hipError_t make_side_stream(mtb_ctx *c) {
+    hipError_t e = hipStreamCreateWithFlags(&c->side_stream, hipStreamNonBlocking);
+    if (e != hipSuccess) { c->side_stream = nullptr; return e; }
+    for (int k = 0; k < 3 && e == hipSuccess; k++) { e = hipEventCreateWithFlags(&c->side_ev[k], hipEventDisableTiming); if (e != hipSuccess) c->side_ev[k] = nullptr; }
+    if (e != hipSuccess) {
+        for (int k = 0; k < 3; k++) if (c->side_ev[k]) { hipError_t e2 = hipEventDestroy(c->side_ev[k]); (void)e2; c->side_ev[k] = nullptr; }
+        hipError_t e2 = hipStreamDestroy(c->side_stream); (void)e2; c->side_stream = nullptr;
+    }
+    return e;
+}
 mtb_status mtb_ctx_create(int device, void *stream, mtb_ctx **out) {
     if (!out) return fail(MTB_ERR_ARG, "out is NULL");
     int n = 0;
@@ -379,6 +397,8 @@
     HIPCHK(hipSetDevice(device));
     mtb_ctx *c = new mtb_ctx();
     c->device = device; c->stream = (hipStream_t)stream;
+    {   const hipError_t es = make_side_stream(c);
+        if (es != hipSuccess) { delete c; return fail(MTB_ERR_DEVICE, std::string("side stream of the score stage: ") + hipGetErrorString(es)); } }
     mtb_build_tables(&c->h_tabs);
     HIPCHK(hipMalloc((void **)&c->d_tabs, sizeof(mtb_tables)));
     HIPCHK(hipMemcpy(c->d_tabs, &c->h_tabs, sizeof(mtb_tables), hipMemcpyHostToDevice));
@@ -406,6 +426,8 @@
     if (c->down_ready) e = hipEventDestroy(c->down_ready);
     if (c->down_done) e = hipEventDestroy(c->down_done);
     if (c->copy_stream) { e = hipStreamSynchronize(c->copy_stream); e = hipStreamDestroy(c->copy_stream); }
+    if (c->side_stream) { e = hipStreamSynchronize(c->side_stream); e = hipStreamDestroy(c->side_stream); }
+    for (int k = 0; k < 3; k++) if (c->side_ev[k]) e = hipEventDestroy(c->side_ev[k]);
     for (int k = 0; k < 2; k++) { if (c->copy_done[k]) e = hipEventDestroy(c->copy_done[k]); if (c->unpacked[k]) e = hipEventDestroy(c->unpacked[k]); }
     for (int q = 0; q < 4; q++) if (c->join_tunes[q].e0) { e = hipEventDestroy(c->join_tunes[q].e0); e = hipEventDestroy(c->join_tunes[q].e1); }
     for (int i = 0; i < 8; i++) e = hipEventDestroy(c->ev[i]);
@@ -453,6 +475,7 @@
         mtb_ctx *l = new mtb_ctx();
         l->device = c->device; l->is_lane = true; l->d_tabs = c->d_tabs; l->h_tabs = c->h_tabs; l->profiling = c->profiling; l->placement_probe = c->placement_probe; l->opt = c->opt;
         HIPCHK(hipStreamCreateWithFlags(&l->stream, hipStreamNonBlocking));
+        HIPCHK(make_side_stream(l));
         HIPCHK(hipMalloc((void **)&l->d_scal, SC_WORDS * sizeof(uint64_t)));
         HIPCHK(hipMalloc((void **)&l->d_ovfctr, MTB_OVF_STRIPES * 64));
         for (int i = 0; i < 8; i++) HIPCHK(hipEventCreate(&l->ev[i]));
@@ -464,11 +487,12 @@
 
 }
 
-static mtb_status d2h(mtb_ctx *c, void *dst, const void *src, size_t bytes) {
-    HIPCHK(hipMemcpyAsync(dst, src, bytes, hipMemcpyDeviceToHost, c->stream));
-    HIPCHK(hipStreamSynchronize(c->stream));
-    return MTB_OK;
-}
+static mtb_status d2h(mtb_ctx *c, void *dst, const void *src, size_t bytes, hipStream_t st) {
+    HIPCHK(hipMemcpyAsync(dst, src, bytes, hipMemcpyDeviceToHost, st));
+    HIPCHK(hipStreamSynchronize(st));
+    return MTB_OK;
+}
+static mtb_status d2h(mtb_ctx *c, void *dst, const void *src, size_t bytes) { return d2h(c, dst, src, bytes, c->stream); }
 static mtb_status h2d(mtb_ctx *c, void *dst, const void *src, size_t bytes) {
     if (bytes == 0) return MTB_OK;
     HIPCHK(hipMemcpyAsync(dst, src, bytes, hipMemcpyHostToDevice, c->stream));
@@ -932,10 +956,16 @@
     const uint8_t *only_flagged = nullptr;
     const uint32_t *seg_cnt = nullptr;
     const void *bound_by_buckets = nullptr;
+    bool overflowed_listed = false;
 };
 
 struct ScoreLaunch { const uint64_t *d_tcoff; bool key64; mtb_score_params sp; ReadLens lens; ResultSink out; };
 typedef std::function<mtb_status(ScoreSrc *, bool *, const ScoreLaunch &)> ScoreSecond;
+typedef std::function<mtb_status(const ScoreLaunch &)> ScoreFork;
+static bool fast_scorer_applies(const mtb_ctx *c, const mtb_index *ix, const mtb_params *p, const ReadLens &lens, uint32_t stride) {
+    const bool key64 = ix->tax.max_id < (1 << 22) && lens.max_len + 3 < (1u << 11);
+    return key64 && stride <= 384u && !c->opt.no_fast_scorer && !(p->seq_mode == 2 && c->opt.no_fast_pairs);
+}
 static mtb_status taxcnt_layout(mtb_ctx *c, uint64_t n_reads, const uint64_t *d_seg, const uint32_t *d_cnt, const ReadLens &lens, const ResultSink &out, int dna_shift, uint64_t *d_tcoff, uint64_t *n_tc) {
     uint32_t *d_bound; uint64_t *d_ws;
     STCHK(ensure(c, "bound", n_reads, &d_bound)); STCHK(ensure(c, "scanws", scan_ws_elems(n_reads + 1), &d_ws));
@@ -947,7 +977,7 @@
     return MTB_OK;
 }
 static mtb_status dev_score(mtb_ctx *c, mtb_index *ix, const mtb_params *p, uint64_t n_reads, const ReadLens &lens, const ResultSink &out, uint64_t *n_tc,
-                            const ScoreSrc &first, const ScoreSecond *second) {
+                            const ScoreSrc &first, const ScoreSecond *second, const ScoreFork *fork = nullptr) {
     mtb_score_params sp; mtb_make_score_params(p, &sp);
     uint64_t *d_tcoff;
     STCHK(ensure(c, "tcoff", n_reads + 1, &d_tcoff));
@@ -956,6 +986,11 @@
     const uint32_t max_nb_first = (uint32_t)mtb_num_buckets((int32_t)lens.max_len, sp.dna_shift);
     const uint32_t max_nb_second = (uint32_t)mtb_num_buckets((int32_t)std::max(lens.max_len, first.max_len_deferred), sp.dna_shift);
     if (max_nb_second > 65535u) return fail(MTB_ERR_ARG, "read too long for mtb_result.n_taxcnt (16 bits): more than 65535 position buckets");
+    if (fork) {
+        uint8_t *d_slow_early;
+        if (first.cursor && fast_scorer_applies(c, ix, p, lens, first.stride)) STCHK(ensure(c, "slowflag", n_reads, &d_slow_early));
+        STCHK((*fork)(ScoreLaunch{d_tcoff, key64, sp, lens, out}));
+    }
     ScoreSrc second_src;
     for (int pass = 0; pass < 2; pass++) {
         const uint32_t max_nb = pass ? max_nb_second : max_nb_first;
@@ -987,7 +1022,7 @@
         out.tc_base, S->list, S->n_list, S->cursor, S->stride, S->seg_by_list, S->direct, S->epoch, S->big_list, S->n_big, S->cnt_out, d_work, S->only_flagged, S->seg_cnt)
         ScoreSrc S_rest;
         const bool pairs = p->seq_mode == 2;
-        if (S->cursor && pass == 0 && key64 && S->stride <= 384u && !c->opt.no_fast_scorer && !(pairs && c->opt.no_fast_pairs)) {
+        if (S->cursor && pass == 0 && fast_scorer_applies(c, ix, p, lens, S->stride)) {
             uint8_t *d_slow;
             STCHK(ensure(c, "slowflag", n_reads, &d_slow));
             HIPCHK(hipMemsetAsync(d_slow, 0, n_reads, c->stream));
@@ -999,7 +1034,7 @@
               else if (S->stride <= 128) MTB_LAUNCH_FAST(2); else if (S->stride <= 192) MTB_LAUNCH_FAST(3); else if (S->stride <= 256) MTB_LAUNCH_FAST(4); else MTB_LAUNCH_FAST(5, 6, false); }
 #undef MTB_LAUNCH_FAST
             hipLaunchKernelGGL(k_count_flags, dim3(256), dim3(256), 0, c->stream, (const uint8_t *)d_slow, n_reads, scal<unsigned long long>(c, SC_N_GENERIC));
-            if (S->big_list && S->n_big) hipLaunchKernelGGL(k_list_flag2, dim3((uint32_t)((n_reads + 255) / 256)), dim3(256), 0, c->stream, (const uint8_t *)d_slow, n_reads, S->big_list, S->n_big);
+            if (S->big_list && S->n_big && !S->overflowed_listed) hipLaunchKernelGGL(k_list_flag2, dim3((uint32_t)((n_reads + 255) / 256)), dim3(256), 0, c->stream, (const uint8_t *)d_slow, n_reads, S->big_list, S->n_big);
             c->fast_used = true;
             S_rest = *S; S_rest.only_flagged = d_slow;
             S = &S_rest;
@@ -2110,10 +2145,10 @@
 static uint64_t ovf_cap_regrown(uint64_t n) { return n + n / 16 + 1024; }
 
 static mtb_status score_fixed_slots(mtb_ctx *c, mtb_index *ix, const mtb_params *p, uint64_t n_reads, const ReadLens &lens, uint64_t nk_real, const SlotSegs &sl,
-                                    const ResultSink &out, uint64_t *n_taxcnt, uint64_t *nm_out) {
+                                    const ResultSink &out, uint64_t *n_taxcnt, uint64_t *nm_out, bool may_overlap = true) {
     hipStream_t st = c->stream;
     uint64_t nm = 0;
-    memset(c->many_stats, 0, sizeof(c->many_stats));
+    memset(c->many_stats, 0, sizeof(c->many_stats)); c->score_overlapped = 0;
     uint32_t *d_biglist, *d_bigcnt, *d_bigidx, *d_bigcur, *d_cnt; uint64_t *d_bigstart = nullptr, *d_ws2, *d_tot; mtb_match *d_big = nullptr;
     STCHK(ensure(c, "biglist", n_reads, &d_biglist)); STCHK(ensure(c, "bigidx", n_reads, &d_bigidx)); STCHK(ensure(c, "livecnt", n_reads, &d_cnt));
     STCHK(ensure(c, "segstart", n_reads + 1, &d_tot)); STCHK(ensure(c, "scanws", scan_ws_elems(n_reads + 1), &d_ws2));
@@ -2127,81 +2162,142 @@
     }
     a.max_seg = a.cap;
     a.big_list = d_biglist; a.n_big = scal<uint32_t>(c, SC_N_DEFERRED); a.cnt_out = d_cnt;
+    const bool tiers = !c->opt.no_score_many && sl.stride <= 384u;
+    const bool early = tiers && may_overlap && fast_scorer_applies(c, ix, p, lens, sl.stride);
+    const bool overlap = early && MTB_SCORE_OVERLAP != 0 && !c->profiling && c->side_stream != nullptr;
+    const bool have_ovf = sl.ovf_region ? c->ovf_max_region != 0 : sl.n_ovf != 0;
+    const bool cap192 = c->opt.many_cap ? c->opt.many_cap <= 192 : sl.stride <= 192u;
+    enum { MS_REST = 0, MS_WORK = 1, MS_STATS = 2, MS_LONG_WORK = 8, MS_N_FIN = 9, MS_N_A = 15, MS_RUN = 16 };
+    unsigned long long *d_ms = nullptr;
+    uint32_t *d_alist = nullptr, *d_rest[2] = {nullptr, nullptr}, *d_fin = nullptr, *d_novf = nullptr, *d_ocur = nullptr, *d_bc3 = nullptr, *d_segcnt = nullptr;
+    uint64_t *d_ostart = nullptr, *d_bs3 = nullptr, *d_wss = d_ws2; uint8_t *d_todo = nullptr;
+    mtb_match *d_ovfg = nullptr;
+    bool grouped = false, many_timed = false, sort_on = false;
+    uint32_t n_a = 0, n_fin = 0, n_rest_all = 0;
+    auto tier_buffers = [&](uint64_t n_sort) -> mtb_status {
+        if (d_ms) return MTB_OK;
+        STCHK(ensure(c, "manystat", 2 * MS_RUN, &d_ms)); STCHK(ensure(c, "restlist", n_reads, &d_rest[0])); STCHK(ensure(c, "restlist2", n_reads, &d_fin));
+        if (early) { STCHK(ensure(c, "overflowed", n_reads, &d_alist)); STCHK(ensure(c, "restlistb", n_reads, &d_rest[1])); STCHK(ensure(c, "scanwsside", scan_ws_elems(n_reads + 1), &d_wss)); }
+        if (have_ovf) {
+            STCHK(ensure(c, "novf", n_reads, &d_novf)); STCHK(ensure(c, "ocur", n_reads, &d_ocur)); STCHK(ensure(c, "ovfstart", n_reads + 1, &d_ostart));
+            STCHK(scratch(c, "ovfg", sl.n_ovf + 1, &d_ovfg));
+        }
+        STCHK(ensure(c, "bigcnt", n_sort, &d_bc3)); STCHK(ensure(c, "bigstart", n_sort + 1, &d_bs3)); STCHK(ensure(c, "bigseg", n_sort, &d_segcnt));
+        STCHK(ensure(c, "todoflag", n_reads, &d_todo));
+        HIPCHK(hipMemsetAsync(d_ms, 0, 2 * MS_RUN * 8, st));
+        return MTB_OK;
+    };
+    auto group_ovf = [&](hipStream_t sq) -> mtb_status {
+        if (!have_ovf || grouped) return MTB_OK;
+        grouped = true;
+        HIPCHK(hipMemsetAsync(d_ocur, 0, n_reads * 4, sq));
+        hipLaunchKernelGGL(k_ovf_count, dim3((uint32_t)((n_reads + 255) / 256)), dim3(256), 0, sq, (const uint32_t *)sl.d_rc, sl.d_off_reads, n_reads, sl.stride - sl.direct, d_novf);
+        scan_launch<uint32_t, uint64_t, false>(sq, d_novf, n_reads, true, d_ostart, d_wss);
+        if (sl.ovf_region) hipLaunchKernelGGL(k_ovf_group, dim3((uint32_t)((c->ovf_max_region + 255) / 256), MTB_OVF_STRIPES), dim3(256), 0, sq, (const mtb_match *)sl.d_ovf, sl.n_ovf,
+                                           (const uint64_t *)d_ostart, (const uint32_t *)d_novf, d_ocur, d_ovfg, sl.ovf_region, (const unsigned long long *)c->d_ovfctr);
+        else hipLaunchKernelGGL(k_ovf_group, dim3((uint32_t)((sl.n_ovf + 255) / 256)), dim3(256), 0, sq, (const mtb_match *)sl.d_ovf, sl.n_ovf,
+                                (const uint64_t *)d_ostart, (const uint32_t *)d_novf, d_ocur, d_ovfg, (uint64_t)0, (const unsigned long long *)nullptr);
+        return MTB_OK;
+    };
+    auto tier_begin = [&](int run, hipStream_t sq, const uint32_t *d_list, const uint32_t *d_n, uint32_t grid, const ScoreLaunch &SL) -> mtb_status {
+        unsigned long long *ms = d_ms + run * MS_RUN;
+        sort_on = SL.key64 && !c->opt.no_many_sort;
+        uint32_t *rest = sort_on ? d_rest[run] : d_rest[0]; uint32_t *n_rest = (uint32_t *)((sort_on ? ms : d_ms) + MS_REST);
+#define MTB_LAUNCH_MANY(K64, CAPV) hipLaunchKernelGGL((k_score_many<K64, CAPV>), dim3(grid), dim3(64), 0, sq, (const mtb_slot16 *)sl.d_segm, sl.stride, sl.direct, sl.epoch, (const uint32_t *)sl.d_rc, sl.d_off_reads, \
+        (const mtb_match *)d_ovfg, (const uint64_t *)d_ostart, d_list, d_n, SL.lens.d_ql, SL.lens.d_ql2, tax_view(ix), SL.sp, SL.d_tcoff, SL.out.d_res, \
+        SL.out.d_tc_tax, SL.out.d_tc_cnt, SL.out.tc_cap, SL.out.tc_base, rest, n_rest, d_cnt, ms + MS_WORK, ms + MS_STATS)
+        if (cap192) { if (SL.key64) MTB_LAUNCH_MANY(true, 192); else MTB_LAUNCH_MANY(false, 192); }
+        else { if (SL.key64) MTB_LAUNCH_MANY(true, 320); else MTB_LAUNCH_MANY(false, 320); }
+#undef MTB_LAUNCH_MANY
+        HIPCHK(hipGetLastError());
+        return MTB_OK;
+    };
+    auto tier_end = [&](int run, hipStream_t sq, uint32_t n_list, const ScoreLaunch &SL) -> mtb_status {
+        unsigned long long *ms = d_ms + run * MS_RUN;
+        uint64_t h[2 * MS_RUN];
+        STCHK(d2h(c, h, d_ms, sizeof(h), sq));
+        const uint64_t *hr = h + run * MS_RUN;
+        if (run == 0 && early) n_list = n_a = (uint32_t)(h[MS_N_A] & 0xFFFFFFFFull);
+        const uint32_t rest_seen = (uint32_t)((sort_on ? hr[MS_REST] : h[MS_REST]) & 0xFFFFFFFFull);
+        const uint32_t n_rest = sort_on ? rest_seen : rest_seen - n_rest_all;
+        n_rest_all += n_rest;
+        c->many_stats[2] += hr[MS_STATS]; c->many_stats[3] += hr[MS_STATS + 1];
+        if (c->opt.many_verbose) fprintf(stderr, "mtb: k_score_many: %u reads listed, %u handed on (routed off / buckets / counts %llu, species table full %llu, survivors beyond the staging %llu); %llu matches, %llu survive the dead-species drop\n",
+                                                n_list, n_rest, (unsigned long long)hr[MS_STATS + 2], (unsigned long long)hr[MS_STATS + 3], (unsigned long long)hr[MS_STATS + 4], (unsigned long long)hr[MS_STATS], (unsigned long long)hr[MS_STATS + 1]);
+        if (!sort_on) { n_fin = n_rest_all; return MTB_OK; }
+        if (!n_rest) return MTB_OK;
+        const uint32_t *d_r = d_rest[run]; mtb_match *d_big3;
+        if (!early) { STCHK(ensure(c, "bigcnt", n_rest, &d_bc3)); STCHK(ensure(c, "bigstart", (uint64_t)n_rest + 1, &d_bs3)); STCHK(ensure(c, "bigseg", n_rest, &d_segcnt)); }
+        hipLaunchKernelGGL(k_big_count, dim3(std::min<uint32_t>(n_rest, 4096)), dim3(64), 0, sq, (const mtb_slot16 *)sl.d_segm, sl.stride, sl.direct, sl.epoch,
+                           (const uint32_t *)sl.d_rc, d_r, n_rest, d_bc3, d_bigidx, scal<uint32_t>(c, SC_MAX_BIG_SEG), sl.d_off_reads);
+        scan_launch<uint32_t, uint64_t, false>(sq, d_bc3, n_rest, true, d_bs3, d_wss);
+        uint64_t total3 = 0;
+        STCHK(d2h(c, &total3, d_bs3 + n_rest, 8, sq));
+        STCHK(scratch(c, "manym", total3 + 1, &d_big3));
+        HIPCHK(hipMemsetAsync(d_todo, 0, n_reads, sq));
+        hipLaunchKernelGGL((k_many_sort<11, 2048u>), dim3(std::min<uint32_t>(n_rest, 256u * 8u)), dim3(MTB_MSORT_NT), 0, sq, (const mtb_slot16 *)sl.d_segm, sl.stride, sl.direct, sl.epoch, (const uint32_t *)sl.d_rc, sl.d_off_reads,
+                           (const mtb_match *)d_ovfg, (const uint64_t *)d_ostart, d_r, n_rest, SL.lens.d_ql, SL.lens.d_ql2, SL.sp.dna_shift, (const uint64_t *)d_bs3, d_big3, d_segcnt, d_todo, 0u, 2u);
+        hipLaunchKernelGGL((k_many_sort<12, 4096u>), dim3(std::min<uint32_t>(n_rest, 256u * 3u)), dim3(MTB_MSORT_NT), 0, sq, (const mtb_slot16 *)sl.d_segm, sl.stride, sl.direct, sl.epoch, (const uint32_t *)sl.d_rc, sl.d_off_reads,
+                           (const mtb_match *)d_ovfg, (const uint64_t *)d_ostart, d_r, n_rest, SL.lens.d_ql, SL.lens.d_ql2, SL.sp.dna_shift, (const uint64_t *)d_bs3, d_big3, d_segcnt, d_todo, 2u, 1u);
+        hipLaunchKernelGGL((k_score_long<2048, 256, 256, 256>), dim3(std::min<uint32_t>(n_rest, 256u * 5u)), dim3(MTB_LONG_NT), 0, sq, (const mtb_match *)d_big3, (const uint64_t *)d_bs3, n_reads, SL.lens.d_ql, SL.lens.d_ql2,
+                           tax_view(ix), SL.sp, SL.d_tcoff, SL.out.d_res, SL.out.d_tc_tax, SL.out.d_tc_cnt, SL.out.tc_cap, SL.out.tc_base, d_todo, ms + MS_LONG_WORK, (const uint32_t *)d_segcnt, d_r, n_rest);
+        hipLaunchKernelGGL(k_list_flagged, dim3((n_rest + 255) / 256), dim3(256), 0, sq, d_r, n_rest, (const uint8_t *)d_todo, (const uint32_t *)d_bc3, d_fin, (uint32_t *)(d_ms + MS_N_FIN), d_cnt);
+        HIPCHK(hipGetLastError());
+        uint64_t left = 0;
+        STCHK(d2h(c, &left, d_ms + MS_N_FIN, 8, sq));
+        if (c->opt.many_verbose) fprintf(stderr, "mtb: k_many_sort + k_score_long: %u reads (%llu records), %llu in all left for the exact-segment path\n", n_rest, (unsigned long long)total3, (unsigned long long)(left & 0xFFFFFFFFull));
+        n_fin = (uint32_t)(left & 0xFFFFFFFFull);
+        return MTB_OK;
+    };
+    ScoreFork fork = [&](const ScoreLaunch &SL) -> mtb_status {
+        STCHK(tier_buffers(n_reads));
+        hipStream_t ss = overlap ? c->side_stream : st;
+        if (overlap) { HIPCHK(hipEventRecord(c->side_ev[0], st)); HIPCHK(hipStreamWaitEvent(ss, c->side_ev[0], 0)); }
+        hipLaunchKernelGGL(k_list_overflowed, dim3((uint32_t)((n_reads + 255) / 256)), dim3(256), 0, ss, (const uint32_t *)sl.d_rc, n_reads, sl.stride - sl.direct, d_alist, (uint32_t *)(d_ms + MS_N_A));
+        if (!overlap) {
+            uint64_t na = 0;
+            STCHK(d2h(c, &na, d_ms + MS_N_A, 8));
+            n_a = (uint32_t)na;
+            if (!n_a) return MTB_OK;
+            KTimer ktm(c, MTB_K_SCORE_MANY); many_timed = true;
+            STCHK(group_ovf(ss));
+            STCHK(tier_begin(0, ss, d_alist, (const uint32_t *)(d_ms + MS_N_A), std::min<uint32_t>((uint32_t)na, 256u * (cap192 ? 12u : 7u)), SL));
+            return tier_end(0, ss, (uint32_t)na, SL);
+        }
+        STCHK(group_ovf(ss));
+        HIPCHK(hipEventRecord(c->side_ev[1], ss));
+        STCHK(tier_begin(0, ss, d_alist, (const uint32_t *)(d_ms + MS_N_A), 256u * MTB_SCORE_OVERLAP_GRID, SL));
+        HIPCHK(hipStreamWaitEvent(st, c->side_ev[1], 0));
+        c->score_overlapped = 1;
+        return MTB_OK;
+    };
     ScoreSecond second = [&](ScoreSrc *b, bool *go, const ScoreLaunch &SL) -> mtb_status {
+        if (overlap) {
+            STCHK(tier_end(0, c->side_stream, 0, SL));
+            HIPCHK(hipEventRecord(c->side_ev[2], c->side_stream)); HIPCHK(hipStreamWaitEvent(st, c->side_ev[2], 0));
+        }
         uint64_t sc = 0;
         STCHK(d2h(c, &sc, scal<uint64_t>(c, SC_N_DEFERRED), 8));
-        uint32_t n_big = (uint32_t)sc;
+        const uint32_t n_b = (uint32_t)sc;
+        uint32_t n_big = n_a + n_b;
         *go = n_big != 0;
         if (!n_big) return MTB_OK;
         c->many_stats[0] = n_big; c->many_stats[1] = 0;
-        const bool no_many = c->opt.no_score_many != 0;
-        uint32_t *d_novf = nullptr; uint64_t *d_ostart = nullptr; mtb_match *d_ovfg = nullptr;
-        if (!no_many && sl.stride <= 384u) {
-            KTimer ktm(c, MTB_K_SCORE_MANY);
-            uint32_t *d_ocur = nullptr, *d_rest;
-            STCHK(ensure(c, "restlist", n_reads, &d_rest));
-            const bool have_ovf = sl.ovf_region ? c->ovf_max_region != 0 : sl.n_ovf != 0;
-            if (have_ovf) {
-                STCHK(ensure(c, "novf", n_reads, &d_novf)); STCHK(ensure(c, "ocur", n_reads, &d_ocur)); STCHK(ensure(c, "ovfstart", n_reads + 1, &d_ostart));
-                STCHK(scratch(c, "ovfg", sl.n_ovf + 1, &d_ovfg));
-                HIPCHK(hipMemsetAsync(d_ocur, 0, n_reads * 4, st));
-                hipLaunchKernelGGL(k_ovf_count, dim3((uint32_t)((n_reads + 255) / 256)), dim3(256), 0, st, (const uint32_t *)sl.d_rc, sl.d_off_reads, n_reads, sl.stride - sl.direct, d_novf);
-                scan_launch<uint32_t, uint64_t, false>(st, d_novf, n_reads, true, d_ostart, d_ws2);
-                if (sl.ovf_region) hipLaunchKernelGGL(k_ovf_group, dim3((uint32_t)((c->ovf_max_region + 255) / 256), MTB_OVF_STRIPES), dim3(256), 0, st, (const mtb_match *)sl.d_ovf, sl.n_ovf,
-                                                   (const uint64_t *)d_ostart, (const uint32_t *)d_novf, d_ocur, d_ovfg, sl.ovf_region, (const unsigned long long *)c->d_ovfctr);
-                else hipLaunchKernelGGL(k_ovf_group, dim3((uint32_t)((sl.n_ovf + 255) / 256)), dim3(256), 0, st, (const mtb_match *)sl.d_ovf, sl.n_ovf,
-                                        (const uint64_t *)d_ostart, (const uint32_t *)d_novf, d_ocur, d_ovfg, (uint64_t)0, (const unsigned long long *)nullptr);
+        if (tiers) {
+            if (n_b) {
+                KTimer ktm(c, many_timed ? MTB_K_SEGSORT : MTB_K_SCORE_MANY);
+                STCHK(tier_buffers(1));
+                STCHK(group_ovf(st));
+                const int run = early ? 1 : 0;
+                STCHK(tier_begin(run, st, (const uint32_t *)d_biglist, scal<const uint32_t>(c, SC_N_DEFERRED), std::min<uint32_t>(n_b, 256u * (cap192 ? 12u : 7u)), SL));
+                STCHK(tier_end(run, st, n_b, SL));
             }
-            unsigned long long *d_ms;
-            STCHK(ensure(c, "manystat", 16, &d_ms));
-            HIPCHK(hipMemsetAsync(d_ms, 0, 16 * 8, st));
-            const bool cap192 = c->opt.many_cap ? c->opt.many_cap <= 192 : sl.stride <= 192u;
-            const uint32_t gridm = std::min<uint32_t>(n_big, 256u * (cap192 ? 12u : 7u));
-#define MTB_LAUNCH_MANY(K64, CAPV) hipLaunchKernelGGL((k_score_many<K64, CAPV>), dim3(gridm), dim3(64), 0, st, (const mtb_slot16 *)sl.d_segm, sl.stride, sl.direct, sl.epoch, (const uint32_t *)sl.d_rc, sl.d_off_reads, \
-            (const mtb_match *)d_ovfg, (const uint64_t *)d_ostart, (const uint32_t *)d_biglist, scal<const uint32_t>(c, SC_N_DEFERRED), SL.lens.d_ql, SL.lens.d_ql2, tax_view(ix), SL.sp, SL.d_tcoff, SL.out.d_res, \
-            SL.out.d_tc_tax, SL.out.d_tc_cnt, SL.out.tc_cap, SL.out.tc_base, d_rest, (uint32_t *)d_ms, d_cnt, d_ms + 1, d_ms + 2)
-            if (cap192) { if (SL.key64) MTB_LAUNCH_MANY(true, 192); else MTB_LAUNCH_MANY(false, 192); }
-            else { if (SL.key64) MTB_LAUNCH_MANY(true, 320); else MTB_LAUNCH_MANY(false, 320); }
-#undef MTB_LAUNCH_MANY
-            HIPCHK(hipGetLastError());
-            uint64_t ms4[8] = {0, 0, 0, 0, 0, 0, 0, 0};
-            STCHK(d2h(c, ms4, d_ms, 64));
-            const uint32_t n_rest = (uint32_t)(ms4[0] & 0xFFFFFFFFull);
-            c->many_stats[1] = n_big - n_rest; c->many_stats[2] = ms4[2]; c->many_stats[3] = ms4[3];
-            if (c->opt.many_verbose) fprintf(stderr, "mtb: k_score_many: %u reads listed, %u handed on (routed off / buckets / counts %llu, species table full %llu, survivors beyond the staging %llu); %llu matches, %llu survive the dead-species drop\n",
-                                                    n_big, n_rest, (unsigned long long)ms4[4], (unsigned long long)ms4[5], (unsigned long long)ms4[6], (unsigned long long)ms4[2], (unsigned long long)ms4[3]);
-            n_big = n_rest;
-            const unsigned long long *d_nleft = d_ms;
-            if (n_big && SL.key64 && !c->opt.no_many_sort) {
-                uint32_t *d_bc3, *d_segcnt, *d_rest2; uint64_t *d_bs3; uint8_t *d_todo; mtb_match *d_big3;
-                STCHK(ensure(c, "bigcnt", n_big, &d_bc3)); STCHK(ensure(c, "bigstart", (uint64_t)n_big + 1, &d_bs3)); STCHK(ensure(c, "bigseg", n_big, &d_segcnt));
-                STCHK(ensure(c, "restlist2", n_reads, &d_rest2)); STCHK(ensure(c, "todoflag", n_reads, &d_todo));
-                hipLaunchKernelGGL(k_big_count, dim3(std::min<uint32_t>(n_big, 4096)), dim3(64), 0, st, (const mtb_slot16 *)sl.d_segm, sl.stride, sl.direct, sl.epoch,
-                                   (const uint32_t *)sl.d_rc, (const uint32_t *)d_rest, n_big, d_bc3, d_bigidx, scal<uint32_t>(c, SC_MAX_BIG_SEG), sl.d_off_reads);
-                scan_launch<uint32_t, uint64_t, false>(st, d_bc3, n_big, true, d_bs3, d_ws2);
-                uint64_t total3 = 0;
-                STCHK(d2h(c, &total3, d_bs3 + n_big, 8));
-                STCHK(scratch(c, "manym", total3 + 1, &d_big3));
-                HIPCHK(hipMemsetAsync(d_todo, 0, n_reads, st));
-                hipLaunchKernelGGL((k_many_sort<11, 2048u>), dim3(std::min<uint32_t>(n_big, 256u * 8u)), dim3(MTB_MSORT_NT), 0, st, (const mtb_slot16 *)sl.d_segm, sl.stride, sl.direct, sl.epoch, (const uint32_t *)sl.d_rc, sl.d_off_reads,
-                                   (const mtb_match *)d_ovfg, (const uint64_t *)d_ostart, (const uint32_t *)d_rest, n_big, SL.lens.d_ql, SL.lens.d_ql2, SL.sp.dna_shift, (const uint64_t *)d_bs3, d_big3, d_segcnt, d_todo, 0u, 2u);
-                hipLaunchKernelGGL((k_many_sort<12, 4096u>), dim3(std::min<uint32_t>(n_big, 256u * 3u)), dim3(MTB_MSORT_NT), 0, st, (const mtb_slot16 *)sl.d_segm, sl.stride, sl.direct, sl.epoch, (const uint32_t *)sl.d_rc, sl.d_off_reads,
-                                   (const mtb_match *)d_ovfg, (const uint64_t *)d_ostart, (const uint32_t *)d_rest, n_big, SL.lens.d_ql, SL.lens.d_ql2, SL.sp.dna_shift, (const uint64_t *)d_bs3, d_big3, d_segcnt, d_todo, 2u, 1u);
-                hipLaunchKernelGGL((k_score_long<2048, 256, 256, 256>), dim3(std::min<uint32_t>(n_big, 256u * 5u)), dim3(MTB_LONG_NT), 0, st, (const mtb_match *)d_big3, (const uint64_t *)d_bs3, n_reads, SL.lens.d_ql, SL.lens.d_ql2,
-                                   tax_view(ix), SL.sp, SL.d_tcoff, SL.out.d_res, SL.out.d_tc_tax, SL.out.d_tc_cnt, SL.out.tc_cap, SL.out.tc_base, d_todo, d_ms + 8, (const uint32_t *)d_segcnt, (const uint32_t *)d_rest, n_big);
-                hipLaunchKernelGGL(k_list_flagged, dim3((n_big + 255) / 256), dim3(256), 0, st, (const uint32_t *)d_rest, n_big, (const uint8_t *)d_todo, (const uint32_t *)d_bc3, d_rest2, (uint32_t *)(d_ms + 9), d_cnt);
-                HIPCHK(hipGetLastError());
-                uint64_t left = 0;
-                STCHK(d2h(c, &left, d_ms + 9, 8));
-                if (c->opt.many_verbose) fprintf(stderr, "mtb: k_many_sort + k_score_long: %u reads (%llu records), %llu left for the exact-segment path\n", n_big, (unsigned long long)total3, (unsigned long long)(left & 0xFFFFFFFFull));
-                n_big = (uint32_t)(left & 0xFFFFFFFFull);
-                d_rest = d_rest2; d_nleft = d_ms + 9;
-            }
+            n_big = n_fin;
             c->many_stats[1] = c->many_stats[0] - n_big;
             *go = n_big != 0;
             if (!n_big) return MTB_OK;
-            d_biglist = d_rest;
-            HIPCHK(hipMemcpyAsync(scal<uint64_t>(c, SC_N_DEFERRED), d_nleft, 8, hipMemcpyDeviceToDevice, st));
+            d_biglist = sort_on ? d_fin : d_rest[0];
+            HIPCHK(hipMemcpyAsync(scal<uint64_t>(c, SC_N_DEFERRED), d_ms + (sort_on ? MS_N_FIN : MS_REST), 8, hipMemcpyDeviceToDevice, st));
         }
         KTimer kt(c, MTB_K_SEGSORT);
         HIPCHK(hipMemsetAsync(d_bigidx, 0xFF, n_reads * 4, st));
@@ -2238,7 +2334,9 @@
         b->sort = false; b->max_seg = (uint32_t)mx; b->grid = std::min<uint32_t>(n_big, 256u * 14u); b->cap = 320;
         return MTB_OK;
     };
-    STCHK(dev_score(c, ix, p, n_reads, lens, out, n_taxcnt, a, &second));
+    a.overflowed_listed = early;
+    {   const mtb_status rs = dev_score(c, ix, p, n_reads, lens, out, n_taxcnt, a, &second, early ? &fork : nullptr);
+        if (rs != MTB_OK) { if (c->score_overlapped) { hipError_t e = hipStreamSynchronize(c->side_stream); (void)e; } return rs; } }
     { KTimer kt(c, MTB_K_SCAN); scan_launch<uint32_t, uint64_t, false>(st, d_cnt, n_reads, true, d_tot, d_ws2); }
     STCHK(d2h(c, &nm, d_tot + n_reads, 8));
     nm += big_total;
@@ -2662,7 +2760,7 @@
     S.n_reads = n_reads; S.n_bases = ex.n_bases; S.n_kmers = ex.nk_real; S.n_matches = nm; S.n_targets = ix->T;
     STCHK(take_generic_reads(c, n_reads, &S.n_generic_reads));
     S.n_slot_reads = (fixed || lslot) ? n_reads : 0;
-    if (fixed) { S.n_deferred_reads = c->many_stats[0]; S.n_many_reads = c->many_stats[1]; S.n_many_matches = c->many_stats[2]; S.n_many_kept = c->many_stats[3]; }
+    if (fixed) { S.n_deferred_reads = c->many_stats[0]; S.n_many_reads = c->many_stats[1]; S.n_many_matches = c->many_stats[2]; S.n_many_kept = c->many_stats[3]; S.score_overlapped = c->score_overlapped; }
     return MTB_OK;
 }
 static mtb_status classify_one(mtb_ctx *c, mtb_index *ix, const mtb_params *p, const Reads &rd, const ResultSink &out, uint64_t *n_taxcnt) {
@@ -2681,7 +2779,7 @@
     S.join_variant = L.join_variant; S.join_tuned = L.join_tuned;
     for (int v = 0; v < 3; v++) S.join_tune_ms[v] = L.join_tune_ms[v];
     S.join_tiles += L.join_tiles; S.join_tiles_windowed += L.join_tiles_windowed; S.join_tiles_outside += L.join_tiles_outside;
-    S.lslot_tail_factor = L.lslot_tail_factor; S.n_lslot_big_reads += L.n_lslot_big_reads;
+    S.score_overlapped |= L.score_overlapped; S.lslot_tail_factor = L.lslot_tail_factor; S.n_lslot_big_reads += L.n_lslot_big_reads;
 }
 
 static mtb_status classify_budgeted(mtb_ctx *c, mtb_index *ix, const mtb_params *p, const Reads &rd, uint64_t n_bases_total, const ResultSink &out, uint64_t *n_taxcnt) {
@@ -3169,7 +3267,7 @@
             ovf_cap = ovf_cap_regrown(sl.n_ovf);
         }
         uint64_t nm = 0; memset(&c->stats, 0, sizeof(c->stats));
-        STCHK(score_fixed_slots(c, ix, p, n_reads, ReadLens{d_ql, d_ql2, c->part_max_len}, c->part_nk_real, sl, sink, n_taxcnt, &nm));
+        STCHK(score_fixed_slots(c, ix, p, n_reads, ReadLens{d_ql, d_ql2, c->part_max_len}, c->part_nk_real, sl, sink, n_taxcnt, &nm,  false));
         c->stats.n_reads = n_reads; c->stats.n_matches = nm; c->stats.n_slot_reads = n_reads; c->stats.n_kmers = c->part_nk_real;
         STCHK(take_generic_reads(c,  0, &c->stats.n_generic_reads));
         return download_packed(c, d_res, d_tt, d_tc, n_reads, results, taxcnt_tax, taxcnt_cnt, n_taxcnt);
```

Result: faster. 73.39, median of 6 (+1.8%).
